# knightyxp/VideoCoF

Measured on AMD Instinct MI355X. Metric: denoised latent tokens/s (4-step 81f@480p Wan2.1 DiT denoise loop, all DiT tokens counted), higher is better.
Workload: dtype bf16; 1 GPU; Wan2.1-T2V-14B + VideoCoF layout, 4-step, 81f@480p (BASELINE configs[2]); layout=VideoCoF (src|ground|tgt), global_batch=1, parallelism=single

## Files before the change

include/wan_hip.h:

```cpp
#ifndef WAN_HIP_H
#define WAN_HIP_H

#include <stdint.h>

#ifdef __cplusplus
extern "C" {
#endif

#define WAN_ABI_VERSION 11

typedef enum {
    WAN_OK = 0,
    WAN_ERR_INVALID = 1,
    WAN_ERR_UNSUPPORTED = 2,
    WAN_ERR_LAUNCH = 3
} wan_status_t;

int wan_abi_version(void);
const char* wan_last_error(void);

wan_status_t wan_set_tuning(const char* key, int value);
int wan_get_tuning(const char* key);
#define WAN_ATTN_VARIANT_W4_LAZY 1
#define WAN_ATTN_VARIANT_W4_MAXFREE 2
#define WAN_ATTN_VARIANT_W8_RUNNING_MAX 3
#define WAN_ATTN_VARIANT_W4_LAZY_QK8 4
#define WAN_ATTN_VARIANT_W4_F8 5
#define WAN_ATTN_VARIANT_FAMILY_MASK 15
#define WAN_ATTN_VARIANT_XCD_PINNED 16
#define WAN_ATTN_VARIANT_SPLIT_TAIL 32

wan_status_t wan_ln_modulate(const float* x, const float* scale, const float* shift, int add_one,
                             void* out_bf16, int64_t rows, int dim, int64_t rows_per_batch,
                             float eps, void* stream);

typedef struct {
    int F, Hp, Wp;
    int mode;
    int f_src;
    int ground_end;
    int64_t token_offset;
    int64_t rows_per_batch;
    int max_pos;
} wan_rope_params;

wan_status_t wan_rmsnorm_rope(void* x0_bf16, const float* w0, void* x1_bf16, const float* w1,
                              int64_t ld, int64_t rows, int dim, int head_dim, float eps,
                              const float* rope_cos, const float* rope_sin,
                              const wan_rope_params* rp, float x0_scale, void* stream);

typedef enum {
    WAN_EPI_BF16 = 0,
    WAN_EPI_GELU_BF16 = 1,
    WAN_EPI_F32 = 2,
    WAN_EPI_RESID_F32 = 3,
    WAN_EPI_BF16_T = 4
} wan_epilogue_t;

wan_status_t wan_gemm_bf16(const void* A, int64_t lda, const void* W, int64_t ldw, const float* bias,
                           void* out, int64_t ldo, int M, int N, int K, int epilogue,
                           const float* gate, int64_t rows_per_batch, void* stream);
int wan_gemm_plan(int M, int N, int K);
#define WAN_GEMM_VARIANT_128 0
#define WAN_GEMM_VARIANT_256_W8 1
#define WAN_GEMM_VARIANT_256_W4 2
#define WAN_GEMM_VARIANT_256_PK 3

wan_status_t wan_gemm_bf16_ws(const void* A, int64_t lda, const void* W, int64_t ldw, const float* bias,
                              void* out, int64_t ldo, int M, int N, int K, int epilogue,
                              const float* gate, int64_t rows_per_batch, void* workspace, int64_t workspace_bytes, void* stream);
int64_t wan_gemm_workspace_bytes(int M, int N, int K);
int wan_gemm_ws_plan(int M, int N, int K);
int wan_gemm_ws_splits(int M, int N, int K);
int wan_gemm_pk_grid(int M, int N);
int wan_gemm_pk_segment(int M, int N, int K, int worker, int index, int* out);

wan_status_t wan_gemm_fp8(const void* A_fp8, int64_t lda, const float* a_row_scale, const void* W_fp8, int64_t ldw,
                          const float* w_row_scale, const float* bias, void* out, int64_t ldo, int M, int N, int K,
                          int epilogue, const float* gate, int64_t rows_per_batch, void* stream);
int wan_gemm_fp8_ws_plan(int M, int N, int K);
int64_t wan_gemm_fp8_workspace_bytes(int M, int N, int K);
wan_status_t wan_gemm_fp8_ws(const void* A_fp8, int64_t lda, const float* a_row_scale, const void* W_fp8, int64_t ldw,
                             const float* w_row_scale, const float* bias, void* out, int64_t ldo, int M, int N, int K,
                             int epilogue, const float* gate, int64_t rows_per_batch, void* workspace, int64_t workspace_bytes,
                             void* stream);
int wan_gemm_fp8_pk_segment(int M, int N, int K, int worker, int index, int* out);
wan_status_t wan_quantize_rows_fp8(const void* x_bf16, int64_t ldx, void* out_fp8, int64_t ldo, float* out_row_scale,
                                   int64_t rows, int cols, void* stream);
wan_status_t wan_ln_modulate_fp8(const float* x, const float* scale, const float* shift, int add_one, void* out_fp8,
                                 float* out_row_scale, int64_t rows, int dim, int64_t rows_per_batch, float eps, void* stream);

wan_status_t wan_attention_fwd(const void* q, int64_t ldq, int64_t q_bstride,
                               const void* k, int64_t ldk, int64_t k_bstride,
                               const void* vt, int64_t ldvt, int64_t vt_bstride,
                               void* out, int64_t ldo, int64_t o_bstride,
                               int batch, int Lq, int Lk, int num_heads, int head_dim,
                               float softmax_scale, int flags, void* workspace, int64_t workspace_bytes,
                               void* stream);
wan_status_t wan_attention_fwd_varlen(const void* q, int64_t ldq, int64_t q_bstride,
                                      const void* k, int64_t ldk, int64_t k_bstride,
                                      const void* vt, int64_t ldvt, int64_t vt_bstride,
                                      void* out, int64_t ldo, int64_t o_bstride,
                                      int batch, int Lq, int Lk, const int32_t* k_lens, int num_heads, int head_dim,
                                      float softmax_scale, int flags, void* workspace, int64_t workspace_bytes,
                                      void* stream);
int64_t wan_attention_workspace_bytes(int batch, int Lq, int Lk, int num_heads, int head_dim);
int wan_attention_plan(int batch, int Lq, int Lk, int num_heads, int head_dim, int flags, int64_t workspace_bytes);
#define WAN_ATTN_Q_PRESCALED 1
#define WAN_ATTN_QK_FP8 2
#define WAN_ATTN_PV_FP8 4
#define WAN_ATTN_QSCALE(softmax_scale) ((softmax_scale) * 1.4426950408889634f)

wan_status_t wan_attention_fwd_qk8(const void* q8, int64_t ldq8, int64_t q8_bstride, int q_exp,
                                   const void* k8, int64_t ldk8, int64_t k8_bstride, int k_exp,
                                   const void* vt, int64_t ldvt, int64_t vt_bstride,
                                   void* out, int64_t ldo, int64_t o_bstride,
                                   int batch, int Lq, int Lk, int num_heads, int head_dim,
                                   void* workspace, int64_t workspace_bytes, void* stream);
wan_status_t wan_attention_fwd_f8(const void* q8, int64_t ldq8, int64_t q8_bstride, int q_exp,
                                  const void* k8, int64_t ldk8, int64_t k8_bstride, int k_exp,
                                  const void* v8, int64_t ldv8, int64_t v8_bstride, const void* v8_scales,
                                  const void* vt, int64_t ldvt, int64_t vt_bstride,
                                  void* out, int64_t ldo, int64_t o_bstride,
                                  int batch, int Lq, int Lk, int num_heads, int head_dim,
                                  void* workspace, int64_t workspace_bytes, void* stream);
int64_t wan_vt_mx_scale_bytes(int batch, int num_heads, int Lk);
wan_status_t wan_vt_quantize_mx(const void* vt_bf16, int64_t ldvt, int64_t vt_bstride, int batch, int num_heads, int Lk,
                                void* v8, int64_t ldv8, int64_t v8_bstride, void* v8_scales, void* stream);
wan_status_t wan_rmsnorm_rope_fp8(const void* x0_bf16, const float* w0, const void* x1_bf16, const float* w1,
                                  int64_t ld, int64_t rows, int dim, int head_dim, float eps,
                                  const float* rope_cos, const float* rope_sin, const wan_rope_params* rp,
                                  float x0_scale, float x1_scale, void* out0_fp8, void* out1_fp8, void* stream);

int64_t wan_col_mean_workspace_bytes(int batch, int dim);
wan_status_t wan_col_mean_bf16(const void* x_bf16, int64_t ld, int64_t rows_per_batch, int valid_rows, int batch, int dim,
                               void* workspace, float* mean, void* stream);
wan_status_t wan_qk_quantize_fp8(const void* q_bf16, const void* k_bf16, int64_t ld, int64_t rows, int dim, int64_t rows_per_batch,
                                 const float* k_mean, float q_scale, float k_scale, void* q8, void* k8, void* stream);

wan_status_t wan_cross_probs(const void* q, int64_t ldq, const void* k, int64_t ldk, int64_t k_bstride, void* probs, int64_t ldp,
                             int batch, int64_t rows_per_batch, int num_heads, int kept, int pad_count, void* stream);
wan_status_t wan_cross_fold_values(const void* w_co, int64_t ldw, const void* vt, int64_t ldvt, int64_t vt_bstride, void* vfold,
                                   int64_t ldo, int64_t vfold_bstride, int batch, int dim, int num_heads, int kept, void* stream);
int wan_cross_fold_plan(int64_t rows, int num_heads, int text_len, int kept, int weights_bf16);
int64_t wan_cross_fold_workspace_bytes(int batch, int dim);

wan_status_t wan_transpose_bf16(const void* in, int64_t ld, void* out_t, int64_t ldt,
                                int64_t rows, int cols, void* stream);

wan_status_t wan_patchify(const void* latent, int in_dtype, void* tokens_bf16, int64_t ldt,
                          int Cin, int F, int H, int W, int pt, int ph, int pw, void* stream);
wan_status_t wan_unpatchify(const float* tokens, int64_t ldt, void* out, int out_dtype,
                            int Cout, int F, int Hp, int Wp, int pt, int ph, int pw, int zero_frames, void* stream);
wan_status_t wan_unpatchify_rep(const float* tokens, int64_t ldt, void* out, int out_dtype,
                                int Cout, int F, int Hp, int Wp, int pt, int ph, int pw, int zero_frames,
                                int rep, int64_t rep_stride, void* stream);

wan_status_t wan_rmsnorm_rope_sp(const void* x0_bf16, const float* w0, const void* x1_bf16, const float* w1,
                                 int64_t ld, int64_t rows, int dim, int head_dim, float eps,
                                 const float* rope_cos, const float* rope_sin, const wan_rope_params* rp,
                                 float x0_scale, void* wire0, void* wire1, int slabs, int batch, void* stream);
wan_status_t wan_sp_pack_heads(const void* x_bf16, int64_t ldx, void* wire, int P, int T, int B, int Cl, void* stream);
wan_status_t wan_sp_unpack_heads(const void* wire, void* x_bf16, int64_t ldx, int P, int T, int B, int Cl, void* stream);
wan_status_t wan_sp_unpack_vt(const void* wire, void* vt_bf16, int64_t ldvt, int P, int B, int Cl, int T, void* stream);
wan_status_t wan_rmsnorm_rope_sp_split(const void* x0_bf16, const float* w0, const void* x1_bf16, const float* w1,
                                       int64_t ld, int64_t rows, int dim, int head_dim, float eps,
                                       const float* rope_cos, const float* rope_sin, const wan_rope_params* rp,
                                       float x0_scale, void* wire0, void* wire1, int slabs, int batch, int split, void* stream);
wan_status_t wan_sp_pack_heads_split(const void* x_bf16, int64_t ldx, void* wire, int P, int T, int B, int Cl, int split, void* stream);
wan_status_t wan_sp_unpack_heads_split(const void* wire, void* x_bf16, int64_t ldx, int P, int T, int B, int Cl, int split, void* stream);

typedef struct wan_sp_comm wan_sp_comm;
#define WAN_SP_UNIQUE_ID_BYTES 128
wan_status_t wan_sp_unique_id(void* id128);
wan_status_t wan_sp_init(wan_sp_comm** comm, const void* id128, int rank, int world_size);
wan_status_t wan_sp_init_from_comm(wan_sp_comm** comm, void* nccl_comm, int rank, int world_size);
int wan_sp_rank(const wan_sp_comm* comm);
int wan_sp_world_size(const wan_sp_comm* comm);
wan_status_t wan_sp_a2a_scatter_heads(wan_sp_comm* comm, const void* send_wire, void* recv_wire, int64_t bytes_total, void* compute_stream);
wan_status_t wan_sp_a2a_gather_heads(wan_sp_comm* comm, const void* send_wire, void* recv_wire, int64_t bytes_total, void* compute_stream);
wan_status_t wan_sp_all_gather(wan_sp_comm* comm, const void* send, void* recv, int64_t bytes_per_rank, void* compute_stream);
wan_status_t wan_sp_wait(wan_sp_comm* comm, void* compute_stream);
int64_t wan_sp_ticket(const wan_sp_comm* comm);
wan_status_t wan_sp_wait_for(wan_sp_comm* comm, int64_t ticket, void* compute_stream);
wan_status_t wan_sp_destroy(wan_sp_comm* comm);

wan_status_t wan_sp_channel_copy(void* dst, const void* src, int64_t bytes, int channels, int threads, void* stream);

typedef struct {
    int dim, ffn_dim, num_heads, text_len;
    float eps;
    const void *w_qk, *w_v, *w_o, *w_cq, *w_co, *w_ffn0, *w_ffn2;
    const float *b_qk, *b_v, *b_o, *b_cq, *b_co, *b_ffn0, *b_ffn2;
    const float *norm_q, *norm_k, *norm_cq;
    const float *norm3_w, *norm3_b;
} wan_block_weights;

typedef struct {
    void *h, *qk, *att, *cq, *ff, *vt;
    int64_t ldvt;
    void* attn_ws_self; int64_t attn_ws_self_bytes;
    void* attn_ws_cross; int64_t attn_ws_cross_bytes;
    void* gemm_ws; int64_t gemm_ws_bytes;
    void* vfold; int64_t vfold_bytes;
    int text_kept;
} wan_block_workspace;

wan_status_t wan_dit_block_forward(float* x, const float* emod, const void* ctx_k, const void* ctx_vt,
                                   const wan_block_weights* w, const wan_block_workspace* ws,
                                   const float* rope_cos, const float* rope_sin, const wan_rope_params* rp,
                                   int batch, int64_t rows_per_batch, int64_t valid_tokens, void* stream);
wan_status_t wan_dit_block_tail_forward(float* x, const float* emod, const void* ctx_k, const void* ctx_vt,
                                        const wan_block_weights* w, const wan_block_workspace* ws,
                                        int batch, int64_t rows_per_batch, void* stream);
wan_status_t wan_dit_block_workspace_bytes(int dim, int ffn_dim, int batch, int64_t rows_per_batch, int64_t valid_tokens,
                                           int64_t* bytes , int64_t* ldvt);

typedef struct {
    int num_layers, in_dim, out_dim, pt, ph, pw;
    const wan_block_weights* blocks;
    const void* pe_w; const float* pe_b;
    const void* head_w; const float* head_b;
} wan_dit_weights;

typedef struct {
    wan_block_workspace block;
    float* x;
    void* tokens;
    float* head_out;
} wan_dit_workspace;

wan_status_t wan_dit_forward(const void* latent, int latent_dtype, void* out, int out_dtype, const float* emod,
                             const float* ehead, const void* const* ctx_k, const void* const* ctx_vt,
                             const wan_dit_weights* w, const wan_dit_workspace* ws, const float* rope_cos,
                             const float* rope_sin, const wan_rope_params* rp, int batch, int F, int H, int W,
                             int64_t rows_per_batch, int zero_frames, void* stream);
wan_status_t wan_dit_forward_rep(const void* latent, int latent_dtype, void* out, int out_dtype, const float* emod,
                                 const float* ehead, const void* const* ctx_k, const void* const* ctx_vt,
                                 const wan_dit_weights* w, const wan_dit_workspace* ws, const float* rope_cos,
                                 const float* rope_sin, const wan_rope_params* rp, int batch, int F, int H, int W,
                                 int64_t rows_per_batch, int zero_frames, int rep, void* stream);

wan_status_t wan_lincomb(void* out, int dtype, const void* x0, const void* x1, const void* x2, const void* x3,
                         float c0, float c1, float c2, float c3, int64_t n, void* stream);

wan_status_t wan_solver_step(void* x0_out, void* prev_out, int dtype, const void* sample, const void* v, const void* m1,
                             const void* m2, const float* noise, float a_s, float a_v, float c_s, float c_0, float c_1,
                             float c_2, float c_n, int64_t n, void* stream);


typedef struct {
    int T_in, H_in, W_in, Cin;
    int T_out, H_out, W_out, Cout;
    int KT, KH, KW;
    int st, sh, sw;
    int pt, ph, pw;
    int upsample2x;
    int time_interleave;
} wan_conv_params;

wan_status_t wan_conv_cl(const void* x, const void* hist, int hist_frames, const void* w, int64_t ldw,
                         const float* bias, const void* resid, void* out, int64_t ldo,
                         const wan_conv_params* p, void* stream);

wan_status_t wan_rmsnorm_silu_cl(const void* x_bf16, const float* gamma, void* out_bf16, int64_t rows, int C,
                                 int silu, void* stream);

wan_status_t wan_softmax_rows(const float* scores, int64_t lds, void* probs_bf16, int64_t ldp, int64_t rows,
                              int n, int npad, float scale, void* stream);

wan_status_t wan_video_to_cl(const void* video, int in_dtype, void* out_bf16, int Cv, int Cpad, int64_t npix, void* stream);
wan_status_t wan_cl_to_video(const void* x_bf16, int64_t ld, void* out, int out_dtype, int Cv, int64_t npix,
                             int clamp, void* stream);


wan_status_t wan_frames_u8_to_video(const void* frames_u8, void* out, int out_dtype, int B, int T, int H, int W,
                                    void* stream);

wan_status_t wan_video_to_frames_u8(const void* video, int in_dtype, void* frames_u8, int B, int T, int H, int W,
                                    int t0, int nt, int T_out, int t_dst, void* stream);

#define WAN_RESAMPLE_MAX_TAPS 24
int64_t wan_frames_resample_table_bytes(int n_out, int taps);
wan_status_t wan_frames_u8_resample(const void* src_u8, void* dst_u8, int B, int T, int H, int W, int Ho, int Wo,
                                    const void* xtab, int kx, const void* ytab, int ky, void* stream);

#define WAN_COMPOSE_MAX_SRC 16
enum { WAN_COMPOSE_U8 = 0, WAN_COMPOSE_F32 = 1, WAN_COMPOSE_BF16 = 2 };
enum { WAN_COMPOSE_COPY = 0, WAN_COMPOSE_LOADER_ROUNDTRIP = 1, WAN_COMPOSE_WRITER = 2, WAN_COMPOSE_NORMALIZE = 3 };
typedef struct {
    const void* base;
    const int* rescale_flag;
    int64_t extent;
    int64_t stride_c, stride_t, stride_y, stride_x;
// ... 74 lines not shown
```

videocof_amd/_lib.py:

```python
from __future__ import annotations

import ctypes
import os
from ctypes import POINTER, Structure, c_char_p, c_float, c_int, c_int64, c_void_p

_HERE = os.path.dirname(os.path.abspath(__file__))
LIB_PATH = os.environ.get("WAN_HIP_LIB") or os.path.join(_HERE, "libwan_hip.so")
ABI_VERSION = 11
ATTN_Q_PRESCALED = 1
LOG2E = 1.4426950408889634
ATTN_VARIANT_NAMES = {1: "attn_fwd_w4_kernel<.,.,ref> (4-wave, lazy softmax reference)",
                      2: "attn_fwd_w4_kernel<.,false,0> (4-wave, max-free attempt) + attn_fwd_w4_kernel<.,false,1,true> (lazy-reference fix-up of flagged workgroups)",
                      3: "(retired in round 5: the 8-wave running-max kernel)",
                      4: "attn_fwd_w4_kernel<0,.,1,false,true> (4-wave, lazy softmax reference, QK^T on the fp8 matrix pipe)",
                      5: "attn_fwd_f8_kernel (4-wave, QK^T and P.V on the fp8 matrix pipe, checked max-free softmax) + "
                         "attn_fwd_w4_kernel<0,false,1,true,true> (fp8-QK^T lazy-reference fix-up of flagged workgroups)"}
ATTN_VARIANT_XCD_PINNED, ATTN_VARIANT_SPLIT_TAIL = 16, 32
GEMM_VARIANT_KERNELS = {0: "gemm_bf16_kernel", 1: "gemm256_kernel", 2: "gemm_w4_kernel", 3: "gemm_pk_kernel"}


def attn_variant_name(code: int) -> str:
    name = ATTN_VARIANT_NAMES.get(code & 15, f"unknown({code})")
    if code & ATTN_VARIANT_XCD_PINNED:
        name += ", heads pinned to XCDs"
    if code & ATTN_VARIANT_SPLIT_TAIL:
        name += " + split-KV tail round (4-wave SPLIT kernel + attn_combine_kernel)"
    return name

WAN_OK, WAN_ERR_INVALID, WAN_ERR_UNSUPPORTED, WAN_ERR_LAUNCH = 0, 1, 2, 3
EPI_BF16, EPI_GELU_BF16, EPI_F32, EPI_RESID_F32, EPI_BF16_T = 0, 1, 2, 3, 4


class RopeParams(Structure):
    _fields_ = [("F", c_int), ("Hp", c_int), ("Wp", c_int), ("mode", c_int), ("f_src", c_int),
                ("ground_end", c_int), ("token_offset", c_int64), ("rows_per_batch", c_int64),
                ("max_pos", c_int)]


class BoxProbeResult(Structure):
    _fields_ = [("mfma_mix_tflops", c_float), ("copy_tbps", c_float), ("mfma_ms", c_float), ("copy_ms", c_float)]


class ComposeSrc(Structure):
    _fields_ = ([("base", c_void_p), ("rescale_flag", c_void_p), ("extent", c_int64)] +
                [(n, c_int64) for n in ("stride_c", "stride_t", "stride_y", "stride_x")] +
                [(n, c_int) for n in ("kind", "mode", "rescale", "t0", "y0", "x0", "nt", "h", "w", "dst_y", "dst_x")])


COMPOSE_MAX_SRC = 16
COMPOSE_U8, COMPOSE_F32, COMPOSE_BF16 = 0, 1, 2
COMPOSE_COPY, COMPOSE_LOADER_ROUNDTRIP, COMPOSE_WRITER, COMPOSE_NORMALIZE = 0, 1, 2, 3


class YuvPlanes(Structure):
    _fields_ = ([(n, c_void_p) for n in ("y", "cb", "cr")] +
                [(n, c_int64) for n in ("y_extent", "cb_extent", "cr_extent", "y_row", "y_frame", "c_row", "c_frame")] +
                [(n, c_int) for n in ("c_step", "sub_x", "sub_y", "cosited")])


class YuvCoef(Structure):
    _fields_ = [("k", c_int * 9), ("yo", c_int)]


class ConvParams(Structure):
    _fields_ = [(n, c_int) for n in ("T_in", "H_in", "W_in", "Cin", "T_out", "H_out", "W_out", "Cout",
                                     "KT", "KH", "KW", "st", "sh", "sw", "pt", "ph", "pw",
                                     "upsample2x", "time_interleave")]


class BlockWeights(Structure):
    _fields_ = ([(n, c_int) for n in ("dim", "ffn_dim", "num_heads", "text_len")] + [("eps", c_float)] +
                [(n, c_void_p) for n in ("w_qk", "w_v", "w_o", "w_cq", "w_co", "w_ffn0", "w_ffn2",
                                         "b_qk", "b_v", "b_o", "b_cq", "b_co", "b_ffn0", "b_ffn2",
                                         "norm_q", "norm_k", "norm_cq", "norm3_w", "norm3_b")])


class BlockWorkspace(Structure):
    _fields_ = ([(n, c_void_p) for n in ("h", "qk", "att", "cq", "ff", "vt")] + [("ldvt", c_int64)] +
                [("attn_ws_self", c_void_p), ("attn_ws_self_bytes", c_int64),
                 ("attn_ws_cross", c_void_p), ("attn_ws_cross_bytes", c_int64),
                 ("gemm_ws", c_void_p), ("gemm_ws_bytes", c_int64),
                 ("vfold", c_void_p), ("vfold_bytes", c_int64), ("text_kept", c_int)])


class DitWeights(Structure):
    _fields_ = ([(n, c_int) for n in ("num_layers", "in_dim", "out_dim", "pt", "ph", "pw")] +
                [("blocks", POINTER(BlockWeights))] + [(n, c_void_p) for n in ("pe_w", "pe_b", "head_w", "head_b")])


class DitWorkspace(Structure):
    _fields_ = [("block", BlockWorkspace), ("x", c_void_p), ("tokens", c_void_p), ("head_out", c_void_p)]


SIGNATURES = {
    "wan_abi_version": (c_int, []),
    "wan_box_probe_scratch_bytes": (c_int64, []),
    "wan_box_probe": (c_int, [POINTER(BoxProbeResult), c_void_p, c_int64, c_int, c_void_p]),
    "wan_last_error": (c_char_p, []),
    "wan_set_tuning": (c_int, [c_char_p, c_int]),
    "wan_get_tuning": (c_int, [c_char_p]),
    "wan_ln_modulate": (c_int, [c_void_p, c_void_p, c_void_p, c_int, c_void_p, c_int64, c_int, c_int64,
                                c_float, c_void_p]),
    "wan_rmsnorm_rope": (c_int, [c_void_p, c_void_p, c_void_p, c_void_p, c_int64, c_int64, c_int, c_int,
                                 c_float, c_void_p, c_void_p, POINTER(RopeParams), c_float, c_void_p]),
    "wan_gemm_bf16": (c_int, [c_void_p, c_int64, c_void_p, c_int64, c_void_p, c_void_p, c_int64,
                              c_int, c_int, c_int, c_int, c_void_p, c_int64, c_void_p]),
    "wan_rmsnorm_rope_sp": (c_int, [c_void_p, c_void_p, c_void_p, c_void_p, c_int64, c_int64, c_int, c_int,
                                    c_float, c_void_p, c_void_p, POINTER(RopeParams), c_float, c_void_p, c_void_p, c_int, c_int,
                                    c_void_p]),
    "wan_sp_pack_heads": (c_int, [c_void_p, c_int64, c_void_p, c_int, c_int, c_int, c_int, c_void_p]),
    "wan_sp_unpack_heads": (c_int, [c_void_p, c_void_p, c_int64, c_int, c_int, c_int, c_int, c_void_p]),
    "wan_sp_unpack_vt": (c_int, [c_void_p, c_void_p, c_int64, c_int, c_int, c_int, c_int, c_void_p]),
    "wan_rmsnorm_rope_sp_split": (c_int, [c_void_p, c_void_p, c_void_p, c_void_p, c_int64, c_int64, c_int, c_int,
                                          c_float, c_void_p, c_void_p, POINTER(RopeParams), c_float, c_void_p, c_void_p, c_int, c_int,
                                          c_int, c_void_p]),
    "wan_sp_pack_heads_split": (c_int, [c_void_p, c_int64, c_void_p, c_int, c_int, c_int, c_int, c_int, c_void_p]),
    "wan_sp_unpack_heads_split": (c_int, [c_void_p, c_void_p, c_int64, c_int, c_int, c_int, c_int, c_int, c_void_p]),
    "wan_dit_block_forward": (c_int, [c_void_p, c_void_p, c_void_p, c_void_p, POINTER(BlockWeights), POINTER(BlockWorkspace),
                                      c_void_p, c_void_p, POINTER(RopeParams), c_int, c_int64, c_int64, c_void_p]),
    "wan_dit_block_tail_forward": (c_int, [c_void_p, c_void_p, c_void_p, c_void_p, POINTER(BlockWeights), POINTER(BlockWorkspace),
                                           c_int, c_int64, c_void_p]),
    "wan_dit_forward": (c_int, [c_void_p, c_int, c_void_p, c_int, c_void_p, c_void_p, POINTER(c_void_p), POINTER(c_void_p),
                                POINTER(DitWeights), POINTER(DitWorkspace), c_void_p, c_void_p, POINTER(RopeParams),
                                c_int, c_int, c_int, c_int, c_int64, c_int, c_void_p]),
    "wan_dit_forward_rep": (c_int, [c_void_p, c_int, c_void_p, c_int, c_void_p, c_void_p, POINTER(c_void_p), POINTER(c_void_p),
                                    POINTER(DitWeights), POINTER(DitWorkspace), c_void_p, c_void_p, POINTER(RopeParams),
                                    c_int, c_int, c_int, c_int, c_int64, c_int, c_int, c_void_p]),
    "wan_dit_block_workspace_bytes": (c_int, [c_int, c_int, c_int, c_int64, c_int64, POINTER(c_int64), POINTER(c_int64)]),
    "wan_gemm_fp8": (c_int, [c_void_p, c_int64, c_void_p, c_void_p, c_int64, c_void_p, c_void_p, c_void_p, c_int64,
                             c_int, c_int, c_int, c_int, c_void_p, c_int64, c_void_p]),
    "wan_gemm_fp8_ws": (c_int, [c_void_p, c_int64, c_void_p, c_void_p, c_int64, c_void_p, c_void_p, c_void_p, c_int64,
                                c_int, c_int, c_int, c_int, c_void_p, c_int64, c_void_p, c_int64, c_void_p]),
    "wan_gemm_fp8_ws_plan": (c_int, [c_int, c_int, c_int]),
    "wan_gemm_fp8_workspace_bytes": (c_int64, [c_int, c_int, c_int]),
    "wan_gemm_fp8_pk_segment": (c_int, [c_int, c_int, c_int, c_int, c_int, POINTER(c_int)]),
    "wan_quantize_rows_fp8": (c_int, [c_void_p, c_int64, c_void_p, c_int64, c_void_p, c_int64, c_int, c_void_p]),
    "wan_ln_modulate_fp8": (c_int, [c_void_p, c_void_p, c_void_p, c_int, c_void_p, c_void_p, c_int64, c_int, c_int64,
                                    c_float, c_void_p]),
    "wan_attention_fwd": (c_int, [c_void_p, c_int64, c_int64, c_void_p, c_int64, c_int64,
                                  c_void_p, c_int64, c_int64, c_void_p, c_int64, c_int64,
                                  c_int, c_int, c_int, c_int, c_int, c_float, c_int, c_void_p, c_int64, c_void_p]),
    "wan_attention_fwd_varlen": (c_int, [c_void_p, c_int64, c_int64, c_void_p, c_int64, c_int64,
                                         c_void_p, c_int64, c_int64, c_void_p, c_int64, c_int64,
                                         c_int, c_int, c_int, c_void_p, c_int, c_int, c_float, c_int, c_void_p, c_int64, c_void_p]),
    "wan_attention_fwd_qk8": (c_int, [c_void_p, c_int64, c_int64, c_int, c_void_p, c_int64, c_int64, c_int,
                                      c_void_p, c_int64, c_int64, c_void_p, c_int64, c_int64,
                                      c_int, c_int, c_int, c_int, c_int, c_void_p, c_int64, c_void_p]),
    "wan_rmsnorm_rope_fp8": (c_int, [c_void_p, c_void_p, c_void_p, c_void_p, c_int64, c_int64, c_int, c_int,
                                     c_float, c_void_p, c_void_p, POINTER(RopeParams), c_float, c_float, c_void_p, c_void_p,
                                     c_void_p]),
    "wan_attention_fwd_f8": (c_int, [c_void_p, c_int64, c_int64, c_int, c_void_p, c_int64, c_int64, c_int,
                                     c_void_p, c_int64, c_int64, c_void_p, c_void_p, c_int64, c_int64, c_void_p, c_int64, c_int64,
                                     c_int, c_int, c_int, c_int, c_int, c_void_p, c_int64, c_void_p]),
    "wan_vt_mx_scale_bytes": (c_int64, [c_int, c_int, c_int]),
    "wan_vt_quantize_mx": (c_int, [c_void_p, c_int64, c_int64, c_int, c_int, c_int, c_void_p, c_int64, c_int64, c_void_p, c_void_p]),
    "wan_col_mean_workspace_bytes": (c_int64, [c_int, c_int]),
    "wan_col_mean_bf16": (c_int, [c_void_p, c_int64, c_int64, c_int, c_int, c_int, c_void_p, c_void_p, c_void_p]),
    "wan_qk_quantize_fp8": (c_int, [c_void_p, c_void_p, c_int64, c_int64, c_int, c_int64, c_void_p, c_float, c_float, c_void_p, c_void_p,
                                    c_void_p]),
    "wan_attention_workspace_bytes": (c_int64, [c_int, c_int, c_int, c_int, c_int]),
    "wan_cross_probs": (c_int, [c_void_p, c_int64, c_void_p, c_int64, c_int64, c_void_p, c_int64, c_int, c_int64, c_int, c_int, c_int,
                                c_void_p]),
    "wan_cross_fold_values": (c_int, [c_void_p, c_int64, c_void_p, c_int64, c_int64, c_void_p, c_int64, c_int64, c_int, c_int, c_int,
                                      c_int, c_void_p]),
    "wan_cross_fold_plan": (c_int, [c_int64, c_int, c_int, c_int, c_int]),
    "wan_cross_fold_workspace_bytes": (c_int64, [c_int, c_int]),
    "wan_sp_unique_id": (c_int, [c_void_p]),
    "wan_sp_init": (c_int, [ctypes.POINTER(c_void_p), c_void_p, c_int, c_int]),
    "wan_sp_init_from_comm": (c_int, [ctypes.POINTER(c_void_p), c_void_p, c_int, c_int]),
    "wan_sp_rank": (c_int, [c_void_p]),
    "wan_sp_world_size": (c_int, [c_void_p]),
    "wan_sp_a2a_scatter_heads": (c_int, [c_void_p, c_void_p, c_void_p, c_int64, c_void_p]),
    "wan_sp_a2a_gather_heads": (c_int, [c_void_p, c_void_p, c_void_p, c_int64, c_void_p]),
    "wan_sp_all_gather": (c_int, [c_void_p, c_void_p, c_void_p, c_int64, c_void_p]),
    "wan_sp_wait": (c_int, [c_void_p, c_void_p]),
    "wan_sp_ticket": (c_int64, [c_void_p]),
    "wan_sp_wait_for": (c_int, [c_void_p, c_int64, c_void_p]),
    "wan_sp_destroy": (c_int, [c_void_p]),
    "wan_sp_channel_copy": (c_int, [c_void_p, c_void_p, c_int64, c_int, c_int, c_void_p]),
    "wan_attention_plan": (c_int, [c_int, c_int, c_int, c_int, c_int, c_int, c_int64]),
    "wan_gemm_plan": (c_int, [c_int, c_int, c_int]),
    "wan_gemm_ws_plan": (c_int, [c_int, c_int, c_int]),
    "wan_gemm_ws_splits": (c_int, [c_int, c_int, c_int]),
    "wan_gemm_workspace_bytes": (c_int64, [c_int, c_int, c_int]),
    "wan_gemm_pk_grid": (c_int, [c_int, c_int]),
    "wan_gemm_pk_segment": (c_int, [c_int, c_int, c_int, c_int, c_int, POINTER(c_int)]),
    "wan_gemm_bf16_ws": (c_int, [c_void_p, c_int64, c_void_p, c_int64, c_void_p, c_void_p, c_int64,
                                 c_int, c_int, c_int, c_int, c_void_p, c_int64, c_void_p, c_int64, c_void_p]),
    "wan_transpose_bf16": (c_int, [c_void_p, c_int64, c_void_p, c_int64, c_int64, c_int, c_void_p]),
    "wan_patchify": (c_int, [c_void_p, c_int, c_void_p, c_int64, c_int, c_int, c_int, c_int,
                             c_int, c_int, c_int, c_void_p]),
    "wan_unpatchify": (c_int, [c_void_p, c_int64, c_void_p, c_int, c_int, c_int, c_int, c_int,
                               c_int, c_int, c_int, c_int, c_void_p]),
    "wan_unpatchify_rep": (c_int, [c_void_p, c_int64, c_void_p, c_int, c_int, c_int, c_int, c_int,
                                   c_int, c_int, c_int, c_int, c_int, c_int64, c_void_p]),
    "wan_lincomb": (c_int, [c_void_p, c_int, c_void_p, c_void_p, c_void_p, c_void_p, c_float, c_float, c_float, c_float,
                            c_int64, c_void_p]),
    "wan_solver_step": (c_int, [c_void_p, c_void_p, c_int, c_void_p, c_void_p, c_void_p, c_void_p, c_void_p, c_float, c_float,
                                c_float, c_float, c_float, c_float, c_float, c_int64, c_void_p]),
    "wan_gemm_bf16_batched": (c_int, [c_void_p, c_int64, c_int64, c_void_p, c_int64, c_int64, c_void_p, c_int64, c_int64,
                                      c_int, c_int, c_int, c_int, c_int, c_void_p]),
    "wan_embedding_rows": (c_int, [c_void_p, c_void_p, c_int64, c_void_p, c_int64, c_int, c_void_p]),
    "wan_rmsnorm_rows": (c_int, [c_void_p, c_void_p, c_void_p, c_int, c_int64, c_int, c_float, c_void_p]),
    "wan_t5_softmax_bias": (c_int, [c_void_p, c_int64, c_void_p, c_void_p, c_void_p, c_int64, c_int, c_int, c_int, c_int,
                                    c_int, c_void_p]),
    "wan_mul_bf16": (c_int, [c_void_p, c_void_p, c_void_p, c_int64, c_void_p]),
    "wan_conv_cl": (c_int, [c_void_p, c_void_p, c_int, c_void_p, c_int64, c_void_p, c_void_p, c_void_p, c_int64,
                            POINTER(ConvParams), c_void_p]),
    "wan_rmsnorm_silu_cl": (c_int, [c_void_p, c_void_p, c_void_p, c_int64, c_int, c_int, c_void_p]),
    "wan_softmax_rows": (c_int, [c_void_p, c_int64, c_void_p, c_int64, c_int64, c_int, c_int, c_float, c_void_p]),
    "wan_video_to_cl": (c_int, [c_void_p, c_int, c_void_p, c_int, c_int, c_int64, c_void_p]),
    "wan_cl_to_video": (c_int, [c_void_p, c_int64, c_void_p, c_int, c_int, c_int64, c_int, c_void_p]),
    "wan_frames_u8_to_video": (c_int, [c_void_p, c_void_p, c_int, c_int, c_int, c_int, c_int, c_void_p]),
    "wan_video_to_frames_u8": (c_int, [c_void_p, c_int, c_void_p, c_int, c_int, c_int, c_int, c_int, c_int, c_int, c_int,
                                       c_void_p]),
    "wan_frames_resample_table_bytes": (c_int64, [c_int, c_int]),
    "wan_frames_u8_resample": (c_int, [c_void_p, c_void_p, c_int, c_int, c_int, c_int, c_int, c_int, c_void_p, c_int, c_void_p, c_int,
                                       c_void_p]),
    "wan_frames_u8_compose": (c_int, [POINTER(ComposeSrc), c_int, c_void_p, c_int, c_int, c_int, c_int, c_void_p]),
    "wan_video_range_flag": (c_int, [c_void_p, c_int, c_int64, c_void_p, c_void_p]),
    "wan_yuv_to_frames_u8": (c_int, [POINTER(YuvPlanes), POINTER(YuvCoef), c_void_p, c_int, c_int, c_int, c_void_p]),
    "wan_frames_u8_to_yuv": (c_int, [c_void_p, POINTER(YuvPlanes), POINTER(YuvCoef), c_int, c_int, c_int, c_void_p]),
    "wan_change_mask_workspace_bytes": (c_int64, [c_int, c_int, c_int, c_int]),
    "wan_change_mask": (c_int, [c_void_p, c_void_p, c_void_p, c_int, c_int, c_int, c_int, c_int, c_int, c_int, c_int, c_int, c_void_p,
                                c_int64, c_void_p]),
    "wan_plane_u8_resample": (c_int, [c_void_p, c_void_p, c_void_p, c_int, c_int, c_int, c_int, c_int, c_void_p, c_int, c_void_p, c_int,
                                      c_void_p]),
    "wan_frames_u8_composite": (c_int, [c_void_p, c_void_p, c_void_p, c_void_p, c_int, c_int, c_int, c_int, c_int, c_int, c_int,
                                        c_void_p]),
    "wan_clip_stats_workspace_bytes": (c_int64, [c_int, c_int, c_int]),
    "wan_clip_stats": (c_int, [c_void_p, c_void_p, c_void_p, c_void_p, c_int, c_int, c_int, c_int, c_void_p, c_int64, c_void_p]),
}

_lib = None


def load() -> ctypes.CDLL:
    global _lib
    if _lib is not None:
        return _lib
    if not os.path.isfile(LIB_PATH):
        raise RuntimeError(
            f"{LIB_PATH} not found: the HIP kernels are not built. Run `make` (or "
            "`python -c 'import __graft_entry__ as g; g.build()'`) in the repo root. "
            "There is no CPU/eager fallback for this path.")
    lib = ctypes.CDLL(LIB_PATH)
    for name, (res, args) in SIGNATURES.items():
        try:
            fn = getattr(lib, name)
        except AttributeError as e:
            raise RuntimeError(f"{LIB_PATH} does not export `{name}` (stale build?)") from e
        fn.restype = res
        fn.argtypes = args
    if lib.wan_abi_version() != ABI_VERSION:
        raise RuntimeError(f"libwan_hip ABI {lib.wan_abi_version()} != binding ABI {ABI_VERSION}; rebuild")
    _lib = lib
    return lib


def check(status: int, what: str) -> None:
    if status == WAN_OK:
        return
    msg = load().wan_last_error().decode(errors="replace")
    if status == WAN_ERR_INVALID:
        raise ValueError(f"{what}: {msg}")
    raise RuntimeError(f"{what}: {msg} (status {status})")
```

videocof_amd/csrc/common.hpp:

```cpp
#pragma once
#include <hip/hip_runtime.h>
#include <stdint.h>
#include <stdio.h>
#include <stdarg.h>

#include "../../include/wan_hip.h"

typedef __bf16 bf16_t;
typedef __bf16 bf16x2 __attribute__((ext_vector_type(2)));
typedef __bf16 bf16x4 __attribute__((ext_vector_type(4)));
typedef __bf16 bf16x8 __attribute__((ext_vector_type(8)));
typedef float f32x2 __attribute__((ext_vector_type(2)));
typedef float f32x4 __attribute__((ext_vector_type(4)));
typedef float f32x16 __attribute__((ext_vector_type(16)));
typedef unsigned int u32x2 __attribute__((ext_vector_type(2)));
typedef unsigned int u32x4 __attribute__((ext_vector_type(4)));

#define WAN_WAVE 64

void wan_set_error(const char* fmt, ...);
int wan_cu_count();
int wan_resident_cus();
enum { WAN_TUNE_ATTN_TAIL = 0, WAN_TUNE_ATTN_FAST, WAN_TUNE_ATTN_XCD_MAP, WAN_TUNE_GEMM_GM, WAN_TUNE_GEMM_PHASES,
       WAN_TUNE_DEBUG_CHECKS, WAN_TUNE_GEMM_VARIANT, WAN_TUNE_CONV_XCD, WAN_TUNE_GEMM_W4, WAN_TUNE_CONV_FAST, WAN_TUNE_CONV_PATCH, WAN_TUNE_ATTN_REF, WAN_TUNE_CONV_HEAD, WAN_TUNE_GEMM_EXP, WAN_TUNE_GEMM_PK, WAN_TUNE_GEMM_PK_WORKERS, WAN_TUNE_GEMM_PK_MIN_UNITS, WAN_TUNE_GEMM_PK_ORDER, WAN_TUNE_GEMM_PK_FORM, WAN_TUNE_ROW_GROUP, WAN_TUNE_SP_INLINE, WAN_TUNE_GEMM_SPLITK, WAN_TUNE_CONV_MFMA, WAN_TUNE_ATTN_PERSIST, WAN_TUNE_SP_RESERVE_CUS, WAN_TUNE_CROSS_FOLD, WAN_TUNE_COUNT };
int wan_tune(int which);
void wan_note_attn_variant(int variant);
void wan_note_cross_fold(int folded);
int wan_last_cross_fold();
#ifdef __cplusplus
#include <atomic>
wan_status_t wan_once_per_device(std::atomic<uint64_t>& done, wan_status_t (*init)());
#endif
#define WAN_REQUIRE(cond, code, ...)            \
    do {                                        \
        if (!(cond)) {                          \
            wan_set_error(__VA_ARGS__);         \
            return (code);                      \
        }                                       \
    } while (0)
#define WAN_CHECK_LAUNCH(name)                                                        \
    do {                                                                              \
        hipError_t e__ = hipGetLastError();                                           \
        if (e__ != hipSuccess) {                                                      \
            wan_set_error("%s: launch failed: %s", name, hipGetErrorString(e__));     \
            return WAN_ERR_LAUNCH;                                                    \
        }                                                                             \
    } while (0)

__device__ __forceinline__ float bf16lo_to_f32(unsigned int w) { return __uint_as_float(w << 16); }
__device__ __forceinline__ float bf16hi_to_f32(unsigned int w) { return __uint_as_float(w & 0xffff0000u); }

__device__ __forceinline__ unsigned int pack_bf16x2(float lo, float hi) {
    f32x2 v = {lo, hi};
    bf16x2 b = __builtin_convertvector(v, bf16x2);
    return __builtin_bit_cast(unsigned int, b);
}

__device__ __forceinline__ float wave_sum(float v) {
#pragma unroll
    for (int o = 32; o > 0; o >>= 1) v += __shfl_xor(v, o, 64);
    return v;
}

template <int NW>
__device__ __forceinline__ float block_sum(float v, float* red) {
    v = wave_sum(v);
    const int wid = threadIdx.x >> 6;
    __syncthreads();
    if ((threadIdx.x & 63) == 0) red[wid] = v;
    __syncthreads();
    float t = 0.f;
#pragma unroll
    for (int i = 0; i < NW; ++i) t += red[i];
    return t;
}

__device__ __forceinline__ float wave_max(float v) {
#pragma unroll
    for (int o = 32; o > 0; o >>= 1) v = fmaxf(v, __shfl_xor(v, o, 64));
    return v;
}

template <int NW>
__device__ __forceinline__ float block_max(float v, float* red) {
    v = wave_max(v);
    const int wid = threadIdx.x >> 6;
    __syncthreads();
    if ((threadIdx.x & 63) == 0) red[wid] = v;
    __syncthreads();
    float t = red[0];
#pragma unroll
    for (int i = 1; i < NW; ++i) t = fmaxf(t, red[i]);
    return t;
}

__device__ __forceinline__ unsigned int pack_fp8x4(float a, float b, float c, float d) {
    a = fminf(fmaxf(a, -448.f), 448.f); b = fminf(fmaxf(b, -448.f), 448.f);
    c = fminf(fmaxf(c, -448.f), 448.f); d = fminf(fmaxf(d, -448.f), 448.f);
    int w = __builtin_amdgcn_cvt_pk_fp8_f32(a, b, 0, false);
    w = __builtin_amdgcn_cvt_pk_fp8_f32(c, d, w, true);
    return (unsigned int)w;
}

__device__ __forceinline__ float gelu_tanh_f32(float x) {
    constexpr float k1 = -2.0f * 0.7978845608028654f * 1.4426950408889634f;
    constexpr float k3 = k1 * 0.044715f;
    const float a = __builtin_fmaf(x * x, k3, k1) * x;
    return x * __builtin_amdgcn_rcpf(1.0f + __builtin_amdgcn_exp2f(a));
}

__device__ __forceinline__ void glds16(const void* gsrc, void* lds_wave_base) {
    __builtin_amdgcn_global_load_lds(
        (const __attribute__((address_space(1))) void*)gsrc,
        (__attribute__((address_space(3))) void*)lds_wave_base, 16, 0, 0);
}
```

videocof_amd/csrc/cross_fold.hip:

```cpp
#include "common.hpp"

#include <math.h>

namespace {

constexpr int CF_KEYS = 64;
constexpr int CF_D = 128;
constexpr int CF_PROB_NB = 8;
constexpr int CF_FOLD_NB = 2;
constexpr int CF_VS_LD = CF_D + 8;

__device__ __forceinline__ int perm_row(int t, int r) { return 16 * (r >> 3) + 8 * ((r >> 2) & 1) + 4 * t + (r & 3); }

__device__ __forceinline__ void mfma_head(const bf16x8 (&a)[2][8], const bf16x8 (&b)[8], f32x16 (&acc)[2]) {
#pragma unroll
    for (int t = 0; t < 2; ++t) {
#pragma unroll
        for (int i = 0; i < 16; ++i) acc[t][i] = 0.f;
#pragma unroll
        for (int s = 0; s < 8; ++s) acc[t] = __builtin_amdgcn_mfma_f32_32x32x16_bf16(a[t][s], b[s], acc[t], 0, 0, 0);
    }
}

__device__ __forceinline__ u32x4 pack8(const f32x16 (&acc)[2], int i) {
    u32x4 o;
    o[0] = pack_bf16x2(acc[0][4 * i + 0], acc[0][4 * i + 1]);
    o[1] = pack_bf16x2(acc[0][4 * i + 2], acc[0][4 * i + 3]);
    o[2] = pack_bf16x2(acc[1][4 * i + 0], acc[1][4 * i + 1]);
    o[3] = pack_bf16x2(acc[1][4 * i + 2], acc[1][4 * i + 3]);
    return o;
}

__global__ __launch_bounds__(256) void cross_probs_kernel(const bf16_t* __restrict__ q, int64_t ldq, const bf16_t* __restrict__ k,
                                                          int64_t ldk, int64_t k_bstride, bf16_t* __restrict__ p, int64_t ldp, int L,
                                                          int kept, float log2_pad) {
    const int lane = threadIdx.x & 63, wave = threadIdx.x >> 6, r = lane & 31, g = lane >> 5;
    const int h = blockIdx.y, b = blockIdx.z;
    const bf16x8 zero8 = {0, 0, 0, 0, 0, 0, 0, 0};
    bf16x8 ka[2][8];
    const bf16_t* kh = k + (int64_t)b * k_bstride + (int64_t)h * CF_D + g * 64;
#pragma unroll
    for (int t = 0; t < 2; ++t) {
        const int key = perm_row(t, r);
#pragma unroll
        for (int s = 0; s < 8; ++s) ka[t][s] = key <= kept ? *(const bf16x8*)(kh + (int64_t)key * ldk + s * 8) : zero8;
    }
    const int first = blockIdx.x * (4 * CF_PROB_NB);
    for (int it = 0; it < CF_PROB_NB; ++it) {
        const int row0 = (first + it * 4 + wave) * 32;
        if (row0 >= L) break;
        const int row = row0 + r;
        const int64_t grow = (int64_t)b * L + (row < L ? row : L - 1);
        const bf16_t* qr = q + grow * ldq + (int64_t)h * CF_D + g * 64;
        bf16x8 qb[8];
#pragma unroll
        for (int s = 0; s < 8; ++s) qb[s] = *(const bf16x8*)(qr + s * 8);
        f32x16 acc[2];
        mfma_head(ka, qb, acc);
        float m = -INFINITY;
#pragma unroll
        for (int t = 0; t < 2; ++t)
#pragma unroll
            for (int i = 0; i < 4; ++i)
#pragma unroll
                for (int jj = 0; jj < 4; ++jj) {
                    const int key = 16 * i + 8 * g + 4 * t + jj;
                    float s = acc[t][4 * i + jj];
                    s = key == kept ? s + log2_pad : s;
                    s = key > kept ? -INFINITY : s;
                    acc[t][4 * i + jj] = s;
                    m = fmaxf(m, s);
                }
        m = fmaxf(m, __shfl_xor(m, 32, 64));
        float sum = 0.f;
#pragma unroll
        for (int t = 0; t < 2; ++t)
#pragma unroll
            for (int i = 0; i < 16; ++i) {
                const float e = __builtin_amdgcn_exp2f(acc[t][i] - m);
                acc[t][i] = e;
                sum += e;
            }
        sum += __shfl_xor(sum, 32, 64);
        const float inv = __builtin_amdgcn_rcpf(sum);
#pragma unroll
        for (int t = 0; t < 2; ++t)
#pragma unroll
            for (int i = 0; i < 16; ++i) acc[t][i] *= inv;
        if (row < L) {
            bf16_t* pr = p + grow * ldp + (int64_t)h * CF_KEYS + 8 * g;
#pragma unroll
            for (int i = 0; i < 4; ++i) *(u32x4*)(pr + 16 * i) = pack8(acc, i);
        }
    }
}

__global__ __launch_bounds__(256) void cross_fold_kernel(const bf16_t* __restrict__ w, int64_t ldw, const bf16_t* __restrict__ vt,
                                                         int64_t ldvt, int64_t vt_bstride, bf16_t* __restrict__ out, int64_t ldo,
                                                         int64_t out_bstride, int C, int kept) {
    __shared__ __attribute__((aligned(16))) bf16_t vs[CF_KEYS * CF_VS_LD];
    const int lane = threadIdx.x & 63, wave = threadIdx.x >> 6, r = lane & 31, g = lane >> 5;
    const int h = blockIdx.y, b = blockIdx.z;
    const bf16_t* vh = vt + (int64_t)b * vt_bstride + (int64_t)h * CF_D * ldvt;
#pragma unroll
    for (int it = 0; it < 4; ++it) {
        const int idx = it * 256 + threadIdx.x, d = idx >> 3, c = idx & 7;
        bf16x8 v = {0, 0, 0, 0, 0, 0, 0, 0};
        if (c * 8 <= kept) v = *(const bf16x8*)(vh + (int64_t)d * ldvt + c * 8);
#pragma unroll
        for (int e = 0; e < 8; ++e) vs[(c * 8 + e) * CF_VS_LD + d] = c * 8 + e <= kept ? v[e] : (bf16_t)0.f;
    }
    __syncthreads();
    bf16x8 va[2][8];
#pragma unroll
    for (int t = 0; t < 2; ++t)
#pragma unroll
        for (int s = 0; s < 8; ++s) va[t][s] = *(const bf16x8*)(vs + perm_row(t, r) * CF_VS_LD + g * 64 + s * 8);
    const int first = blockIdx.x * (4 * CF_FOLD_NB);
    for (int it = 0; it < CF_FOLD_NB; ++it) {
        const int n0 = (first + it * 4 + wave) * 32;
        if (n0 >= C) break;
        const int n = n0 + r;
        const bf16_t* wr = w + (int64_t)n * ldw + (int64_t)h * CF_D + g * 64;
        bf16x8 wb[8];
#pragma unroll
        for (int s = 0; s < 8; ++s) wb[s] = *(const bf16x8*)(wr + s * 8);
        f32x16 acc[2];
        mfma_head(va, wb, acc);
        bf16_t* orow = out + (int64_t)b * out_bstride + (int64_t)n * ldo + (int64_t)h * CF_KEYS + 8 * g;
#pragma unroll
        for (int i = 0; i < 4; ++i) *(u32x4*)(orow + 16 * i) = pack8(acc, i);
    }
}

inline bool aligned16(const void* p) { return ((uintptr_t)p & 15) == 0; }

std::atomic<int> g_last_cross_fold{0};

}

int wan_last_cross_fold() { return g_last_cross_fold.load(std::memory_order_relaxed); }
void wan_note_cross_fold(int folded) { g_last_cross_fold.store(folded, std::memory_order_relaxed); }

#define WAN_CROSS_FOLD_MIN_ROWS 2048
extern "C" int wan_cross_fold_plan(int64_t rows, int num_heads, int text_len, int kept, int weights_bf16) {
    const int mode = wan_tune(WAN_TUNE_CROSS_FOLD);
    if (mode <= 0 || !weights_bf16 || rows <= 0 || num_heads <= 0) return 0;
    if (kept < 1 || kept + 1 > CF_KEYS || kept >= text_len) return 0;
    if (mode >= 2) return 1;
    const int K = num_heads * CF_KEYS;
    if (K < 1024 || K % 128 != 0) return 0;
    return rows >= WAN_CROSS_FOLD_MIN_ROWS ? 1 : 0;
}

extern "C" int64_t wan_cross_fold_workspace_bytes(int batch, int dim) {
    if (batch <= 0 || dim <= 0 || dim % CF_D != 0) return 0;
    return (int64_t)batch * dim * (dim / CF_D * CF_KEYS) * 2;
}

extern "C" wan_status_t wan_cross_probs(const void* q, int64_t ldq, const void* k, int64_t ldk, int64_t k_bstride, void* probs,
                                        int64_t ldp, int batch, int64_t rows_per_batch, int num_heads, int kept, int pad_count,
                                        void* stream) {
    WAN_REQUIRE(q && k && probs, WAN_ERR_INVALID, "wan_cross_probs: null tensor");
    WAN_REQUIRE(batch > 0 && rows_per_batch > 0 && num_heads > 0 && (int64_t)batch * rows_per_batch <= 0x7fffffff && batch <= 65535 &&
                    num_heads <= 65535,
                WAN_ERR_INVALID, "wan_cross_probs: batch=%d rows_per_batch=%lld heads=%d", batch, (long long)rows_per_batch, num_heads);
    WAN_REQUIRE(kept >= 0 && kept + 1 <= CF_KEYS && pad_count >= 1, WAN_ERR_UNSUPPORTED,
                "wan_cross_probs: kept=%d (kept + 1 distinct keys must be <= 64) pad_count=%d", kept, pad_count);
    WAN_REQUIRE(ldq >= (int64_t)num_heads * CF_D && ldk >= (int64_t)num_heads * CF_D && ldp >= (int64_t)num_heads * CF_KEYS &&
                    k_bstride >= (int64_t)(kept + 1) * ldk,
                WAN_ERR_INVALID, "wan_cross_probs: ldq=%lld ldk=%lld ldp=%lld k_bstride=%lld too small", (long long)ldq, (long long)ldk,
                (long long)ldp, (long long)k_bstride);
    WAN_REQUIRE(ldq % 8 == 0 && ldk % 8 == 0 && ldp % 8 == 0 && k_bstride % 8 == 0 && aligned16(q) && aligned16(k) && aligned16(probs),
                WAN_ERR_INVALID, "wan_cross_probs: rows must be 16-byte aligned");
    const int L = (int)rows_per_batch;
    const int per_wg = 32 * 4 * CF_PROB_NB;
    dim3 grid((L + per_wg - 1) / per_wg, num_heads, batch);
    hipLaunchKernelGGL(cross_probs_kernel, grid, dim3(256), 0, (hipStream_t)stream, (const bf16_t*)q, ldq, (const bf16_t*)k, ldk,
                       k_bstride, (bf16_t*)probs, ldp, L, kept, log2f((float)pad_count));
    WAN_CHECK_LAUNCH("wan_cross_probs");
    return WAN_OK;
}

extern "C" wan_status_t wan_cross_fold_values(const void* w_co, int64_t ldw, const void* vt, int64_t ldvt, int64_t vt_bstride,
                                              void* vfold, int64_t ldo, int64_t vfold_bstride, int batch, int dim, int num_heads,
                                              int kept, void* stream) {
    WAN_REQUIRE(w_co && vt && vfold, WAN_ERR_INVALID, "wan_cross_fold_values: null tensor");
    WAN_REQUIRE(batch > 0 && batch <= 65535 && num_heads > 0 && num_heads <= 65535 && dim == num_heads * CF_D, WAN_ERR_UNSUPPORTED,
                "wan_cross_fold_values: batch=%d dim=%d heads=%d (head_dim must be 128)", batch, dim, num_heads);
    WAN_REQUIRE(kept >= 0 && kept + 1 <= CF_KEYS, WAN_ERR_UNSUPPORTED, "wan_cross_fold_values: kept=%d (kept + 1 must be <= 64)", kept);
    const int64_t K = (int64_t)num_heads * CF_KEYS;
    WAN_REQUIRE(ldw >= dim && ldvt >= (kept + 8) / 8 * 8 && ldo >= K && vt_bstride >= (int64_t)dim * ldvt && vfold_bstride >= (int64_t)dim * ldo,
                WAN_ERR_INVALID, "wan_cross_fold_values: ldw=%lld ldvt=%lld ldo=%lld vt_bstride=%lld vfold_bstride=%lld too small",
                (long long)ldw, (long long)ldvt, (long long)ldo, (long long)vt_bstride, (long long)vfold_bstride);
    WAN_REQUIRE(ldw % 8 == 0 && ldvt % 8 == 0 && ldo % 8 == 0 && vt_bstride % 8 == 0 && vfold_bstride % 8 == 0 && aligned16(w_co) &&
                    aligned16(vt) && aligned16(vfold),
                WAN_ERR_INVALID, "wan_cross_fold_values: rows must be 16-byte aligned");
    const int per_wg = 32 * 4 * CF_FOLD_NB;
    dim3 grid((dim + per_wg - 1) / per_wg, num_heads, batch);
    hipLaunchKernelGGL(cross_fold_kernel, grid, dim3(256), 0, (hipStream_t)stream, (const bf16_t*)w_co, ldw, (const bf16_t*)vt, ldvt,
                       vt_bstride, (bf16_t*)vfold, ldo, vfold_bstride, dim, kept);
    WAN_CHECK_LAUNCH("wan_cross_fold_values");
    return WAN_OK;
}
```

videocof_amd/csrc/dit_block.cpp:

```cpp
#include "common.hpp"

namespace {
inline const char* at(const void* p, int64_t bytes) { return (const char*)p + bytes; }
inline char* at(void* p, int64_t bytes) { return (char*)p + bytes; }
}

#define WAN_TRY(call)                   \
    do {                                \
        const wan_status_t st__ = (call); \
        if (st__ != WAN_OK) return st__; \
    } while (0)

extern "C" wan_status_t wan_dit_block_tail_forward(float* x, const float* emod, const void* ctx_k, const void* ctx_vt,
                                                   const wan_block_weights* w, const wan_block_workspace* ws,
                                                   int batch, int64_t rows_per_batch, void* stream);

extern "C" wan_status_t wan_dit_block_forward(float* x, const float* emod, const void* ctx_k, const void* ctx_vt,
                                              const wan_block_weights* w, const wan_block_workspace* ws,
                                              const float* rope_cos, const float* rope_sin, const wan_rope_params* rp,
                                              int batch, int64_t rows_per_batch, int64_t valid_tokens, void* stream) {
    WAN_REQUIRE(x && emod && ctx_k && ctx_vt && w && ws && rope_cos && rope_sin && rp, WAN_ERR_INVALID,
                "wan_dit_block_forward: null argument");
    WAN_REQUIRE(batch > 0 && rows_per_batch > 0 && valid_tokens > 0 && valid_tokens <= rows_per_batch, WAN_ERR_INVALID,
                "wan_dit_block_forward: batch=%d rows_per_batch=%lld valid_tokens=%lld", batch, (long long)rows_per_batch,
                (long long)valid_tokens);
    const int C = w->dim, F = w->ffn_dim, H = w->num_heads, T = w->text_len;
    WAN_REQUIRE(C > 0 && H > 0 && C == H * 128 && F > 0 && T > 0, WAN_ERR_UNSUPPORTED,
                "wan_dit_block_forward: dim=%d heads=%d (head_dim must be 128) ffn=%d text_len=%d", C, H, F, T);
    WAN_REQUIRE(ws->h && ws->qk && ws->att && ws->cq && ws->ff && ws->vt, WAN_ERR_INVALID, "wan_dit_block_forward: null workspace");
    void* const GWS = ws->gemm_ws;
    const int64_t GWSB = ws->gemm_ws_bytes;
    const int64_t Ll = rows_per_batch, M = (int64_t)batch * Ll;
    WAN_REQUIRE(M <= 0x7fffffff && valid_tokens <= 0x7fffffff, WAN_ERR_UNSUPPORTED, "wan_dit_block_forward: too many rows");
    const int64_t lk_pad = (valid_tokens + 63) / 64 * 64;
    WAN_REQUIRE(ws->ldvt >= lk_pad && ws->ldvt % 8 == 0, WAN_ERR_INVALID,
                "wan_dit_block_forward: ldvt=%lld must be >= roundup(valid_tokens,64)=%lld and a multiple of 8", (long long)ws->ldvt,
                (long long)lk_pad);
    const float eps = w->eps;
    const float qs = (float)(0.08838834764831845 * 1.4426950408889634);
    const int64_t bC = (int64_t)batch * C;
    const float* shift_msa = emod, *scale_msa = emod + bC, *gate_msa = emod + 2 * bC;
    void* qk = ws->qk;
    void* kpart = at(qk, (int64_t)C * 2);
    wan_rope_params rope = *rp;
    rope.rows_per_batch = Ll;

    WAN_TRY(wan_ln_modulate(x, scale_msa, shift_msa, 1, ws->h, M, C, Ll, eps, stream));
    WAN_TRY(wan_gemm_bf16_ws(ws->h, C, w->w_qk, C, w->b_qk, qk, 2 * C, (int)M, 2 * C, C, WAN_EPI_BF16, nullptr, 0, GWS, GWSB, stream));
    WAN_TRY(wan_rmsnorm_rope(qk, w->norm_q, kpart, w->norm_k, 2 * C, M, C, 128, eps, rope_cos, rope_sin, &rope, qs, stream));
    for (int b = 0; b < batch; ++b)
        WAN_TRY(wan_gemm_bf16_ws(at(ws->h, (int64_t)b * Ll * C * 2), C, w->w_v, C, w->b_v, at(ws->vt, (int64_t)b * C * ws->ldvt * 2),
                              ws->ldvt, (int)valid_tokens, C, C, WAN_EPI_BF16_T, nullptr, 0, GWS, GWSB, stream));
    WAN_TRY(wan_attention_fwd(qk, 2 * C, Ll * 2 * C, kpart, 2 * C, Ll * 2 * C, ws->vt, ws->ldvt, (int64_t)C * ws->ldvt, ws->att, C, Ll * C,
                              batch, (int)Ll, (int)valid_tokens, H, 128, 0.f, WAN_ATTN_Q_PRESCALED, ws->attn_ws_self,
                              ws->attn_ws_self_bytes, stream));
    WAN_TRY(wan_gemm_bf16_ws(ws->att, C, w->w_o, C, w->b_o, x, C, (int)M, C, C, WAN_EPI_RESID_F32, gate_msa, Ll, GWS, GWSB, stream));
    return wan_dit_block_tail_forward(x, emod, ctx_k, ctx_vt, w, ws, batch, rows_per_batch, stream);
}

extern "C" wan_status_t wan_dit_block_tail_forward(float* x, const float* emod, const void* ctx_k, const void* ctx_vt,
                                                   const wan_block_weights* w, const wan_block_workspace* ws,
                                                   int batch, int64_t rows_per_batch, void* stream) {
    WAN_REQUIRE(x && emod && ctx_k && ctx_vt && w && ws, WAN_ERR_INVALID, "wan_dit_block_tail_forward: null argument");
    WAN_REQUIRE(batch > 0 && rows_per_batch > 0, WAN_ERR_INVALID, "wan_dit_block_tail_forward: batch=%d rows_per_batch=%lld", batch,
                (long long)rows_per_batch);
    const int C = w->dim, F = w->ffn_dim, H = w->num_heads, T = w->text_len;
    WAN_REQUIRE(C > 0 && H > 0 && C == H * 128 && F > 0 && T > 0, WAN_ERR_UNSUPPORTED,
                "wan_dit_block_tail_forward: dim=%d heads=%d (head_dim must be 128) ffn=%d text_len=%d", C, H, F, T);
    WAN_REQUIRE(ws->h && ws->att && ws->cq && ws->ff, WAN_ERR_INVALID, "wan_dit_block_tail_forward: null workspace");
    void* const GWS = ws->gemm_ws;
    const int64_t GWSB = ws->gemm_ws_bytes;
    const int64_t Ll = rows_per_batch, M = (int64_t)batch * Ll;
    WAN_REQUIRE(M <= 0x7fffffff, WAN_ERR_UNSUPPORTED, "wan_dit_block_tail_forward: too many rows");
    const float eps = w->eps;
    const float qs = (float)(0.08838834764831845 * 1.4426950408889634);
    const int64_t bC = (int64_t)batch * C;
    const float* shift_mlp = emod + 3 * bC, *scale_mlp = emod + 4 * bC, *gate_mlp = emod + 5 * bC;
    WAN_TRY(wan_ln_modulate(x, w->norm3_w, w->norm3_b, 0, ws->h, M, C, M, eps, stream));
    WAN_TRY(wan_gemm_bf16_ws(ws->h, C, w->w_cq, C, w->b_cq, ws->cq, C, (int)M, C, C, WAN_EPI_BF16, nullptr, 0, GWS, GWSB, stream));
    WAN_TRY(wan_rmsnorm_rope(ws->cq, w->norm_cq, nullptr, nullptr, C, M, C, 128, eps, nullptr, nullptr, nullptr, qs, stream));
    const int kept = ws->text_kept;
    const bool fold = ws->vfold && ws->vfold_bytes >= wan_cross_fold_workspace_bytes(batch, C) && wan_cross_fold_plan(M, H, T, kept, 1);
    wan_note_cross_fold(fold ? 1 : 0);
    if (fold) {
        const int64_t Kf = (int64_t)H * 64;
        WAN_TRY(wan_cross_probs(ws->cq, C, ctx_k, C, (int64_t)T * C, ws->att, Kf, batch, Ll, H, kept, T - kept, stream));
        WAN_TRY(wan_cross_fold_values(w->w_co, C, ctx_vt, T, (int64_t)C * T, ws->vfold, Kf, (int64_t)C * Kf, batch, C, H, kept, stream));
        for (int b = 0; b < batch; ++b)
            WAN_TRY(wan_gemm_bf16_ws(at(ws->att, (int64_t)b * Ll * Kf * 2), Kf, at(ws->vfold, (int64_t)b * C * Kf * 2), Kf, w->b_co,
                                  x + (int64_t)b * Ll * C, C, (int)Ll, C, (int)Kf, WAN_EPI_RESID_F32, nullptr, 0, GWS, GWSB, stream));
    } else {
        WAN_TRY(wan_attention_fwd(ws->cq, C, Ll * C, ctx_k, C, (int64_t)T * C, ctx_vt, T, (int64_t)C * T, ws->att, C, Ll * C, batch, (int)Ll,
                                  T, H, 128, 0.f, WAN_ATTN_Q_PRESCALED, ws->attn_ws_cross, ws->attn_ws_cross_bytes, stream));
        WAN_TRY(wan_gemm_bf16_ws(ws->att, C, w->w_co, C, w->b_co, x, C, (int)M, C, C, WAN_EPI_RESID_F32, nullptr, 0, GWS, GWSB, stream));
    }
    WAN_TRY(wan_ln_modulate(x, scale_mlp, shift_mlp, 1, ws->h, M, C, Ll, eps, stream));
    WAN_TRY(wan_gemm_bf16_ws(ws->h, C, w->w_ffn0, C, w->b_ffn0, ws->ff, F, (int)M, F, C, WAN_EPI_GELU_BF16, nullptr, 0, GWS, GWSB, stream));
    WAN_TRY(wan_gemm_bf16_ws(ws->ff, F, w->w_ffn2, F, w->b_ffn2, x, C, (int)M, C, F, WAN_EPI_RESID_F32, gate_mlp, Ll, GWS, GWSB, stream));
    return WAN_OK;
}

extern "C" wan_status_t wan_dit_block_workspace_bytes(int dim, int ffn_dim, int batch, int64_t rows_per_batch, int64_t valid_tokens,
                                                      int64_t* bytes , int64_t* ldvt) {
    WAN_REQUIRE(bytes && ldvt && dim > 0 && ffn_dim > 0 && batch > 0 && rows_per_batch > 0 && valid_tokens > 0, WAN_ERR_INVALID,
                "wan_dit_block_workspace_bytes: bad argument");
    const int64_t M = (int64_t)batch * rows_per_batch;
    *ldvt = (valid_tokens + 63) / 64 * 64;
    bytes[0] = M * dim * 2; bytes[1] = M * 2 * dim * 2; bytes[2] = M * dim * 2; bytes[3] = M * dim * 2;
    bytes[4] = M * ffn_dim * 2; bytes[5] = (int64_t)batch * dim * *ldvt * 2;
    return WAN_OK;
}

static wan_status_t dit_forward(const void* latent, int latent_dtype, void* out, int out_dtype, const float* emod,
                                const float* ehead, const void* const* ctx_k, const void* const* ctx_vt,
                                const wan_dit_weights* w, const wan_dit_workspace* ws, const float* rope_cos,
                                const float* rope_sin, const wan_rope_params* rp, int batch, int F, int H, int W,
                                int64_t rows_per_batch, int zero_frames, int rep, void* stream) {
    WAN_REQUIRE(latent && out && emod && ehead && ctx_k && ctx_vt && w && ws && rp, WAN_ERR_INVALID, "wan_dit_forward: null argument");
    WAN_REQUIRE(w->num_layers > 0 && w->blocks && w->pe_w && w->pe_b && w->head_w && w->head_b, WAN_ERR_INVALID,
                "wan_dit_forward: incomplete weights");
    WAN_REQUIRE(ws->x && ws->tokens && ws->head_out, WAN_ERR_INVALID, "wan_dit_forward: null workspace");
    void* const GWS = ws->block.gemm_ws;
    const int64_t GWSB = ws->block.gemm_ws_bytes;
    const int pt = w->pt, ph = w->ph, pw = w->pw;
    WAN_REQUIRE(pt > 0 && ph > 0 && pw > 0 && F > 0 && H > 0 && W > 0 && F % pt == 0 && H % ph == 0 && W % pw == 0, WAN_ERR_INVALID,
                "wan_dit_forward: latent (%d,%d,%d) is not a multiple of the patch (%d,%d,%d)", F, H, W, pt, ph, pw);
    const int gf = F / pt, gh = H / ph, gw = W / pw;
    const int64_t L = (int64_t)gf * gh * gw, Ll = rows_per_batch;
    WAN_REQUIRE(batch > 0 && L <= Ll && (int64_t)batch * Ll <= 0x7fffffff, WAN_ERR_INVALID,
                "wan_dit_forward: batch=%d tokens=%lld rows_per_batch=%lld", batch, (long long)L, (long long)Ll);
    WAN_REQUIRE(rp->F == gf && rp->Hp == gh && rp->Wp == gw, WAN_ERR_INVALID, "wan_dit_forward: rope grid (%d,%d,%d) != latent grid (%d,%d,%d)",
                rp->F, rp->Hp, rp->Wp, gf, gh, gw);
    const int C = w->blocks[0].dim;
    const int pv = pt * ph * pw, Kpe = w->in_dim * pv, Nh = w->out_dim * pv;
    const int64_t M = (int64_t)batch * Ll;
    const int64_t lat_el = latent_dtype == 0 ? 4 : 2, out_el = out_dtype == 0 ? 4 : 2;
    WAN_REQUIRE((latent_dtype == 0 || latent_dtype == 1) && (out_dtype == 0 || out_dtype == 1), WAN_ERR_INVALID,
                "wan_dit_forward: dtypes must be 0 (fp32) or 1 (bf16)");

    WAN_REQUIRE(hipMemsetAsync(ws->x, 0, (size_t)M * C * 4, (hipStream_t)stream) == hipSuccess, WAN_ERR_LAUNCH,
                "wan_dit_forward: hipMemsetAsync failed");
    for (int b = 0; b < batch; ++b) {
        WAN_TRY(wan_patchify(at(latent, (int64_t)b * w->in_dim * F * H * W * lat_el), latent_dtype, ws->tokens, Kpe, w->in_dim, F, H, W,
                             pt, ph, pw, stream));
        WAN_TRY(wan_gemm_bf16_ws(ws->tokens, Kpe, w->pe_w, Kpe, w->pe_b, ws->x + (int64_t)b * Ll * C, C, (int)L, C, Kpe, WAN_EPI_F32,
                              nullptr, 0, GWS, GWSB, stream));
    }
    const int64_t emod_layer = 6 * (int64_t)batch * C;
    for (int l = 0; l < w->num_layers; ++l) {
        WAN_REQUIRE(w->blocks[l].dim == C, WAN_ERR_INVALID, "wan_dit_forward: block %d has dim %d != %d", l, w->blocks[l].dim, C);
        WAN_TRY(wan_dit_block_forward(ws->x, emod + l * emod_layer, ctx_k[l], ctx_vt[l], &w->blocks[l], &ws->block, rope_cos, rope_sin, rp,
                                      batch, Ll, L, stream));
    }
    const int64_t bC = (int64_t)batch * C;
    WAN_TRY(wan_ln_modulate(ws->x, ehead + bC, ehead, 1, ws->block.h, M, C, Ll, w->blocks[0].eps, stream));
    WAN_TRY(wan_gemm_bf16_ws(ws->block.h, C, w->head_w, C, w->head_b, ws->head_out, Nh, (int)M, Nh, C, WAN_EPI_F32, nullptr, 0, GWS, GWSB, stream));
    WAN_REQUIRE(rep >= 1, WAN_ERR_INVALID, "wan_dit_forward: rep=%d", rep);
    const int64_t sample = (int64_t)w->out_dim * F * H * W;
    for (int b = 0; b < batch; ++b) {
        if (rep == 1)
            WAN_TRY(wan_unpatchify(ws->head_out + (int64_t)b * Ll * Nh, Nh, at(out, b * sample * out_el), out_dtype,
                                   w->out_dim, gf, gh, gw, pt, ph, pw, zero_frames, stream));
        else
            WAN_TRY(wan_unpatchify_rep(ws->head_out + (int64_t)b * Ll * Nh, Nh, at(out, b * sample * out_el), out_dtype,
                                       w->out_dim, gf, gh, gw, pt, ph, pw, zero_frames, rep, batch * sample, stream));
    }
    return WAN_OK;
}

extern "C" wan_status_t wan_dit_forward(const void* latent, int latent_dtype, void* out, int out_dtype, const float* emod,
                                        const float* ehead, const void* const* ctx_k, const void* const* ctx_vt,
                                        const wan_dit_weights* w, const wan_dit_workspace* ws, const float* rope_cos,
                                        const float* rope_sin, const wan_rope_params* rp, int batch, int F, int H, int W,
                                        int64_t rows_per_batch, int zero_frames, void* stream) {
    return dit_forward(latent, latent_dtype, out, out_dtype, emod, ehead, ctx_k, ctx_vt, w, ws, rope_cos, rope_sin, rp, batch, F, H, W,
                       rows_per_batch, zero_frames, 1, stream);
}

extern "C" wan_status_t wan_dit_forward_rep(const void* latent, int latent_dtype, void* out, int out_dtype, const float* emod,
                                            const float* ehead, const void* const* ctx_k, const void* const* ctx_vt,
                                            const wan_dit_weights* w, const wan_dit_workspace* ws, const float* rope_cos,
                                            const float* rope_sin, const wan_rope_params* rp, int batch, int F, int H, int W,
                                            int64_t rows_per_batch, int zero_frames, int rep, void* stream) {
    return dit_forward(latent, latent_dtype, out, out_dtype, emod, ehead, ctx_k, ctx_vt, w, ws, rope_cos, rope_sin, rp, batch, F, H, W,
                       rows_per_batch, zero_frames, rep, stream);
}
```

videocof_amd/csrc/norm_kernels.hip:

```cpp
#include "common.hpp"

namespace {

constexpr int kThreads = 256;
constexpr int kWaves = kThreads / 64;

template <int NV, bool FP8 = false>
__global__ __launch_bounds__(kThreads) void ln_modulate_kernel(
    const float* __restrict__ x, const float* __restrict__ scale, const float* __restrict__ shift,
    float add_one, bf16_t* __restrict__ out, int dim, int64_t rows_per_batch, float eps, float* __restrict__ row_scale = nullptr) {
    __shared__ float red[kWaves];
    const int64_t row = blockIdx.x;
    const int64_t b = row / rows_per_batch;
    const int nvec = dim >> 2;
    const float4* xr = reinterpret_cast<const float4*>(x + row * (int64_t)dim);
    float4 v[NV];
    float s = 0.f;
#pragma unroll
    for (int i = 0; i < NV; ++i) {
        const int idx = threadIdx.x + i * kThreads;
        if (idx < nvec) {
            v[i] = xr[idx];
            s += (v[i].x + v[i].y) + (v[i].z + v[i].w);
        } else {
            v[i] = make_float4(0.f, 0.f, 0.f, 0.f);
        }
    }
    const float mean = block_sum<kWaves>(s, red) / (float)dim;
    float q = 0.f;
#pragma unroll
    for (int i = 0; i < NV; ++i) {
        const int idx = threadIdx.x + i * kThreads;
        if (idx < nvec) {
            const float a = v[i].x - mean, bb = v[i].y - mean, c = v[i].z - mean, d = v[i].w - mean;
            q += (a * a + bb * bb) + (c * c + d * d);
        }
    }
    const float rstd = rsqrtf(block_sum<kWaves>(q, red) / (float)dim + eps);
    const float4* sc = scale ? reinterpret_cast<const float4*>(scale + b * dim) : nullptr;
    const float4* sh = shift ? reinterpret_cast<const float4*>(shift + b * dim) : nullptr;
    u32x2* orow = reinterpret_cast<u32x2*>(out + row * (int64_t)dim);
    float amax = 0.f;
#pragma unroll
    for (int i = 0; i < NV; ++i) {
        const int idx = threadIdx.x + i * kThreads;
        if (idx < nvec) {
            float4 a = make_float4(add_one, add_one, add_one, add_one);
            float4 c = make_float4(0.f, 0.f, 0.f, 0.f);
            if (sc) { const float4 t = sc[idx]; a.x += t.x; a.y += t.y; a.z += t.z; a.w += t.w; }
            else if (add_one == 0.f) { a = make_float4(1.f, 1.f, 1.f, 1.f); }
            if (sh) c = sh[idx];
            const float y0 = (v[i].x - mean) * rstd * a.x + c.x;
            const float y1 = (v[i].y - mean) * rstd * a.y + c.y;
            const float y2 = (v[i].z - mean) * rstd * a.z + c.z;
            const float y3 = (v[i].w - mean) * rstd * a.w + c.w;
            if constexpr (FP8) {
                v[i] = make_float4(y0, y1, y2, y3);
                amax = fmaxf(fmaxf(amax, fmaxf(fabsf(y0), fabsf(y1))), fmaxf(fabsf(y2), fabsf(y3)));
            } else {
                u32x2 o = {pack_bf16x2(y0, y1), pack_bf16x2(y2, y3)};
                orow[idx] = o;
            }
        }
    }
    if constexpr (FP8) {
        amax = fmaxf(block_max<kWaves>(amax, red), 1e-12f);
        const float s = amax * (1.0f / 448.0f), inv = 448.0f / amax;
        if (threadIdx.x == 0) row_scale[row] = s;
        unsigned int* qrow = reinterpret_cast<unsigned int*>(reinterpret_cast<unsigned char*>(out) + row * (int64_t)dim);
#pragma unroll
        for (int i = 0; i < NV; ++i) {
            const int idx = threadIdx.x + i * kThreads;
            if (idx < nvec) qrow[idx] = pack_fp8x4(v[i].x * inv, v[i].y * inv, v[i].z * inv, v[i].w * inv);
        }
    }
}


template <int NW, int R>
__device__ __forceinline__ void block_sum_n(float (&v)[R], float (*red)[NW]) {
#pragma unroll
    for (int r = 0; r < R; ++r) v[r] = wave_sum(v[r]);
    const int wid = threadIdx.x >> 6;
    __syncthreads();
    if ((threadIdx.x & 63) == 0) {
#pragma unroll
        for (int r = 0; r < R; ++r) red[r][wid] = v[r];
    }
    __syncthreads();
#pragma unroll
    for (int r = 0; r < R; ++r) {
        float t = 0.f;
#pragma unroll
        for (int i = 0; i < NW; ++i) t += red[r][i];
        v[r] = t;
    }
}

template <int NV, int R>
__global__ __launch_bounds__(kThreads) void ln_modulate_rows_kernel(
    const float* __restrict__ x, const float* __restrict__ scale, const float* __restrict__ shift,
    float add_one, bf16_t* __restrict__ out, int dim, int64_t rows, int64_t rows_per_batch, float eps) {
    __shared__ float red[R][kWaves];
    const int64_t row0 = (int64_t)blockIdx.x * R;
    const int nvec = dim >> 2;
    float4 v[R][NV];
#pragma unroll
    for (int r = 0; r < R; ++r) {
        const float4* xr = reinterpret_cast<const float4*>(x + (row0 + r) * (int64_t)dim);
        const bool live = row0 + r < rows;
#pragma unroll
        for (int i = 0; i < NV; ++i) {
            const int idx = threadIdx.x + i * kThreads;
            v[r][i] = (live && idx < nvec) ? xr[idx] : make_float4(0.f, 0.f, 0.f, 0.f);
        }
    }
    float s[R];
#pragma unroll
    for (int r = 0; r < R; ++r) {
        s[r] = 0.f;
#pragma unroll
        for (int i = 0; i < NV; ++i)
            if (threadIdx.x + i * kThreads < nvec) s[r] += (v[r][i].x + v[r][i].y) + (v[r][i].z + v[r][i].w);
    }
    block_sum_n<kWaves, R>(s, red);
    float mean[R], q[R];
#pragma unroll
    for (int r = 0; r < R; ++r) {
        mean[r] = s[r] / (float)dim;
        q[r] = 0.f;
#pragma unroll
        for (int i = 0; i < NV; ++i) {
            if (threadIdx.x + i * kThreads < nvec) {
                const float a = v[r][i].x - mean[r], bb = v[r][i].y - mean[r], c = v[r][i].z - mean[r], d = v[r][i].w - mean[r];
                q[r] += (a * a + bb * bb) + (c * c + d * d);
            }
        }
    }
    block_sum_n<kWaves, R>(q, red);
    const int64_t last = (row0 + R < rows ? row0 + R : rows) - 1;
    const int64_t b0 = row0 / rows_per_batch;
    const bool one_sample = last / rows_per_batch == b0;
#pragma unroll
    for (int i = 0; i < NV; ++i) {
        const int idx = threadIdx.x + i * kThreads;
        if (idx < nvec) {
            float4 a, c;
            auto fetch = [&](int64_t b) {
                a = make_float4(add_one, add_one, add_one, add_one);
                c = make_float4(0.f, 0.f, 0.f, 0.f);
                if (scale) { const float4 t = reinterpret_cast<const float4*>(scale + b * dim)[idx]; a.x += t.x; a.y += t.y; a.z += t.z; a.w += t.w; }
                else if (add_one == 0.f) { a = make_float4(1.f, 1.f, 1.f, 1.f); }
                if (shift) c = reinterpret_cast<const float4*>(shift + b * dim)[idx];
            };
            fetch(b0);
#pragma unroll
            for (int r = 0; r < R; ++r) {
                if (row0 + r < rows) {
                    if (!one_sample) fetch((row0 + r) / rows_per_batch);
                    const float rstd = rsqrtf(q[r] / (float)dim + eps);
                    const float y0 = (v[r][i].x - mean[r]) * rstd * a.x + c.x;
                    const float y1 = (v[r][i].y - mean[r]) * rstd * a.y + c.y;
                    const float y2 = (v[r][i].z - mean[r]) * rstd * a.z + c.z;
                    const float y3 = (v[r][i].w - mean[r]) * rstd * a.w + c.w;
                    u32x2 o = {pack_bf16x2(y0, y1), pack_bf16x2(y2, y3)};
                    reinterpret_cast<u32x2*>(out + (row0 + r) * (int64_t)dim)[idx] = o;
                }
            }
        }
    }
}

struct RopeDev {
    int F, Hp, Wp, mode, f_src, ground_end, max_pos;
    int ct, ch;
    int64_t token_offset, rows_per_batch;
};

template <int NV>
__global__ __launch_bounds__(kThreads) void rmsnorm_rope_kernel(
    bf16_t* __restrict__ x0, const float* __restrict__ w0, bf16_t* __restrict__ x1,
    const float* __restrict__ w1, int64_t ld, int dim, int head_dim, float eps,
    const float* __restrict__ rope_cos, const float* __restrict__ rope_sin, RopeDev rp, float x0_scale,
    bf16_t* __restrict__ out0, bf16_t* __restrict__ out1, int out_slabs, int out_batch, float x1_scale, int out_fp8, int out_split) {
    __shared__ float red[kWaves];
    __shared__ __attribute__((aligned(16))) float2 cs[128];
    const int64_t row = blockIdx.x;
    bf16_t* xb = blockIdx.y == 0 ? x0 : x1;
    bf16_t* ob = blockIdx.y == 0 ? out0 : out1;
    const float* w = blockIdx.y == 0 ? w0 : w1;
    u32x4* xr = reinterpret_cast<u32x4*>(xb + row * ld);
    const int nchunk = dim >> 3;
    const int half = head_dim >> 1;

    bool rotate = rope_cos != nullptr;
    if (rotate) {
        const int64_t tok = rp.token_offset + (row % rp.rows_per_batch);
        const int64_t hw = (int64_t)rp.Hp * rp.Wp;
        rotate = tok < (int64_t)rp.F * hw;
        if (rotate && threadIdx.x < half) {
            const int f = (int)(tok / hw);
            const int rem = (int)(tok - (int64_t)f * hw);
            const int hh = rem / rp.Wp, ww = rem - hh * rp.Wp;
            int pt = f;
            if (rp.mode == 1) pt = f < rp.f_src ? f : f - rp.f_src;
            else if (rp.mode == 2)
                pt = f < rp.f_src ? f + 1 : (f < rp.ground_end ? 0 : f - rp.ground_end + 1);
            const int p = threadIdx.x;
            int pos = p < rp.ct ? pt : (p < rp.ct + rp.ch ? hh : ww);
            pos = pos < rp.max_pos ? pos : rp.max_pos - 1;
            cs[p] = make_float2(rope_cos[(int64_t)pos * half + p], rope_sin[(int64_t)pos * half + p]);
        }
    }

    u32x4 v[NV];
    float ss = 0.f;
#pragma unroll
    for (int i = 0; i < NV; ++i) {
        const int idx = threadIdx.x + i * kThreads;
        if (idx < nchunk) {
            v[i] = xr[idx];
#pragma unroll
            for (int j = 0; j < 4; ++j) {
                const float a = bf16lo_to_f32(v[i][j]), b = bf16hi_to_f32(v[i][j]);
                ss += a * a + b * b;
            }
        }
    }
    const float rstd = rsqrtf(block_sum<kWaves>(ss, red) / (float)dim + eps)
                       * (blockIdx.y == 0 ? x0_scale : x1_scale);
#pragma unroll
    for (int i = 0; i < NV; ++i) {
        const int idx = threadIdx.x + i * kThreads;
        if (idx < nchunk) {
            const float4 wa = reinterpret_cast<const float4*>(w)[idx * 2];
            const float4 wb = reinterpret_cast<const float4*>(w)[idx * 2 + 1];
            const float wv[8] = {wa.x, wa.y, wa.z, wa.w, wb.x, wb.y, wb.z, wb.w};
            const int p0 = ((idx << 3) % head_dim) >> 1;
            u32x4 o;
#pragma unroll
            for (int j = 0; j < 4; ++j) {
                float a = bf16lo_to_f32(v[i][j]) * rstd * wv[2 * j];
                float b = bf16hi_to_f32(v[i][j]) * rstd * wv[2 * j + 1];
                if (rotate) {
                    const float2 c = cs[p0 + j];
                    const float ra = a * c.x - b * c.y;
                    const float rb = a * c.y + b * c.x;
                    a = ra; b = rb;
                }
                o[j] = pack_bf16x2(a, b);
            }
            if (ob == nullptr) {
                xr[idx] = o;
            } else if (out_fp8) {
                u32x2 q8 = {pack_fp8x4(bf16lo_to_f32(o[0]), bf16hi_to_f32(o[0]), bf16lo_to_f32(o[1]), bf16hi_to_f32(o[1])),
                            pack_fp8x4(bf16lo_to_f32(o[2]), bf16hi_to_f32(o[2]), bf16lo_to_f32(o[3]), bf16hi_to_f32(o[3]))};
                *reinterpret_cast<u32x2*>(reinterpret_cast<unsigned char*>(ob) + row * (int64_t)dim + (idx << 3)) = q8;
            } else {
                const int Cl = dim / out_slabs, c = idx << 3;
                const int slab = c / Cl, cl = c - slab * Cl;
                const int64_t bi = row / rp.rows_per_batch, t = row - bi * rp.rows_per_batch;
                const int64_t cell = ((int64_t)slab * rp.rows_per_batch + t) * out_batch + bi;
                const int64_t at = out_split <= 0 ? cell * Cl + cl
                                 : cl < out_split ? cell * out_split + cl
                                                  : (int64_t)out_slabs * rp.rows_per_batch * out_batch * out_split + cell * (Cl - out_split) + (cl - out_split);
                *reinterpret_cast<u32x4*>(ob + at) = o;
            }
        }
    }
}


template <int NV, int R>
__global__ __launch_bounds__(kThreads) void rmsnorm_rope_rows_kernel(
    bf16_t* __restrict__ x0, const float* __restrict__ w0, bf16_t* __restrict__ x1,
    const float* __restrict__ w1, int64_t ld, int64_t rows, int dim, int head_dim, float eps,
    const float* __restrict__ rope_cos, const float* __restrict__ rope_sin, RopeDev rp, float x0_scale,
    bf16_t* __restrict__ out0, bf16_t* __restrict__ out1, int out_slabs, int out_batch, float x1_scale, int out_fp8, int out_split) {
    __shared__ float red[R][kWaves];
    __shared__ __attribute__((aligned(16))) float2 cs[R][128];
    const int64_t row0 = (int64_t)blockIdx.x * R;
    bf16_t* xb = blockIdx.y == 0 ? x0 : x1;
    bf16_t* ob = blockIdx.y == 0 ? out0 : out1;
    const float* w = blockIdx.y == 0 ? w0 : w1;
    const int nchunk = dim >> 3;
    const int half = head_dim >> 1;

    u32x4 v[R][NV];
#pragma unroll
    for (int r = 0; r < R; ++r) {
        const u32x4* xr = reinterpret_cast<const u32x4*>(xb + (row0 + r) * ld);
        const bool live = row0 + r < rows;
#pragma unroll
        for (int i = 0; i < NV; ++i) {
            const int idx = threadIdx.x + i * kThreads;
            if (live && idx < nchunk) v[r][i] = xr[idx]; else v[r][i] = u32x4{0u, 0u, 0u, 0u};
        }
    }
    bool rotate[R];
    const int64_t hw = (int64_t)rp.Hp * rp.Wp;
#pragma unroll
    for (int r = 0; r < R; ++r)
        rotate[r] = rope_cos != nullptr && rp.token_offset + ((row0 + r) % rp.rows_per_batch) < (int64_t)rp.F * hw;
    if (rope_cos != nullptr) {
        for (int e = threadIdx.x; e < R * half; e += kThreads) {
            const int r = e / half, p = e - r * half;
            const int64_t tok = rp.token_offset + ((row0 + r) % rp.rows_per_batch);
            if (row0 + r < rows && tok < (int64_t)rp.F * hw) {
                const int f = (int)(tok / hw);
                const int rem = (int)(tok - (int64_t)f * hw);
                const int hh = rem / rp.Wp, ww = rem - hh * rp.Wp;
                int pt = f;
                if (rp.mode == 1) pt = f < rp.f_src ? f : f - rp.f_src;
                else if (rp.mode == 2)
                    pt = f < rp.f_src ? f + 1 : (f < rp.ground_end ? 0 : f - rp.ground_end + 1);
                int pos = p < rp.ct ? pt : (p < rp.ct + rp.ch ? hh : ww);
                pos = pos < rp.max_pos ? pos : rp.max_pos - 1;
                cs[r][p] = make_float2(rope_cos[(int64_t)pos * half + p], rope_sin[(int64_t)pos * half + p]);
            }
        }
    }
    float ss[R];
#pragma unroll
    for (int r = 0; r < R; ++r) {
        ss[r] = 0.f;
#pragma unroll
        for (int i = 0; i < NV; ++i) {
            if (threadIdx.x + i * kThreads < nchunk) {
#pragma unroll
                for (int j = 0; j < 4; ++j) {
                    const float a = bf16lo_to_f32(v[r][i][j]), b = bf16hi_to_f32(v[r][i][j]);
                    ss[r] += a * a + b * b;
                }
            }
        }
    }
    block_sum_n<kWaves, R>(ss, red);
    const float post = blockIdx.y == 0 ? x0_scale : x1_scale;
#pragma unroll
    for (int i = 0; i < NV; ++i) {
        const int idx = threadIdx.x + i * kThreads;
        if (idx < nchunk) {
            const float4 wa = reinterpret_cast<const float4*>(w)[idx * 2];
            const float4 wb = reinterpret_cast<const float4*>(w)[idx * 2 + 1];
            const float wv[8] = {wa.x, wa.y, wa.z, wa.w, wb.x, wb.y, wb.z, wb.w};
            const int p0 = ((idx << 3) % head_dim) >> 1;
#pragma unroll
            for (int r = 0; r < R; ++r) {
                const int64_t row = row0 + r;
                if (row >= rows) continue;
                const float rstd = rsqrtf(ss[r] / (float)dim + eps) * post;
                u32x4 o;
#pragma unroll
                for (int j = 0; j < 4; ++j) {
                    float a = bf16lo_to_f32(v[r][i][j]) * rstd * wv[2 * j];
                    float b = bf16hi_to_f32(v[r][i][j]) * rstd * wv[2 * j + 1];
                    if (rotate[r]) {
                        const float2 c = cs[r][p0 + j];
                        const float ra = a * c.x - b * c.y;
                        const float rb = a * c.y + b * c.x;
                        a = ra; b = rb;
                    }
                    o[j] = pack_bf16x2(a, b);
                }
                if (ob == nullptr) {
                    reinterpret_cast<u32x4*>(xb + row * ld)[idx] = o;
                } else if (out_fp8) {
                    u32x2 q8 = {pack_fp8x4(bf16lo_to_f32(o[0]), bf16hi_to_f32(o[0]), bf16lo_to_f32(o[1]), bf16hi_to_f32(o[1])),
                                pack_fp8x4(bf16lo_to_f32(o[2]), bf16hi_to_f32(o[2]), bf16lo_to_f32(o[3]), bf16hi_to_f32(o[3]))};
                    *reinterpret_cast<u32x2*>(reinterpret_cast<unsigned char*>(ob) + row * (int64_t)dim + (idx << 3)) = q8;
                } else {
                    const int Cl = dim / out_slabs, c = idx << 3;
                    const int slab = c / Cl, cl = c - slab * Cl;
                    const int64_t bi = row / rp.rows_per_batch, t = row - bi * rp.rows_per_batch;
                    const int64_t cell = ((int64_t)slab * rp.rows_per_batch + t) * out_batch + bi;
                    const int64_t at = out_split <= 0 ? cell * Cl + cl
                                     : cl < out_split ? cell * out_split + cl
                                                      : (int64_t)out_slabs * rp.rows_per_batch * out_batch * out_split + cell * (Cl - out_split) + (cl - out_split);
                    *reinterpret_cast<u32x4*>(ob + at) = o;
                }
            }
        }
    }
}

}

extern "C" wan_status_t wan_ln_modulate(const float* x, const float* scale, const float* shift, int add_one,
                                        void* out_bf16, int64_t rows, int dim, int64_t rows_per_batch,
                                        float eps, void* stream) {
    WAN_REQUIRE(x && out_bf16, WAN_ERR_INVALID, "wan_ln_modulate: null tensor");
    WAN_REQUIRE(dim > 0 && dim % 4 == 0, WAN_ERR_INVALID, "wan_ln_modulate: dim=%d must be a multiple of 4", dim);
    WAN_REQUIRE(dim <= 8192, WAN_ERR_UNSUPPORTED, "wan_ln_modulate: dim=%d > 8192", dim);
    WAN_REQUIRE(rows >= 0 && rows_per_batch > 0, WAN_ERR_INVALID, "wan_ln_modulate: rows=%lld rows_per_batch=%lld",
                (long long)rows, (long long)rows_per_batch);
    if (rows == 0) return WAN_OK;
    hipStream_t s = (hipStream_t)stream;
    const int nv = (dim / 4 + kThreads - 1) / kThreads;
    dim3 grid((unsigned)rows), block(kThreads);
    bf16_t* out = (bf16_t*)out_bf16;
    const float ao = add_one ? 1.f : 0.f;
    const int R = wan_tune(WAN_TUNE_ROW_GROUP);
    if ((R == 2 || R == 4) && nv <= 6) {
        dim3 ggrid((unsigned)((rows + R - 1) / R));
#define LG_CASE(N) case N: if (R == 4) hipLaunchKernelGGL((ln_modulate_rows_kernel<N, 4>), ggrid, block, 0, s, x, scale, shift, ao, out, dim, rows, rows_per_batch, eps); \
                           else hipLaunchKernelGGL((ln_modulate_rows_kernel<N, 2>), ggrid, block, 0, s, x, scale, shift, ao, out, dim, rows, rows_per_batch, eps); break;
        switch (nv) { LG_CASE(1) LG_CASE(2) LG_CASE(3) LG_CASE(4) LG_CASE(5) LG_CASE(6) }
#undef LG_CASE
        WAN_CHECK_LAUNCH("wan_ln_modulate");
        return WAN_OK;
    }
#define LN_CASE(N) case N: hipLaunchKernelGGL(ln_modulate_kernel<N>, grid, block, 0, s, x, scale, shift, ao, out, dim, rows_per_batch, eps); break;
    switch (nv) { LN_CASE(1) LN_CASE(2) LN_CASE(3) LN_CASE(4) LN_CASE(5) LN_CASE(6) LN_CASE(7) LN_CASE(8) }
#undef LN_CASE
    WAN_CHECK_LAUNCH("wan_ln_modulate");
    return WAN_OK;
}

extern "C" wan_status_t wan_ln_modulate_fp8(const float* x, const float* scale, const float* shift, int add_one,
                                            void* out_fp8, float* out_row_scale, int64_t rows, int dim,
                                            int64_t rows_per_batch, float eps, void* stream) {
    WAN_REQUIRE(x && out_fp8 && out_row_scale, WAN_ERR_INVALID, "wan_ln_modulate_fp8: null tensor");
    WAN_REQUIRE(dim > 0 && dim % 16 == 0, WAN_ERR_INVALID, "wan_ln_modulate_fp8: dim=%d must be a multiple of 16", dim);
    WAN_REQUIRE(dim <= 8192, WAN_ERR_UNSUPPORTED, "wan_ln_modulate_fp8: dim=%d > 8192", dim);
    WAN_REQUIRE(rows >= 0 && rows_per_batch > 0, WAN_ERR_INVALID, "wan_ln_modulate_fp8: rows=%lld rows_per_batch=%lld",
                (long long)rows, (long long)rows_per_batch);
    if (rows == 0) return WAN_OK;
    hipStream_t s = (hipStream_t)stream;
    const int nv = (dim / 4 + kThreads - 1) / kThreads;
    dim3 grid((unsigned)rows), block(kThreads);
    const float ao = add_one ? 1.f : 0.f;
#define LN_CASE(N) case N: hipLaunchKernelGGL((ln_modulate_kernel<N, true>), grid, block, 0, s, x, scale, shift, ao, (bf16_t*)out_fp8, dim, rows_per_batch, eps, out_row_scale); break;
    switch (nv) { LN_CASE(1) LN_CASE(2) LN_CASE(3) LN_CASE(4) LN_CASE(5) LN_CASE(6) LN_CASE(7) LN_CASE(8) }
#undef LN_CASE
    WAN_CHECK_LAUNCH("wan_ln_modulate_fp8");
    return WAN_OK;
}

namespace {
__global__ __launch_bounds__(kThreads) void quantize_rows_fp8_kernel(const bf16_t* __restrict__ x, int64_t ldx,
                                                                     unsigned char* __restrict__ out, int64_t ldo,
                                                                     float* __restrict__ row_scale, int cols) {
    __shared__ float red[kWaves];
    const int64_t row = blockIdx.x;
    const u32x2* xr = reinterpret_cast<const u32x2*>(x + row * ldx);
    const int n4 = cols >> 2;
    float amax = 0.f;
    for (int i = threadIdx.x; i < n4; i += kThreads) {
        const u32x2 w = xr[i];
        amax = fmaxf(fmaxf(amax, fmaxf(fabsf(bf16lo_to_f32(w[0])), fabsf(bf16hi_to_f32(w[0])))),
                     fmaxf(fabsf(bf16lo_to_f32(w[1])), fabsf(bf16hi_to_f32(w[1]))));
    }
    amax = fmaxf(block_max<kWaves>(amax, red), 1e-12f);
    const float inv = 448.0f / amax;
    if (threadIdx.x == 0) row_scale[row] = amax * (1.0f / 448.0f);
    unsigned int* qr = reinterpret_cast<unsigned int*>(out + row * ldo);
    for (int i = threadIdx.x; i < n4; i += kThreads) {
        const u32x2 w = xr[i];
        qr[i] = pack_fp8x4(bf16lo_to_f32(w[0]) * inv, bf16hi_to_f32(w[0]) * inv, bf16lo_to_f32(w[1]) * inv, bf16hi_to_f32(w[1]) * inv);
    }
}
}

extern "C" wan_status_t wan_quantize_rows_fp8(const void* x_bf16, int64_t ldx, void* out_fp8, int64_t ldo,
                                              float* out_row_scale, int64_t rows, int cols, void* stream) {
    WAN_REQUIRE(x_bf16 && out_fp8 && out_row_scale, WAN_ERR_INVALID, "wan_quantize_rows_fp8: null tensor");
    WAN_REQUIRE(cols > 0 && cols % 4 == 0 && ldx >= cols && ldx % 4 == 0 && ldo >= cols && ldo % 4 == 0, WAN_ERR_INVALID,
                "wan_quantize_rows_fp8: cols=%d ldx=%lld ldo=%lld must be multiples of 4 with ld >= cols", cols, (long long)ldx, (long long)ldo);
    WAN_REQUIRE(rows >= 0, WAN_ERR_INVALID, "wan_quantize_rows_fp8: rows=%lld", (long long)rows);
    if (rows == 0) return WAN_OK;
    hipLaunchKernelGGL(quantize_rows_fp8_kernel, dim3((unsigned)rows), dim3(kThreads), 0, (hipStream_t)stream, (const bf16_t*)x_bf16,
                       ldx, (unsigned char*)out_fp8, ldo, out_row_scale, cols);
    WAN_CHECK_LAUNCH("wan_quantize_rows_fp8");
    return WAN_OK;
}

static wan_status_t rmsnorm_rope_impl_ex(void* x0, const float* w0, void* x1, const float* w1,
                                         int64_t ld, int64_t rows, int dim, int head_dim, float eps,
                                         const float* rope_cos, const float* rope_sin, const wan_rope_params* rp,
                                         float x0_scale, void* out0, void* out1, int out_slabs, int out_batch, void* stream,
                                         float x1_scale, int out_fp8, int out_split = 0);

static wan_status_t rmsnorm_rope_impl(void* x0, const float* w0, void* x1, const float* w1,
                                      int64_t ld, int64_t rows, int dim, int head_dim, float eps,
                                      const float* rope_cos, const float* rope_sin, const wan_rope_params* rp,
                                      float x0_scale, void* out0, void* out1, int out_slabs, int out_batch, void* stream) {
    return rmsnorm_rope_impl_ex(x0, w0, x1, w1, ld, rows, dim, head_dim, eps, rope_cos, rope_sin, rp, x0_scale, out0, out1, out_slabs,
                                out_batch, stream, 1.0f, 0);
}

static wan_status_t rmsnorm_rope_impl_ex(void* x0, const float* w0, void* x1, const float* w1,
                                         int64_t ld, int64_t rows, int dim, int head_dim, float eps,
                                         const float* rope_cos, const float* rope_sin, const wan_rope_params* rp,
                                         float x0_scale, void* out0, void* out1, int out_slabs, int out_batch, void* stream,
                                         float x1_scale, int out_fp8, int out_split) {
    WAN_REQUIRE(x0 && w0, WAN_ERR_INVALID, "wan_rmsnorm_rope: null tensor");
    if (out_fp8) {
        WAN_REQUIRE(out0 != nullptr && (out1 != nullptr) == (x1 != nullptr), WAN_ERR_INVALID, "wan_rmsnorm_rope_fp8: one output per input tensor");
        WAN_REQUIRE(x1_scale == x1_scale && x1_scale != 0.f, WAN_ERR_INVALID, "wan_rmsnorm_rope_fp8: x1_scale must be a non-zero number");
    } else if (out0 || out1) {
        WAN_REQUIRE(rp != nullptr && rope_cos != nullptr, WAN_ERR_INVALID, "wan_rmsnorm_rope_sp: needs rope tables and parameters");
        WAN_REQUIRE(out0 != nullptr && (out1 != nullptr) == (x1 != nullptr), WAN_ERR_INVALID, "wan_rmsnorm_rope_sp: one output per input tensor");
        WAN_REQUIRE(out_slabs > 0 && out_batch > 0 && dim % out_slabs == 0 && (dim / out_slabs) % 8 == 0 &&
                        rows == (int64_t)out_batch * rp->rows_per_batch, WAN_ERR_INVALID,
// ... 181 lines not shown
```

videocof_amd/ops.py:

```python
from __future__ import annotations

import ctypes
import functools
import math
from typing import Optional, Tuple

import torch

from . import _lib
from ._lib import RopeParams

EPI_BF16, EPI_GELU_BF16, EPI_F32, EPI_RESID_F32, EPI_BF16_T = (
    _lib.EPI_BF16, _lib.EPI_GELU_BF16, _lib.EPI_F32, _lib.EPI_RESID_F32, _lib.EPI_BF16_T)


def _stream() -> int:
    return torch.cuda.current_stream().cuda_stream


def _on_tensor_device(fn):
    @functools.wraps(fn)
    def wrapper(*args, **kwargs):
        t = next((a for a in args if torch.is_tensor(a)), None)
        if t is None and args and isinstance(args[0], (list, tuple)):
# ... 318 lines not shown
                                       int(rows_per_batch), float(eps), _stream()), "wan_ln_modulate_fp8")
    return out, out_scale


@_on_tensor_device
def quantize_rows_fp8(x: torch.Tensor, out: Optional[torch.Tensor] = None,
                      out_scale: Optional[torch.Tensor] = None) -> Tuple[torch.Tensor, torch.Tensor]:
    _need(x, torch.bfloat16, "quantize_rows_fp8.x")
    if x.dim() != 2:
        raise ValueError("quantize_rows_fp8.x must be 2-D")
    rows, cols = x.shape
    if out is None:
        out = torch.empty(rows, cols, device=x.device, dtype=FP8)
    if out_scale is None:
        out_scale = torch.empty(rows, device=x.device, dtype=torch.float32)
    _need(out, FP8, "quantize_rows_fp8.out")
    _need(out_scale, torch.float32, "quantize_rows_fp8.out_scale")
    lib = _lib.load()
    _lib.check(lib.wan_quantize_rows_fp8(_p(x), x.stride(0), _p(out), out.stride(0), _p(out_scale), rows, cols, _stream()),
               "wan_quantize_rows_fp8")
    return out, out_scale


def quantize_weight_fp8(w: torch.Tensor) -> Tuple[torch.Tensor, torch.Tensor]:
    wf = w.float()
    s = wf.abs().amax(dim=1).clamp_min(1e-12) / FP8_MAX
    return (wf / s[:, None]).clamp(-FP8_MAX, FP8_MAX).to(FP8).contiguous(), s.contiguous()


@_on_tensor_device
def gemm_fp8(a: torch.Tensor, a_scale: torch.Tensor, w: torch.Tensor, w_scale: torch.Tensor, bias: Optional[torch.Tensor],
             epilogue: int, out: Optional[torch.Tensor] = None, gate: Optional[torch.Tensor] = None,
             rows_per_batch: int = 0, ldo_t: int = 0) -> torch.Tensor:
    _need(a, FP8, "gemm_fp8.a")
    _need(w, FP8, "gemm_fp8.w")
    _need(a_scale, torch.float32, "gemm_fp8.a_scale")
    _need(w_scale, torch.float32, "gemm_fp8.w_scale")
    M, K = a.shape
    N, Kw = w.shape
    if K != Kw or a_scale.numel() < M or w_scale.numel() != N:
        raise ValueError(f"gemm_fp8: a is [{M},{K}], w is [{N},{Kw}], scales {a_scale.numel()} / {w_scale.numel()}")
    if bias is not None:
        _need(bias, torch.float32, "gemm_fp8.bias")
        if bias.numel() != N:
            raise ValueError("gemm_fp8: bias length != N")
    dev = a.device
    if epilogue in (EPI_BF16, EPI_GELU_BF16):
        if out is None:
            out = torch.empty(M, N, device=dev, dtype=torch.bfloat16)
        _need(out, torch.bfloat16, "gemm_fp8.out")
    elif epilogue == EPI_F32:
        if out is None:
            out = torch.empty(M, N, device=dev, dtype=torch.float32)
        _need(out, torch.float32, "gemm_fp8.out")
    elif epilogue == EPI_RESID_F32:
        if out is None:
            raise ValueError("gemm_fp8: EPI_RESID_F32 needs the residual stream as `out`")
        _need(out, torch.float32, "gemm_fp8.out")
        if gate is not None:
            _need(gate, torch.float32, "gemm_fp8.gate")
    elif epilogue == EPI_BF16_T:
        if out is None:
            out = torch.zeros(N, ldo_t or round_up(M, 64), device=dev, dtype=torch.bfloat16)
        _need(out, torch.bfloat16, "gemm_fp8.out")
        if out.shape[0] != N or out.shape[1] < M:
            raise ValueError(f"gemm_fp8: transposed out must be [N={N}, >= M={M}], got {tuple(out.shape)}")
    else:
        raise ValueError(f"gemm_fp8: unknown epilogue {epilogue}")
    if epilogue != EPI_BF16_T and tuple(out.shape) != (M, N):
        raise ValueError(f"gemm_fp8: out shape {tuple(out.shape)} != ({M},{N})")
    lib = _lib.load()
    ws = gemm_workspace(dev, M, N, K, fp8=True)
    _lib.check(lib.wan_gemm_fp8_ws(_p(a), a.stride(0), _p(a_scale), _p(w), w.stride(0), _p(w_scale), _p(bias), _p(out),
                                   out.stride(0), M, N, K, epilogue, _p(gate), int(rows_per_batch), _p(ws),
                                   ws.numel() if ws is not None else 0, _stream()), "wan_gemm_fp8_ws")
    return out


_ATTN_WS = {}


@_on_tensor_device
def attention_fwd(q: torch.Tensor, k: torch.Tensor, vt: torch.Tensor, num_heads: int, k_len: Optional[int] = None,
                  softmax_scale: Optional[float] = None, out: Optional[torch.Tensor] = None,
                  q_prescaled: bool = False, workspace: Optional[AttentionWorkspace] = None,
                  k_lens: Optional[torch.Tensor] = None) -> torch.Tensor:
    for nm, t in (("q", q), ("k", k), ("vt", vt)):
        _need(t, torch.bfloat16, "attention." + nm)
        if t.dim() != 3:
            raise ValueError(f"attention.{nm} must be 3-D [B, rows, cols]")
    B, Lq, C = q.shape
    Lk = k.shape[1] if k_len is None else int(k_len)
    if Lk > k.shape[1] or Lk <= 0:
        raise ValueError(f"attention: k_len={Lk} outside (0, {k.shape[1]}]")
    head_dim = C // num_heads
    if out is None:
        out = torch.empty(B, Lq, C, device=q.device, dtype=torch.bfloat16)
    _need(out, torch.bfloat16, "attention.out")
    if vt.shape[1] != C or k.shape[2] != C or k.shape[0] != B or vt.shape[0] != B:
        raise ValueError("attention: q/k/vt shapes disagree")
    scale = softmax_scale if softmax_scale is not None else 1.0 / math.sqrt(head_dim)
    lib = _lib.load()
    ws, ws_bytes = None, int(lib.wan_attention_workspace_bytes(B, Lq, Lk, num_heads, head_dim))
    if ws_bytes > 0:
        if workspace is None:
            key = (q.device, _stream())
            workspace = _ATTN_WS.get(key)
            if workspace is None:
                workspace = _ATTN_WS[key] = AttentionWorkspace()
        ws = workspace.get(q.device, ws_bytes)
    if k_lens is not None:
        _need(k_lens, torch.int32, "attention.k_lens")
        if k_lens.shape != (B,) or not k_lens.is_contiguous():
            raise ValueError(f"attention.k_lens must be a contiguous int32 [{B}]")
        _lib.check(lib.wan_attention_fwd_varlen(_p(q), q.stride(1), q.stride(0), _p(k), k.stride(1), k.stride(0),
                                                _p(vt), vt.stride(1), vt.stride(0), _p(out), out.stride(1), out.stride(0),
                                                B, Lq, Lk, _p(k_lens), num_heads, head_dim, float(scale),
                                                _lib.ATTN_Q_PRESCALED if q_prescaled else 0, _p(ws),
                                                ws_bytes if ws is not None else 0, _stream()), "wan_attention_fwd_varlen")
        return out
    _lib.check(lib.wan_attention_fwd(_p(q), q.stride(1), q.stride(0), _p(k), k.stride(1), k.stride(0),
                                     _p(vt), vt.stride(1), vt.stride(0), _p(out), out.stride(1), out.stride(0),
                                     B, Lq, Lk, num_heads, head_dim, float(scale),
                                     _lib.ATTN_Q_PRESCALED if q_prescaled else 0, _p(ws), ws_bytes if ws is not None else 0,
                                     _stream()), "wan_attention_fwd")
    return out


def cross_fold_plan(rows: int, num_heads: int, text_len: int, kept: int, weights_bf16: bool = True) -> bool:
    return bool(_lib.load().wan_cross_fold_plan(int(rows), int(num_heads), int(text_len), int(kept), int(bool(weights_bf16))))


@_on_tensor_device
def cross_probs(q: torch.Tensor, k: torch.Tensor, num_heads: int, kept: int, pad_count: int,
                out: Optional[torch.Tensor] = None) -> torch.Tensor:
    _need(q, torch.bfloat16, "cross_probs.q")
    _need(k, torch.bfloat16, "cross_probs.k")
    B, L, C = q.shape
    if k.dim() != 3 or k.shape[0] != B or k.shape[2] != C or C != num_heads * 128 or k.shape[1] < kept + 1:
        raise ValueError(f"cross_probs: q {tuple(q.shape)} / k {tuple(k.shape)} / heads {num_heads} / kept {kept} disagree")
    if B > 1 and q.stride(0) != L * q.stride(1):
        raise ValueError("cross_probs: the samples of q must follow each other without a gap")
    if out is None:
        out = torch.empty(B * L, num_heads * 64, device=q.device, dtype=torch.bfloat16)
    _need(out, torch.bfloat16, "cross_probs.out")
    if tuple(out.shape) != (B * L, num_heads * 64):
        raise ValueError(f"cross_probs: out shape {tuple(out.shape)} != ({B * L},{num_heads * 64})")
    _lib.check(_lib.load().wan_cross_probs(_p(q), q.stride(1), _p(k), k.stride(1), k.stride(0), _p(out), out.stride(0), B, L,
                                           int(num_heads), int(kept), int(pad_count), _stream()), "wan_cross_probs")
    return out


@_on_tensor_device
def cross_fold_values(w_co: torch.Tensor, vt: torch.Tensor, num_heads: int, kept: int,
                      out: Optional[torch.Tensor] = None) -> torch.Tensor:
    _need(w_co, torch.bfloat16, "cross_fold_values.w_co")
    _need(vt, torch.bfloat16, "cross_fold_values.vt")
    B, C, T = vt.shape
    if tuple(w_co.shape) != (C, C) or C != num_heads * 128:
        raise ValueError(f"cross_fold_values: w_co {tuple(w_co.shape)} / vt {tuple(vt.shape)} / heads {num_heads} disagree")
    if out is None:
        out = torch.empty(B, C, num_heads * 64, device=vt.device, dtype=torch.bfloat16)
    _need(out, torch.bfloat16, "cross_fold_values.out")
    if tuple(out.shape) != (B, C, num_heads * 64):
        raise ValueError(f"cross_fold_values: out shape {tuple(out.shape)} != ({B},{C},{num_heads * 64})")
    _lib.check(_lib.load().wan_cross_fold_values(_p(w_co), w_co.stride(0), _p(vt), vt.stride(1), vt.stride(0), _p(out), out.stride(1),
                                                 out.stride(0), B, C, int(num_heads), int(kept), _stream()), "wan_cross_fold_values")
    return out


@_on_tensor_device
def rmsnorm_rope_fp8(x0: torch.Tensor, w0: torch.Tensor, x1: Optional[torch.Tensor], w1: Optional[torch.Tensor], head_dim: int,
                     eps: float, rope: Optional[Tuple[torch.Tensor, torch.Tensor]], rope_params: Optional[RopeParams],
                     out0: torch.Tensor, out1: Optional[torch.Tensor], x0_scale: float = 1.0, x1_scale: float = 1.0) -> None:
    _need(x0, torch.bfloat16, "rmsnorm_rope_fp8.x0")
    _need(w0, torch.float32, "rmsnorm_rope_fp8.w0")
    rows, dim = x0.shape
    ld = x0.stride(0)
    for nm, t in (("out0", out0), ("out1", out1)):
        if t is not None:
            _need(t, FP8, "rmsnorm_rope_fp8." + nm)
            if not t.is_contiguous() or t.numel() < rows * dim:
                raise ValueError(f"rmsnorm_rope_fp8.{nm} must be contiguous with >= rows * dim bytes")
    if x1 is not None:
        _need(x1, torch.bfloat16, "rmsnorm_rope_fp8.x1")
        _need(w1, torch.float32, "rmsnorm_rope_fp8.w1")
        if x1.shape != x0.shape or x1.stride(0) != ld or out1 is None:
            raise ValueError("rmsnorm_rope_fp8: x0 / x1 must share shape and row stride, and x1 needs out1")
    cos = sin = None
    if rope is not None:
        cos, sin = rope
        if rope_params is None:
            raise ValueError("rmsnorm_rope_fp8: rope tables given without rope_params")
    lib = _lib.load()
    _lib.check(lib.wan_rmsnorm_rope_fp8(_p(x0), _p(w0), _p(x1), _p(w1), ld, rows, dim, head_dim, float(eps), _p(cos), _p(sin),
                                        ctypes.byref(rope_params) if rope_params is not None else None, float(x0_scale),
                                        float(x1_scale), _p(out0), _p(out1), _stream()), "wan_rmsnorm_rope_fp8")


@_on_tensor_device
def vt_quantize_mx(vt: torch.Tensor, num_heads: int, k_len: int, v8: Optional[torch.Tensor] = None,
                   scales: Optional[torch.Tensor] = None) -> Tuple[torch.Tensor, torch.Tensor]:
    _need(vt, torch.bfloat16, "vt_quantize_mx.vt")
    if vt.dim() != 3:
        raise ValueError("vt_quantize_mx.vt must be [B, H*128, ldvt]")
    B, C, ld = vt.shape
    lib = _lib.load()
    nsc = int(lib.wan_vt_mx_scale_bytes(B, num_heads, int(k_len)))
    if v8 is None:
        v8 = torch.empty(B, C, ld, device=vt.device, dtype=FP8)
    if scales is None:
        scales = torch.empty(nsc, device=vt.device, dtype=torch.uint8)
    _need(v8, FP8, "vt_quantize_mx.v8")
    _need(scales, torch.uint8, "vt_quantize_mx.scales")
    if v8.shape != vt.shape or scales.numel() < nsc or not scales.is_contiguous():
        raise ValueError("vt_quantize_mx: v8 must have vt's shape and scales wan_vt_mx_scale_bytes() contiguous bytes")
    _lib.check(lib.wan_vt_quantize_mx(_p(vt), vt.stride(1), vt.stride(0), B, int(num_heads), int(k_len), _p(v8), v8.stride(1), v8.stride(0),
                                      _p(scales), _stream()), "wan_vt_quantize_mx")
    return v8, scales


@_on_tensor_device
def attention_fwd_f8(q8: torch.Tensor, k8: torch.Tensor, v8: torch.Tensor, v8_scales: torch.Tensor, vt: torch.Tensor, num_heads: int,
                     q_exp: int, k_exp: int, k_len: Optional[int] = None, out: Optional[torch.Tensor] = None,
                     workspace: Optional[AttentionWorkspace] = None) -> torch.Tensor:
    for nm, t, dt in (("q8", q8, FP8), ("k8", k8, FP8), ("v8", v8, FP8), ("vt", vt, torch.bfloat16)):
        _need(t, dt, "attention_f8." + nm)
        if t.dim() != 3:
            raise ValueError(f"attention_f8.{nm} must be 3-D [B, rows, cols]")
    _need(v8_scales, torch.uint8, "attention_f8.v8_scales")
    B, Lq, C = q8.shape
    Lk = k8.shape[1] if k_len is None else int(k_len)
    if Lk > k8.shape[1] or Lk <= 0:
        raise ValueError(f"attention_f8: k_len={Lk} outside (0, {k8.shape[1]}]")
    head_dim = C // num_heads
    if out is None:
        out = torch.empty(B, Lq, C, device=q8.device, dtype=torch.bfloat16)
    _need(out, torch.bfloat16, "attention_f8.out")
    if vt.shape[1] != C or v8.shape != vt.shape or k8.shape[2] != C or k8.shape[0] != B or vt.shape[0] != B:
        raise ValueError("attention_f8: q8/k8/v8/vt shapes disagree")
    lib = _lib.load()
    ws_bytes = max(int(lib.wan_attention_workspace_bytes(B, Lq, Lk, num_heads, head_dim)), 16)
    if workspace is None:
        key = (q8.device, _stream())
        workspace = _ATTN_WS.get(key)
        if workspace is None:
            workspace = _ATTN_WS[key] = AttentionWorkspace()
    ws = workspace.get(q8.device, ws_bytes)
    _lib.check(lib.wan_attention_fwd_f8(_p(q8), q8.stride(1), q8.stride(0), int(q_exp), _p(k8), k8.stride(1), k8.stride(0), int(k_exp),
                                        _p(v8), v8.stride(1), v8.stride(0), _p(v8_scales), _p(vt), vt.stride(1), vt.stride(0),
                                        _p(out), out.stride(1), out.stride(0), B, Lq, Lk, num_heads, head_dim, _p(ws), ws_bytes, _stream()),
               "wan_attention_fwd_f8")
    return out


@_on_tensor_device
def col_mean(x: torch.Tensor, rows_per_batch: int, valid_rows: int, batch: int, out: Optional[torch.Tensor] = None,
             workspace: Optional[torch.Tensor] = None) -> torch.Tensor:
    _need(x, torch.bfloat16, "col_mean.x")
    dim = x.shape[1]
    lib = _lib.load()
    need = int(lib.wan_col_mean_workspace_bytes(batch, dim)) // 4
    if workspace is None:
        workspace = torch.empty(need, device=x.device, dtype=torch.float32)
    _need(workspace, torch.float32, "col_mean.workspace")
    if workspace.numel() < need or not workspace.is_contiguous():
        raise ValueError(f"col_mean.workspace needs {need} contiguous fp32 elements")
    if out is None:
        out = torch.empty(batch, dim, device=x.device, dtype=torch.float32)
    _need(out, torch.float32, "col_mean.out")
    _lib.check(lib.wan_col_mean_bf16(_p(x), x.stride(0), int(rows_per_batch), int(valid_rows), int(batch), dim, _p(workspace), _p(out),
                                     _stream()), "wan_col_mean_bf16")
    return out


@_on_tensor_device
def qk_quantize_fp8(q: Optional[torch.Tensor], k: Optional[torch.Tensor], rows_per_batch: int, k_mean: Optional[torch.Tensor],
                    q_scale: float, k_scale: float, q8: Optional[torch.Tensor], k8: Optional[torch.Tensor]) -> None:
    if (q is None) != (q8 is None) or (k is None) != (k8 is None) or (q is None and k is None):
        raise ValueError("qk_quantize_fp8: q comes with q8, k with k8, and at least one pair is needed")
    if k is None and k_mean is not None:
        raise ValueError("qk_quantize_fp8: k_mean without k")
    ref = q if q is not None else k
    for nm, t in (("q", q), ("k", k)):
        if t is not None:
            _need(t, torch.bfloat16, "qk_quantize_fp8." + nm)
            if t.dim() != 2 or t.shape != ref.shape or t.stride(0) != ref.stride(0):
                raise ValueError("qk_quantize_fp8: q and k must be 2-D and share shape and row stride")
    rows, dim = ref.shape
    for nm, t in (("q8", q8), ("k8", k8)):
        if t is None:
            continue
        _need(t, FP8, "qk_quantize_fp8." + nm)
        if not t.is_contiguous() or t.numel() < rows * dim:
            raise ValueError(f"qk_quantize_fp8.{nm} must be contiguous with >= rows * dim bytes")
    if k_mean is not None:
        _need(k_mean, torch.float32, "qk_quantize_fp8.k_mean")
        if not k_mean.is_contiguous() or k_mean.shape[-1] != dim:
            raise ValueError("qk_quantize_fp8.k_mean must be contiguous [batch, dim]")
    lib = _lib.load()
    _lib.check(lib.wan_qk_quantize_fp8(_p(q), _p(k), ref.stride(0), rows, dim, int(rows_per_batch), _p(k_mean), float(q_scale),
                                       float(k_scale), _p(q8), _p(k8), _stream()), "wan_qk_quantize_fp8")


@_on_tensor_device
def attention_fwd_qk8(q8: torch.Tensor, k8: torch.Tensor, vt: torch.Tensor, num_heads: int, q_exp: int, k_exp: int,
# ... 652 lines not shown
```

videocof_amd/wan_transformer3d.py:

```python
from __future__ import annotations

import ctypes
import glob
import json
import math
import os
from collections import namedtuple
from types import SimpleNamespace
from typing import Dict, List, Optional, Sequence, Tuple

import torch
import torch.nn as nn

from . import ops
from ._lib import BlockWeights, BlockWorkspace, DitWeights, DitWorkspace, RopeParams, check, load
from .dist import get_sp_group

__all__ = ["WanTransformer3DModel", "sinusoidal_embedding_1d", "rope_params"]


def sinusoidal_embedding_1d(dim: int, position: torch.Tensor) -> torch.Tensor:
    if dim % 2:
        raise AssertionError("dim must be even")
    half = dim // 2
    pos = position.to(torch.float64)
    inv = torch.exp(-math.log(10000.0) * torch.arange(half, dtype=torch.float64, device=pos.device) / half)
    ang = torch.outer(pos, inv)
    return torch.cat([ang.cos(), ang.sin()], dim=1)


def rope_params(max_seq_len: int, dim: int, theta: float = 10000.0) -> torch.Tensor:
    inv = 1.0 / torch.pow(torch.tensor(theta, dtype=torch.float64),
                          torch.arange(0, dim, 2, dtype=torch.float64) / dim)
    ang = torch.outer(torch.arange(max_seq_len, dtype=torch.float64), inv)
    return torch.polar(torch.ones_like(ang), ang)


IncompatibleKeys = namedtuple("IncompatibleKeys", ["missing_keys", "unexpected_keys"])


class StateDictShapeError(ValueError, RuntimeError):
    """A checkpoint tensor whose shape does not fit the configured model.  ValueError for callers that validate inputs,
    RuntimeError because that is what ``nn.Module.load_state_dict`` raises for "size mismatch for <key>"."""


def ulysses_head_padding(num_heads: int, degree: int, head_dim: int):
    Hl = (num_heads + degree - 1) // degree
    Hp, Cp = Hl * degree, Hl * degree * head_dim
    cp = torch.arange(Cp)
    r, sl, j = cp // (Hl * head_dim), (cp % (Hl * head_dim)) // head_dim, cp % head_dim
    hreal = sl * degree + r
    valid = hreal < num_heads
    src = torch.where(valid, hreal * head_dim + j, torch.zeros_like(cp))
    return Hp, Cp, src, valid


class _Block:
    __slots__ = ("w_qk", "b_qk", "w_v", "b_v", "w_o", "b_o", "nq", "nk",
                 "w_cq", "b_cq", "w_ck", "b_ck", "w_cv", "b_cv", "w_co", "b_co", "ncq", "nck",
                 "n3w", "n3b", "w1", "b1", "w2", "b2", "modulation", "f8", "_cw", "spw")


_LINEARS = {"qk": ("w_qk", "b_qk"), "v": ("w_v", "b_v"), "o": ("w_o", "b_o"), "cq": ("w_cq", "b_cq"), "co": ("w_co", "b_co"),
            "w1": ("w1", "b1"), "w2": ("w2", "b2")}
_SPW_LINEARS = {("qk", 0): ("w_q", "b_q"), ("qk", 1): ("w_k", "b_k"), ("v", None): ("w_v", "b_v"), ("o", None): ("w_o", None)}
_ROW_QUANT = {"o": ("attq", "atts"), "co": ("attq", "atts"), "w2": ("ffq", "ffs")}


def _e4m3_exponent(amax: float) -> int:
    return int(max(-8, min(8, math.floor(math.log2(448.0 / max(amax, 1e-30))) - 1)))


def cfg_skip_active(batch: int, cfg_skip_ratio, current_steps, num_inference_steps) -> bool:
    return bool(batch >= 2 and cfg_skip_ratio is not None and current_steps >= num_inference_steps * (1 - cfg_skip_ratio))


def cfg_skip_half(arg, half: int):
    import numpy as np
    return arg[half:] if isinstance(arg, (torch.Tensor, list, tuple, np.ndarray)) else arg


class WanTransformer3DModel(nn.Module):
    def __init__(self, model_type="t2v", patch_size=(1, 2, 2), text_len=512, in_dim=16, dim=2048,
                 ffn_dim=8192, freq_dim=256, text_dim=4096, out_dim=16, num_heads=16, num_layers=32,
                 window_size=(-1, -1), qk_norm=True, cross_attn_norm=True, eps=1e-6, in_channels=16,
                 hidden_size=2048, add_control_adapter=False, in_dim_control_adapter=24,
                 downscale_factor_control_adapter=8, add_ref_conv=False, in_dim_ref_conv=16,
                 cross_attn_type=None):
        super().__init__()
        if model_type != "t2v" or cross_attn_type not in (None, "t2v_cross_attn"):
            raise NotImplementedError("only the t2v cross-attention variant is on the VideoCoF path")
        if add_control_adapter or add_ref_conv:
            raise NotImplementedError("control adapter / ref conv belong to other model families")
        if not (qk_norm and cross_attn_norm) or tuple(window_size) != (-1, -1):
            raise NotImplementedError("Wan2.1 T2V uses qk_norm, cross_attn_norm and global attention")
        if dim % num_heads or dim // num_heads != 128:
            raise NotImplementedError(f"head_dim {dim / num_heads} (the gfx950 attention kernel is built for 128)")
        self.config = SimpleNamespace(
            model_type=model_type, patch_size=tuple(patch_size), text_len=text_len, in_dim=in_dim, dim=dim,
            ffn_dim=ffn_dim, freq_dim=freq_dim, text_dim=text_dim, out_dim=out_dim, num_heads=num_heads,
            num_layers=num_layers, window_size=tuple(window_size), qk_norm=qk_norm,
            cross_attn_norm=cross_attn_norm, eps=eps,
            in_channels=in_channels, hidden_size=hidden_size, add_control_adapter=add_control_adapter,
            in_dim_control_adapter=in_dim_control_adapter, downscale_factor_control_adapter=downscale_factor_control_adapter,
            add_ref_conv=add_ref_conv, in_dim_ref_conv=in_dim_ref_conv, cross_attn_type=cross_attn_type)
        self.model_type, self.patch_size, self.text_len = model_type, tuple(patch_size), text_len
        self.in_dim, self.dim, self.ffn_dim, self.freq_dim = in_dim, dim, ffn_dim, freq_dim
        self.text_dim, self.out_dim, self.num_heads, self.num_layers = text_dim, out_dim, num_heads, num_layers
        self.eps = eps
        self.d = dim // num_heads
        self._qs = ops.q_prescale(self.d)
        d = self.d
        self.freqs = torch.cat([rope_params(1024, d - 4 * (d // 6)), rope_params(1024, 2 * (d // 6)),
                                rope_params(1024, 2 * (d // 6))], dim=1)
        self._rope_dev: Optional[Tuple[torch.Tensor, torch.Tensor]] = None
        self.blocks: List[_Block] = []
        self._w: Dict[str, torch.Tensor] = {}
        self._dtype = torch.bfloat16
        self._device = torch.device("cpu")
        self.teacache = None
        self.should_calc = True
        self.cfg_skip_ratio = None
        self.current_steps = 0
        self.num_inference_steps = None
        self._cfg_skip_suspended = False
        self._bufs_used = None
        self.sp_world_size = 1
        self.sp_world_rank = 0
        self._sp = None
        self.force_ulysses = False
        self.sp_head_groups = 2
        self._sp_pad = None
        self._usp = False
        self._comm_events = None
        self.cache_context = False
        self._text_kept = text_len
        self.last_cross_fold = False
        self._ctx_cache = None
        self._fp8 = ()
        self.fp8_attn_exponents = (5, 2)
        self.fp8_attn_calibrate = True
        self.fp8_attn_smooth_k = True
        self.use_block_composite = True
        self.use_forward_composite = True
        self._cdw = None
        self._bufs = {}
        self._bufs_last = None
        self._graph_epoch = 0
        self.skip_source_frames = 0
        self.mask_source_frames = 0
        self._ws_self, self._ws_cross = ops.AttentionWorkspace(), ops.AttentionWorkspace()
        self._ws_self_sfx, self._ws_cross_sfx = ops.AttentionWorkspace(), ops.AttentionWorkspace()
        self._probe_layer = None
        self._probe = None
        self._attn_events = None
        self._last_attn_rows = 0
        self._last_attn_variant = 0

    @property
    def dtype(self):
        return self._dtype

    @property
    def device(self):
        return self._device

    def expected_shapes(self) -> Dict[str, Tuple[int, ...]]:
        C, F, T = self.dim, self.ffn_dim, self.text_dim
        pt, ph, pw = self.patch_size
        sh = {"patch_embedding.weight": (C, self.in_dim, pt, ph, pw), "patch_embedding.bias": (C,),
              "text_embedding.0.weight": (C, T), "text_embedding.0.bias": (C,),
              "text_embedding.2.weight": (C, C), "text_embedding.2.bias": (C,),
              "time_embedding.0.weight": (C, self.freq_dim), "time_embedding.0.bias": (C,),
              "time_embedding.2.weight": (C, C), "time_embedding.2.bias": (C,),
              "time_projection.1.weight": (6 * C, C), "time_projection.1.bias": (6 * C,),
              "head.head.weight": (self.out_dim * pt * ph * pw, C), "head.head.bias": (self.out_dim * pt * ph * pw,),
              "head.modulation": (1, 2, C)}
        for i in range(self.num_layers):
            p = f"blocks.{i}."
            sh[p + "modulation"] = (1, 6, C)
            for a in ("self_attn", "cross_attn"):
                for l in ("q", "k", "v", "o"):
                    sh[f"{p}{a}.{l}.weight"], sh[f"{p}{a}.{l}.bias"] = (C, C), (C,)
                sh[f"{p}{a}.norm_q.weight"] = sh[f"{p}{a}.norm_k.weight"] = (C,)
            sh[p + "norm3.weight"] = sh[p + "norm3.bias"] = (C,)
            sh[p + "ffn.0.weight"], sh[p + "ffn.0.bias"] = (F, C), (F,)
            sh[p + "ffn.2.weight"], sh[p + "ffn.2.bias"] = (C, F), (C,)
        return sh

    def _fresh_value(self, key: str, shape: Tuple[int, ...], gen: torch.Generator) -> torch.Tensor:
        if key.endswith("modulation"):
            return torch.randn(shape, generator=gen) / self.dim ** 0.5
        if key.endswith(".bias") or key == "head.head.weight":
            return torch.zeros(shape)
        if "norm" in key:
            return torch.ones(shape)
        if key.startswith(("text_embedding", "time_embedding")):
            return torch.randn(shape, generator=gen) * 0.02
        fan_out, fan_in = shape[0], int(math.prod(shape[1:]))
        bound = math.sqrt(6.0 / (fan_in + fan_out))
        return (torch.rand(shape, generator=gen) * 2 - 1) * bound

    def load_state_dict(self, state_dict, strict: bool = True, device=None):
        sd = state_dict
        expect = self.expected_shapes()
        bad = [(k, tuple(v.shape), expect[k]) for k, v in sd.items() if k in expect and tuple(v.shape) != expect[k]]
        if bad:
            k, got, want = bad[0]
            raise StateDictShapeError(f"size mismatch for {k}: checkpoint tensor is {list(got)}, the model "
                                      f"(dim={self.dim}, ffn_dim={self.ffn_dim}, in_dim={self.in_dim}, text_dim={self.text_dim}) "
                                      f"expects {list(want)}" + (f" (+{len(bad) - 1} more)" if len(bad) > 1 else ""))
        missing = [k for k in expect if k not in sd]
        if strict and missing:
            raise KeyError(f"missing key in state_dict: {missing[0]}" + (f" (+{len(missing) - 1} more)" if len(missing) > 1 else ""))
        if strict and any(k not in expect for k in sd):
            extra = [k for k in sd if k not in expect]
            raise KeyError(f"unexpected keys in state_dict: {extra[:5]}{'...' if len(extra) > 5 else ''}")
        dev = torch.device(device) if device is not None else torch.device("cuda", torch.cuda.current_device())
        if dev.type != "cuda":
            raise RuntimeError("WanTransformer3DModel runs on a HIP device only (no CPU fallback)")
        if missing:
            if getattr(self, "_w", None):
                current = self.state_dict()
                sd = {**{k: current[k] for k in missing}, **sd}
            else:
                gen = torch.Generator().manual_seed(0)
                sd = {**{k: self._fresh_value(k, expect[k], gen) for k in missing}, **sd}
        used = set()

        def get(k):
            if k not in sd:
                raise KeyError(f"missing key in state_dict: {k}")
            used.add(k)
            return sd[k]

        def mat(k):
            return get(k).detach().to(device=dev, dtype=torch.bfloat16).contiguous()

        def vec(k):
            return get(k).detach().to(device=dev, dtype=torch.float32).contiguous()

        def bvec(k):
            return get(k).detach().to(device=dev, dtype=torch.bfloat16).to(torch.float32).contiguous()

        C = self.dim
        w = self._w = {}
        w["pe_w"] = get("patch_embedding.weight").detach().reshape(C, -1).to(device=dev, dtype=torch.bfloat16).contiguous()
        w["pe_b"] = vec("patch_embedding.bias")
        for i in ("0", "2"):
            w[f"te_w{i}"] = mat(f"text_embedding.{i}.weight")
            w[f"te_b{i}"] = vec(f"text_embedding.{i}.bias")
            w[f"tm_w{i}"] = mat(f"time_embedding.{i}.weight").to(torch.float32)
            w[f"tm_b{i}"] = bvec(f"time_embedding.{i}.bias")
        w["tp_w"] = mat("time_projection.1.weight").to(torch.float32)
        w["tp_b"] = bvec("time_projection.1.bias")
        w["head_w"] = mat("head.head.weight")
        w["head_b"] = vec("head.head.bias")
        w["head_mod"] = vec("head.modulation").reshape(2, C)
        self.blocks = []
        for i in range(self.num_layers):
            p = f"blocks.{i}."
            b = _Block()
            b.w_qk = torch.cat([mat(p + "self_attn.q.weight"), mat(p + "self_attn.k.weight")], dim=0).contiguous()
            b.b_qk = torch.cat([vec(p + "self_attn.q.bias"), vec(p + "self_attn.k.bias")]).contiguous()
            b.w_v, b.b_v = mat(p + "self_attn.v.weight"), vec(p + "self_attn.v.bias")
            b.w_o, b.b_o = mat(p + "self_attn.o.weight"), vec(p + "self_attn.o.bias")
            b.nq, b.nk = vec(p + "self_attn.norm_q.weight"), vec(p + "self_attn.norm_k.weight")
            b.w_cq, b.b_cq = mat(p + "cross_attn.q.weight"), vec(p + "cross_attn.q.bias")
            b.w_ck, b.b_ck = mat(p + "cross_attn.k.weight"), vec(p + "cross_attn.k.bias")
            b.w_cv, b.b_cv = mat(p + "cross_attn.v.weight"), vec(p + "cross_attn.v.bias")
            b.w_co, b.b_co = mat(p + "cross_attn.o.weight"), vec(p + "cross_attn.o.bias")
            b.ncq, b.nck = vec(p + "cross_attn.norm_q.weight"), vec(p + "cross_attn.norm_k.weight")
            b.n3w, b.n3b = vec(p + "norm3.weight"), vec(p + "norm3.bias")
            b.w1, b.b1 = mat(p + "ffn.0.weight"), vec(p + "ffn.0.bias")
            b.w2, b.b2 = mat(p + "ffn.2.weight"), vec(p + "ffn.2.bias")
            b.modulation = vec(p + "modulation").reshape(6, C)
            b.f8 = None
            b._cw = None
            b.spw = None
            self.blocks.append(b)
        w["mod_all"] = torch.stack([b.modulation for b in self.blocks])
        self._cdw = None
        extra = [k for k in sd.keys() if k not in used]
        ang = torch.view_as_real(self.freqs)
        self._rope_dev = (ang[..., 0].to(torch.float32).contiguous().to(dev),
                          ang[..., 1].to(torch.float32).contiguous().to(dev))
        self._device = dev
        self._ctx_cache = None
        self._graph_epoch += 1
        self._reset_attention_scratch()
# ... 123 lines not shown
        m, u = model.load_state_dict(kept, strict=False)
        print(f"### missing keys: {len(m)}; \n### unexpected keys: {len(u)};")
        print(m)
        n_all = sum(int(math.prod(s_)) for s_ in expect.values())
        n_attn = sum(int(math.prod(s_)) for k_, s_ in expect.items() if "self_attn." in k_)
        print(f"### All Parameters: {n_all / 1e6} M")
        print(f"### self-attention Parameters: {n_attn / 1e6} M")
        return model

    def enable_multi_gpus_inference(self):
        sp = get_sp_group()
        if sp is None:
            raise RuntimeError("sequence-parallel group is not initialised (videocof_amd.dist.set_multi_gpus_devices)")
        self._sp, self.sp_world_size, self.sp_world_rank = sp, sp.world_size, sp.rank
        self._sp_pad = None
        if self.num_heads % sp.world_size:
            self._pad_heads_for_ulysses(sp.world_size)

    def _pad_heads_for_ulysses(self, P: int):
        if self._fp8:
            raise NotImplementedError("fp8 projections with padded heads under sequence parallelism")
        H, C, d, dev = self.num_heads, self.dim, self.d, self._device
        Hp, Cp, src, valid = ulysses_head_padding(H, P, d)
        src, valid = src.to(dev), valid.to(dev)
        gain = math.sqrt(C / Cp)

        def rows(w):
            out = w.index_select(0, src)
            out[~valid] = 0
            return out.contiguous()
        for blk in self.blocks:
            spw = SimpleNamespace()
            spw.w_q, spw.b_q = rows(blk.w_qk[:C]), rows(blk.b_qk[:C])
            spw.w_k, spw.b_k = rows(blk.w_qk[C:]), rows(blk.b_qk[C:])
            spw.w_v, spw.b_v = rows(blk.w_v), rows(blk.b_v)
            spw.nq, spw.nk = rows(blk.nq) * gain, rows(blk.nk) * gain
            spw.w_o = rows(blk.w_o.t().contiguous()).t().contiguous()
            blk.spw = spw
        self._sp_pad = SimpleNamespace(H=Hp, C=Cp, eps=self.eps * C / Cp, pad_heads=Hp - H)
        self._bufs, self._bufs_last = {}, None

    def enable_fp8_linear(self, layers=("qkv", "ffn"), attn_smooth_k: bool = True):
        if getattr(self, "_sp_pad", None) is not None:
            raise NotImplementedError("fp8 projections with padded heads under sequence parallelism (num_heads % ulysses degree != 0)")
        layers = tuple(layers)
        if not set(layers) <= {"qkv", "ffn", "o", "cross", "attn", "attn_pv"} or not layers:
            raise ValueError(f"enable_fp8_linear: layers must be drawn from ('qkv', 'ffn', 'o', 'cross', 'attn', 'attn_pv'), got {layers}")
        if "attn_pv" in layers and "attn" not in layers:
            raise ValueError("enable_fp8_linear: 'attn_pv' (fp8 P.V) extends 'attn' (fp8 QK^T): name both")
        if "attn" in layers and self.d != 128:
            raise NotImplementedError("the fp8 QK^T attention kernel is built for head_dim 128")
        if self.dim % 128 or self.ffn_dim % 128:
            raise NotImplementedError("fp8 projections need dim and ffn_dim to be multiples of 128")
        self.fp8_attn_smooth_k = bool(attn_smooth_k)
        for blk in self.blocks:
            blk.f8 = {}
            if "qkv" in layers:
                blk.f8["qk"], blk.f8["v"] = ops.quantize_weight_fp8(blk.w_qk), ops.quantize_weight_fp8(blk.w_v)
            if "ffn" in layers:
                blk.f8["w1"], blk.f8["w2"] = ops.quantize_weight_fp8(blk.w1), ops.quantize_weight_fp8(blk.w2)
            if "o" in layers:
                blk.f8["o"], blk.f8["co"] = ops.quantize_weight_fp8(blk.w_o), ops.quantize_weight_fp8(blk.w_co)
            if "cross" in layers:
                blk.f8["cq"] = ops.quantize_weight_fp8(blk.w_cq)
            if "attn" in layers:
                blk.f8["attn"] = True
            if "attn_pv" in layers:
                blk.f8["attn_pv"] = True
        self._fp8 = layers
        self._bufs, self._bufs_last = {}, None
        self._graph_epoch += 1
        self._reset_attention_scratch()

    def disable_fp8_linear(self):
        for blk in self.blocks:
            blk.f8 = None
        self._fp8 = ()
        self._bufs, self._bufs_last = {}, None
        self._graph_epoch += 1
        self._reset_attention_scratch()

    def _reset_attention_scratch(self):
        for ws in (self._ws_self, self._ws_cross, self._ws_self_sfx, self._ws_cross_sfx):
            ws.reset()

    def clear_context_cache(self):
        self._ctx_cache = None

    def enable_teacache(self, coefficients, num_steps: int, rel_l1_thresh: float, num_skip_start_steps: int = 0,
                        offload: bool = True):
        from .cache_utils import TeaCache
        self.teacache = TeaCache(coefficients, num_steps, rel_l1_thresh=rel_l1_thresh,
                                 num_skip_start_steps=num_skip_start_steps, offload=offload)

    def share_teacache(self, transformer=None):
        self.teacache = transformer.teacache

    def disable_teacache(self):
        self.teacache = None

    def enable_cfg_skip(self, cfg_skip_ratio, num_steps):
        if not 0 <= cfg_skip_ratio <= 1:
            raise ValueError(f"enable_cfg_skip: cfg_skip_ratio={cfg_skip_ratio} is a share of the steps, in [0, 1]")
        if cfg_skip_ratio != 0:
            self.cfg_skip_ratio, self.current_steps, self.num_inference_steps = cfg_skip_ratio, 0, num_steps
        else:
            self.cfg_skip_ratio, self.current_steps, self.num_inference_steps = None, 0, None

    def disable_cfg_skip(self):
        self.cfg_skip_ratio, self.current_steps, self.num_inference_steps = None, 0, None

    def cfg_skip_now(self, batch: int) -> bool:
        return not self._cfg_skip_suspended and cfg_skip_active(batch, self.cfg_skip_ratio, self.current_steps,
                                                                self.num_inference_steps)

    def share_cfg_skip(self, transformer=None):
        self.cfg_skip_ratio = transformer.cfg_skip_ratio
        self.current_steps = transformer.current_steps
        self.num_inference_steps = transformer.num_inference_steps

    def enable_riflex(self, k=6, L_test=66, L_test_scale=4.886):
        raise NotImplementedError("RIFLEx temporal frequencies are not built (SURVEY.md section 2: out of scope; no CLI of this path enables them)")

    def disable_riflex(self):
        return None

    def unpatchify(self, x, grid_sizes):
        grids = grid_sizes.tolist() if torch.is_tensor(grid_sizes) else [tuple(g) for g in grid_sizes]
        out = []
        for u, v in zip(x, grids):
            o = ops.unpatchify(u.float().contiguous(), tuple(int(i) for i in v), tuple(self.patch_size), self.out_dim,
                               torch.float32 if u.dtype == torch.float32 else torch.bfloat16)
            out.append(o if o.dtype == u.dtype else o.to(u.dtype))
        return out

    def _time_embed(self, t: torch.Tensor):
        w = self._w
        s = sinusoidal_embedding_1d(self.freq_dim, t.to(self._device)).float()
        e = torch.addmm(w["tm_b2"], torch.nn.functional.silu(torch.addmm(w["tm_b0"], s, w["tm_w0"].t())), w["tm_w2"].t())
        e0 = torch.addmm(w["tp_b"], torch.nn.functional.silu(e), w["tp_w"].t()).unflatten(1, (6, self.dim))
        return e, e0

    def _text_embed(self, context: Sequence[torch.Tensor]) -> torch.Tensor:
        w = self._w
        B = len(context)
        ctx = torch.zeros(B * self.text_len, self.text_dim, device=self._device, dtype=torch.bfloat16)
        for b, u in enumerate(context):
            if u.shape[0] > self.text_len or u.shape[1] != self.text_dim:
                raise ValueError(f"context[{b}] has shape {tuple(u.shape)}; expected [<= {self.text_len}, {self.text_dim}]")
            ctx[b * self.text_len: b * self.text_len + u.shape[0]] = u.to(device=self._device, dtype=torch.bfloat16)
        hid = ops.gemm(ctx, w["te_w0"], w["te_b0"], ops.EPI_GELU_BF16)
        return ops.gemm(hid, w["te_w2"], w["te_b2"], ops.EPI_BF16)

    def _context_kv(self, blk: _Block, ctx: torch.Tensor, B: int, out=None):
        C, T = self.dim, self.text_len
        ck, cvt = out if out is not None else (None, None)
        ck = ops.gemm(ctx, blk.w_ck, blk.b_ck, ops.EPI_BF16, out=None if ck is None else ck.view(B * T, C))
        ops.rmsnorm_rope_(ck, blk.nck, None, None, self.d, self.eps)
        if cvt is None:
            cvt = torch.empty(B, C, T, device=self._device, dtype=torch.bfloat16)
        for b in range(B):
            ops.gemm(ctx[b * T:(b + 1) * T], blk.w_cv, blk.b_cv, ops.EPI_BF16_T, out=cvt[b])
        return ck.view(B, T, C), cvt

    def _hoisted_context(self, context, B, into=None):
        vers = tuple(u._version for u in context)
        if self._ctx_cache is not None:
            held, v0, kv = self._ctx_cache[:3]
            if (len(held) == len(context) and all(a is b for a, b in zip(held, context)) and v0 == vers
                    and (into is None or kv is into)):
                return kv
            n = len(context)
            if (0 < n < len(held) and all(a is b for a, b in zip(held[-n:], context)) and v0[-n:] == vers):
                tails = self._ctx_cache[3]
                if n not in tails:
                    tails[n] = [(ck[-n:], cvt[-n:]) for ck, cvt in kv]
                if into is None or into is tails[n] or into[0][0].data_ptr() == tails[n][0][0].data_ptr():
                    return tails[n] if into is None else into
        old = into
        if old is None and self._ctx_cache is not None and self._ctx_cache[2][0][0].shape[0] == B:
            old = self._ctx_cache[2]
        self._ctx_cache = None
        ctx = self._text_embed(context)
        kv = [self._context_kv(blk, ctx, B, out=None if old is None else old[i]) for i, blk in enumerate(self.blocks)]
        self._ctx_cache = (list(context), vers, kv, {})
        return kv

    def _event_pair(self):
        if self._attn_events is None:
            return None
        a, b = torch.cuda.Event(enable_timing=True), torch.cuda.Event(enable_timing=True)
        a.record()
        return a, b

    def _event_done(self, ev, rows):
        if ev is not None:
            ev[1].record()
            self._attn_events.append(ev)
            self._last_attn_rows = rows
            self._last_attn_variant = ops.get_tuning("last_attn_variant")

    def _comm_pair(self, tag):
        if self._comm_events is None:
            return None
        a, b = torch.cuda.Event(enable_timing=True), torch.cuda.Event(enable_timing=True)
        a.record()
        return tag, a, b

    def _comm_done(self, ev):
        if ev is not None:
            ev[2].record()
            self._comm_events.append(ev)

    def _rope_map(self, grid, frame_split_indices, ground_frame_indices, token_offset, rows):
        mode, f_src, g_end = 0, 0, 0
        if frame_split_indices is not None and len(frame_split_indices) > 0:
            if len(set(frame_split_indices)) != 1:
                raise NotImplementedError("all samples of a call must share frame_split_indices")
            f_src, mode = int(frame_split_indices[0]), 1
            if ground_frame_indices is not None and len(ground_frame_indices) > 0:
                if len(set(tuple(g) for g in ground_frame_indices)) != 1:
                    raise NotImplementedError("all samples of a call must share ground_frame_indices")
                g0, g1 = ground_frame_indices[0]
                if int(g0) != f_src:
                    raise ValueError("ground frames must start at frame_split_indices (pipeline_wan.py:716-718)")
                mode, g_end = 2, int(g1)
        return RopeParams(grid[0], grid[1], grid[2], mode, f_src, g_end, token_offset, rows, self.freqs.shape[0])

    def _workspaces(self, B, Ll, L, seq_len):
        Ca = self._sp_pad.C if (self._usp and self._sp_pad is not None) else self.dim
        key = (B, Ll, L, seq_len, self.sp_world_size, self._usp, str(self._device), tuple(self._fp8), Ca)
        b = self._bufs.get(key)
        if b is not None:
            self._bufs_last = key
            if self._bufs_used is not None:
                self._bufs_used.append(b)
            return b
        keep_b = self.cfg_skip_ratio is not None
        for k in [k for k, v in self._bufs.items() if not getattr(v, "pinned", False) and not (keep_b and k[1:] == key[1:])]:
            del self._bufs[k]
        C, dev, M = self.dim, self._device, B * Ll
        b = SimpleNamespace()
        b.h = torch.empty(M, C, device=dev, dtype=torch.bfloat16)
        b.qk = torch.empty(M, 2 * C, device=dev, dtype=torch.bfloat16)
        b.att = torch.empty(M, C, device=dev, dtype=torch.bfloat16)
        b.cq = torch.empty(M, C, device=dev, dtype=torch.bfloat16)
        b.ff = torch.empty(M, self.ffn_dim, device=dev, dtype=torch.bfloat16)
        P = self.sp_world_size
        if not self._usp:
            b.vt = torch.zeros(B, C, ops.round_up(L, 64), device=dev, dtype=torch.bfloat16)
        else:
            b.vt = None
            for name in ("kw_s", "kw_r", "qw_s", "qw_r", "vw_s", "vw_r", "ow_s", "ow_r"):
                setattr(b, name, torch.empty(M * Ca, device=dev, dtype=torch.bfloat16))
            b.vt_full = torch.zeros(B, Ca // P, ops.round_up(seq_len, 64), device=dev, dtype=torch.bfloat16)
            if Ca != C:
                b.qk_a = torch.empty(M, 2 * Ca, device=dev, dtype=torch.bfloat16)
                b.att_a = torch.empty(M, Ca, device=dev, dtype=torch.bfloat16)
        b.qk3 = b.qk.view(B, Ll, 2 * C)
        if self._fp8:
            b.hq = torch.empty(M, C, device=dev, dtype=ops.FP8)
            b.rs = torch.empty(M, device=dev, dtype=torch.float32)
            if "ffn" in self._fp8:
                b.ffq = torch.empty(M, self.ffn_dim, device=dev, dtype=ops.FP8)
                b.ffs = torch.empty(M, device=dev, dtype=torch.float32)
            if "o" in self._fp8:
                b.attq = torch.empty(M, C, device=dev, dtype=ops.FP8)
                b.atts = torch.empty(M, device=dev, dtype=torch.float32)
            if "attn" in self._fp8:
                b.q8 = torch.empty(M, C, device=dev, dtype=ops.FP8)
                b.k8 = torch.empty(M, C, device=dev, dtype=ops.FP8)
                b.kmean = torch.empty(B, C, device=dev, dtype=torch.float32)
                b.kmean_ws = torch.empty(int(load().wan_col_mean_workspace_bytes(B, C)) // 4, device=dev, dtype=torch.float32)
                if "attn_pv" in self._fp8:
                    b.v8 = torch.empty_like(b.vt_full if self._usp else b.vt, dtype=ops.FP8)
                    b.v8s = torch.empty(int(load().wan_vt_mx_scale_bytes(B, self.num_heads // (P if self._usp else 1), L)), device=dev,
                                        dtype=torch.uint8)
        b.pinned = False
        self._bufs[key] = b
        self._bufs_last = key
        if self._bufs_used is not None:
            self._bufs_used.append(b)
        return b

    def release_workspaces(self, keep_pinned: bool = False):
        if keep_pinned:
            for k in [k for k, v in self._bufs.items() if not getattr(v, "pinned", False)]:
                del self._bufs[k]
        else:
            self._bufs = {}
            self._graph_epoch += 1
        self._bufs_last = None
        self._ctx_cache = None
        ops.release_gemm_workspaces(include_capture=False)

    def _linear(self, blk: _Block, key, a, epilogue, out, half=None, spw=None, **kw):
        wn, bn = _LINEARS[key]
        w, bias = getattr(blk, wn), getattr(blk, bn)
        if spw is not None and (key, half) in _SPW_LINEARS:
            wn, bn = _SPW_LINEARS[key, half]
            w, bias, half = getattr(spw, wn), (getattr(spw, bn) if bn else bias), None
        rows = None if half is None else slice(half * self.dim, (half + 1) * self.dim)
        if isinstance(a, tuple):
            w8, ws8 = blk.f8[key]
            if rows is not None:
                w8, ws8, bias = w8[rows], ws8[rows], bias[rows]
            return ops.gemm_fp8(a[0], a[1], w8, ws8, bias, epilogue, out=out, **kw)
        if rows is not None:
            w, bias = w[rows], bias[rows]
        return ops.gemm(a, w, bias, epilogue, out=out, **kw)

    @staticmethod
    def _rows(a, lo, hi):
        return (a[0][lo:hi], a[1][lo:hi]) if isinstance(a, tuple) else a[lo:hi]

    def _ln_operand(self, blk: _Block, key, x, scale, shift, add_one, rows, bufs, h=None, bf16=False):
# ... 2 lines not shown
            return bufs.hq, bufs.rs
        h = bufs.h if h is None else h
        ops.ln_modulate(x, scale, shift, add_one, rows, self.eps, out=h)
        return h

    def _row_operand(self, blk: _Block, key, a, bufs, bf16=False):
        if not bf16 and blk.f8 and key in blk.f8:
            q, s = (getattr(bufs, name) for name in _ROW_QUANT[key])
            ops.quantize_rows_fp8(a, out=q, out_scale=s)
            return q, s
        return a

    def _o_projection(self, blk: _Block, em, x, att, bufs, n, spw=None, bf16=False):
        self._linear(blk, "o", self._row_operand(blk, "o", att, bufs, bf16), ops.EPI_RESID_F32, x, spw=spw, gate=em[2], rows_per_batch=n)

    def _norm_rope(self, blk: _Block, bufs, rp, B, Ll, L):
        C, f8 = self.dim, blk.f8 or {}
        q, k = bufs.qk[:, :C], bufs.qk[:, C:]
        qe, ke = f8.get("attn_exp") or self.fp8_attn_exponents
        if "attn" in f8 and not self.fp8_attn_smooth_k:
            ops.rmsnorm_rope_fp8(q, blk.nq, k, blk.nk, self.d, self.eps, self._rope_dev, rp, bufs.q8, bufs.k8,
                                 x0_scale=self._qs * 2.0 ** qe, x1_scale=2.0 ** ke)
            return qe, ke
        ops.rmsnorm_rope_(q, blk.nq, k, blk.nk, self.d, self.eps, self._rope_dev, rp, x0_scale=self._qs)
        if "attn" in f8:
            ops.col_mean(k, Ll, L, B, out=bufs.kmean, workspace=bufs.kmean_ws)
            qe, ke = self._calibrate(f8, q, k, bufs.kmean, B, Ll, L)
            ops.qk_quantize_fp8(q, k, Ll, bufs.kmean, 2.0 ** qe, 2.0 ** ke, bufs.q8, bufs.k8)
        return qe, ke

    def _calibrate(self, f8, q_bf16, k_bf16, mean, B, rows_per_batch, L):
        if self.fp8_attn_calibrate and "attn_exp" not in f8 and not torch.cuda.is_current_stream_capturing():
            kc = k_bf16.float().view(B, rows_per_batch, -1)[:, :L] - mean[:, None, :].float()
            aq, ak = float(q_bf16.float().view(B, rows_per_batch, -1)[:, :L].abs().max()), float(kc.abs().max())
            f8["attn_exp"] = (_e4m3_exponent(aq), _e4m3_exponent(ak))
        return f8.get("attn_exp") or self.fp8_attn_exponents

    def _self_attention(self, blk: _Block, em, xs, bufs, rp, B, Ll, L):
        C, H, f8 = self.dim, self.num_heads, blk.f8 or {}
        vt, att = bufs.vt, bufs.att.view(B, Ll, C)
        a = self._ln_operand(blk, "qk", xs, em[1], em[0], True, Ll, bufs)
        self._linear(blk, "qk", a, ops.EPI_BF16, bufs.qk)
        qe, ke = self._norm_rope(blk, bufs, rp, B, Ll, L)
        for b in range(B):
            self._linear(blk, "v", self._rows(a, b * Ll, b * Ll + L), ops.EPI_BF16_T, vt[b])
        ev = self._event_pair()
        if "attn_pv" in f8:
            ops.vt_quantize_mx(vt, H, L, v8=bufs.v8, scales=bufs.v8s)
            ops.attention_fwd_f8(bufs.q8.view(B, Ll, C), bufs.k8.view(B, Ll, C), bufs.v8, bufs.v8s, vt, H, qe, ke, k_len=L, out=att,
                                 workspace=self._ws_self)
        elif "attn" in f8:
            ops.attention_fwd_qk8(bufs.q8.view(B, Ll, C), bufs.k8.view(B, Ll, C), vt, H, qe, ke, k_len=L, out=att, workspace=self._ws_self)
        else:
            ops.attention_fwd(bufs.qk3[:, :, :C], bufs.qk3[:, :, C:], vt, H, k_len=L, out=att, q_prescaled=True, workspace=self._ws_self)
        self._event_done(ev, B * Ll)
        return bufs.att

    def _self_attention_ulysses(self, blk: _Block, em, xs, bufs, rp, B, Ll, L, seq_len):
        P, sp, f8, pad = self.sp_world_size, self._sp, blk.f8 or {}, self._sp_pad
        spw = blk.spw if pad is not None else None
        Ca, Ha, eps_a = (pad.C, pad.H, pad.eps) if pad is not None else (self.dim, self.num_heads, self.eps)
        nq_a, nk_a, qk_a, att_a = (spw.nq, spw.nk, bufs.qk_a, bufs.att_a) if pad is not None else (blk.nq, blk.nk, bufs.qk, bufs.att)
        Cl, Lt = Ca // P, P * Ll
        a = self._ln_operand(blk, "qk", xs, em[1], em[0], True, Ll, bufs)
        self._linear(blk, "qk", a, ops.EPI_BF16, qk_a[:, Ca:], half=1, spw=spw)
        ops.rmsnorm_rope_sp(qk_a[:, Ca:], nk_a, None, None, self.d, eps_a, self._rope_dev, rp, bufs.kw_s, None, P, B)
        wait_k = sp.exchange(bufs.kw_r, bufs.kw_s, async_op=True)
        vsend = bufs.vw_s.view(Ca, B, Ll)
        for b in range(B):
            self._linear(blk, "v", self._rows(a, b * Ll, (b + 1) * Ll), ops.EPI_BF16_T, vsend[:, b], spw=spw)
        wait_v = sp.exchange(bufs.vw_r, bufs.vw_s, async_op=True)
        self._linear(blk, "qk", a, ops.EPI_BF16, qk_a[:, :Ca], half=0, spw=spw)
        Hl = Ha // P
        h0 = Hl // 2 if (self.sp_head_groups >= 2 and Hl >= 2) else 0
        split = h0 * self.d
        ops.rmsnorm_rope_sp(qk_a[:, :Ca], nq_a, None, None, self.d, eps_a, self._rope_dev, rp, bufs.qw_s, None, P, B,
                            x0_scale=self._qs, split=split)
        groups = [(c0, cg, hg, slice(Lt * B * c0, Lt * B * (c0 + cg)))
                  for c0, cg, hg in ([(0, split, h0), (split, Cl - split, Hl - h0)] if h0 else [(0, Cl, Hl)])]
        q_waits = [sp.exchange(bufs.qw_r[cut], bufs.qw_s[cut], async_op=True) for _, _, _, cut in groups]
        cev = self._comm_pair("q_g0")
        wait_k()
        wait_v()
        ops.sp_unpack_vt(bufs.vw_r, bufs.vt_full, P, Ll)
        k_all = bufs.kw_r.view(Lt, B, Cl).permute(1, 0, 2)
        fp8 = self._ulysses_fp8_k(f8, bufs, groups, q_waits, B, Cl, Lt, L) if "attn" in f8 else None
        wait_o = []
        ev = self._event_pair()
        for gi, (c0, cg, hg, cut) in enumerate(groups):
            q_waits[gi]()
            if gi == 0:
                self._comm_done(cev)
            o_g = bufs.ow_s[cut].view(Lt, B, cg).permute(1, 0, 2)
            if fp8 is not None:
                self._ulysses_fp8_attention(f8, bufs, groups[gi], fp8, o_g, B, Lt, L)
            else:
                ops.attention_fwd(bufs.qw_r[cut].view(Lt, B, cg).permute(1, 0, 2), k_all[..., c0:c0 + cg], bufs.vt_full[:, c0:c0 + cg], hg,
                                  k_len=L, out=o_g, q_prescaled=True, workspace=self._ws_self)
            if gi + 1 < len(groups):
                wait_o.append(sp.exchange(bufs.ow_r[cut], bufs.ow_s[cut], async_op=True))
        self._event_done(ev, B * seq_len)
        cev = self._comm_pair("o_g1")
        sp.exchange(bufs.ow_r[cut], bufs.ow_s[cut])
        for w_ in wait_o:
            w_()
        self._comm_done(cev)
        ops.sp_unpack_heads(bufs.ow_r, att_a, P, Ll, B, split=split)
        return att_a, spw

    def _ulysses_fp8_k(self, f8, bufs, groups, q_waits, B, Cl, Lt, L):
        k2d = bufs.kw_r.view(Lt, B * Cl)
        mean = (ops.col_mean(k2d, Lt, L, 1, out=bufs.kmean.view(-1)[:B * Cl].view(1, B * Cl), workspace=bufs.kmean_ws)
                if self.fp8_attn_smooth_k else None)
        if self.fp8_attn_calibrate and not f8.get("attn_exp_agreed"):
            if torch.cuda.is_current_stream_capturing():
                raise RuntimeError("fp8 attention under sequence parallelism calibrates its exponents on the first EAGER forward "
                                   "(one all-reduce per layer); run one before capturing a graph")
            for w_ in q_waits:
                w_()
            kc = k2d[:L].float() if mean is None else k2d[:L].float() - mean.float()
            q_amax = torch.stack([bufs.qw_r[cut.start:cut.start + L * B * cg].float().abs().max() for (_, cg, _, cut) in groups]).max()
            amax = torch.stack([q_amax, kc.abs().max()])
            if self.sp_world_size > 1:
                amax = self._sp.all_reduce_max(amax)
            aq, ak = (float(v) for v in amax.tolist())
            if "attn_exp" not in f8:
                f8["attn_exp"] = (_e4m3_exponent(aq), _e4m3_exponent(ak))
            f8["attn_exp_agreed"] = True
        qe, ke = f8.get("attn_exp") or self.fp8_attn_exponents
        k8w = bufs.k8.view(-1)[:Lt * B * Cl]
        ops.qk_quantize_fp8(None, k2d, Lt, mean, 1.0, 2.0 ** ke, None, k8w)
        return qe, ke, k8w.view(Lt, B, Cl).permute(1, 0, 2), int(load().wan_vt_mx_scale_bytes(1, 1, L)) if "attn_pv" in f8 else 0

    def _ulysses_fp8_attention(self, f8, bufs, group, fp8, o_g, B, Lt, L):
        (c0, cg, hg, cut), (qe, ke, k8_all, hs) = group, fp8
        q8g = bufs.q8.view(-1)[cut]
        ops.qk_quantize_fp8(bufs.qw_r[cut].view(Lt, B * cg), None, Lt, None, 2.0 ** qe, 1.0, q8g, None)
        q8v = q8g.view(Lt, B, cg).permute(1, 0, 2)
        vt_g = bufs.vt_full[:, c0:c0 + cg]
        if "attn_pv" in f8:
            v8g, s8g = bufs.v8[:, c0:c0 + cg], bufs.v8s[B * (c0 // self.d) * hs:B * (c0 // self.d + hg) * hs]
            ops.vt_quantize_mx(vt_g, hg, L, v8=v8g, scales=s8g)
            ops.attention_fwd_f8(q8v, k8_all[..., c0:c0 + cg], v8g, s8g, vt_g, hg, qe, ke, k_len=L, out=o_g, workspace=self._ws_self)
        else:
            ops.attention_fwd_qk8(q8v, k8_all[..., c0:c0 + cg], vt_g, hg, qe, ke, k_len=L, out=o_g, workspace=self._ws_self)

    def _block_tail(self, blk: _Block, em, xs, bufs, ctx_kv, B, n, ws_cross, r0=0, bf16=False):
        C = self.dim
        x, h, cq, att, ff = xs, bufs.h, bufs.cq, bufs.att, bufs.ff
        if r0:
            x, h, cq, att, ff = x[r0:], h[r0:], cq[r0:], att[r0:], ff[r0:]
        a = self._ln_operand(blk, "cq", x, blk.n3w, blk.n3b, False, B * n, bufs, h, bf16)
        self._linear(blk, "cq", a, ops.EPI_BF16, cq)
        ops.rmsnorm_rope_(cq, blk.ncq, None, None, self.d, self.eps, x0_scale=self._qs)
        H, kept = self.num_heads, self._text_kept
        self.last_cross_fold = bool(load().wan_cross_fold_plan(B * n, H, self.text_len, kept, int(bf16 or not (blk.f8 and "co" in blk.f8))))
        if self.last_cross_fold:
            probs = att.reshape(-1)[:B * n * H * 64].view(B * n, H * 64)
            ops.cross_probs(cq.view(B, n, C), ctx_kv[0], H, kept, self.text_len - kept, out=probs)
            vfold = self._vfold(bufs, B)
            ops.cross_fold_values(blk.w_co, ctx_kv[1], H, kept, out=vfold)
            for b in range(B):
                ops.gemm(probs[b * n:(b + 1) * n], vfold[b], blk.b_co, ops.EPI_RESID_F32, out=x[b * n:(b + 1) * n])
        else:
            ops.attention_fwd(cq.view(B, n, C), *ctx_kv, self.num_heads, out=att.view(B, n, C), q_prescaled=True, workspace=ws_cross)
            self._linear(blk, "co", self._row_operand(blk, "co", att, bufs, bf16), ops.EPI_RESID_F32, x)
        a = self._ln_operand(blk, "w1", x, em[4], em[3], True, n, bufs, h, bf16)
        self._linear(blk, "w1", a, ops.EPI_GELU_BF16, ff)
        self._linear(blk, "w2", self._row_operand(blk, "w2", ff, bufs, bf16), ops.EPI_RESID_F32, x, gate=em[5], rows_per_batch=n)

    def _vfold(self, bufs, B):
        if getattr(bufs, "vfold", None) is None:
            bufs.vfold = torch.empty(B, self.dim, self.num_heads * 64, device=self._device, dtype=torch.bfloat16)
        return bufs.vfold

    def _run_block(self, blk: _Block, em, xs, bufs, ctx_kv, rp, B, Ll, L, seq_len):
        composite = not blk.f8 and self._attn_events is None and self.use_block_composite
        if composite and not self._usp:
            self._block_composite(blk, em, xs, bufs, ctx_kv, rp, B, Ll, L)
            return
        e = em.unbind(0)
        if self._usp:
            att, spw = self._self_attention_ulysses(blk, e, xs, bufs, rp, B, Ll, L, seq_len)
        else:
            att, spw = self._self_attention(blk, e, xs, bufs, rp, B, Ll, L), None
        self._o_projection(blk, e, xs, att, bufs, Ll, spw)
        if composite:
            self._block_composite(blk, em, xs, bufs, ctx_kv, None, B, Ll, L)
            return
        self._block_tail(blk, e, xs, bufs, ctx_kv, B, Ll, self._ws_cross)

    def _last_block_suffix(self, blk: _Block, em, xs, bufs, ctx_kv, rp, r0, L):
        C, Ll, em = self.dim, xs.shape[0], em.unbind(0)
        qk, att, n = bufs.qk, bufs.att, Ll - r0
        h = self._ln_operand(blk, "qk", xs, em[1], em[0], True, Ll, bufs, bf16=True)
        self._linear(blk, "qk", h, ops.EPI_BF16, qk[:, C:], half=1)
        self._linear(blk, "qk", h[r0:], ops.EPI_BF16, qk[r0:, :C], half=0)
        ops.rmsnorm_rope_(qk[:r0, C:], blk.nk, None, None, self.d, self.eps, self._rope_dev, rp)
        rp2 = RopeParams(rp.F, rp.Hp, rp.Wp, rp.mode, rp.f_src, rp.ground_end, r0, n, rp.max_pos)
        ops.rmsnorm_rope_(qk[r0:, :C], blk.nq, qk[r0:, C:], blk.nk, self.d, self.eps, self._rope_dev, rp2, x0_scale=self._qs)
        self._linear(blk, "v", h[:L], ops.EPI_BF16_T, bufs.vt[0])
        ops.attention_fwd(qk[r0:, :C].unsqueeze(0), qk[:, C:].unsqueeze(0), bufs.vt, self.num_heads, k_len=L, out=att[r0:].unsqueeze(0),
                          q_prescaled=True, workspace=self._ws_self_sfx)
        self._o_projection(blk, em, xs[r0:], att[r0:], bufs, n, bf16=True)
        self._block_tail(blk, em, xs, bufs, ctx_kv, 1, n, self._ws_cross_sfx, r0=r0, bf16=True)

    def _block_cw(self, blk: _Block):
        if getattr(blk, "_cw", None) is None:
            p = lambda t: ctypes.c_void_p(t.data_ptr())
            blk._cw = BlockWeights(self.dim, self.ffn_dim, self.num_heads, self.text_len, float(self.eps),
                                   p(blk.w_qk), p(blk.w_v), p(blk.w_o), p(blk.w_cq), p(blk.w_co), p(blk.w1), p(blk.w2),
                                   p(blk.b_qk), p(blk.b_v), p(blk.b_o), p(blk.b_cq), p(blk.b_co), p(blk.b1), p(blk.b2),
                                   p(blk.nq), p(blk.nk), p(blk.ncq), p(blk.n3w), p(blk.n3b))
        return blk._cw

    def _block_cws(self, bufs, holder, B, Ll, L):
        if getattr(holder, "cws", None) is None:
            lib = load()
            p = lambda t: ctypes.c_void_p(t.data_ptr())
            H = self.num_heads
            bufs.nself = int(lib.wan_attention_workspace_bytes(B, Ll, L, H, 128))
            bufs.ncross = int(lib.wan_attention_workspace_bytes(B, Ll, self.text_len, H, 128))
            vt = getattr(bufs, "vt", None)
            holder.cws = BlockWorkspace(p(bufs.h), p(bufs.qk), p(bufs.att), p(bufs.cq), p(bufs.ff), p(vt) if vt is not None else None,
                                        vt.stride(1) if vt is not None else 0, None, bufs.nself, None, bufs.ncross, None, 0)
        fold = bool(load().wan_cross_fold_plan(B * Ll, self.num_heads, self.text_len, self._text_kept, 1))
        holder.cws.text_kept = self._text_kept
        holder.cws.vfold = self._vfold(bufs, B).data_ptr() if fold else None
        holder.cws.vfold_bytes = bufs.vfold.numel() * 2 if fold else 0
        holder.cws.attn_ws_self = self._ws_self.get(self._device, max(bufs.nself, 16)).data_ptr()
        holder.cws.attn_ws_cross = self._ws_cross.get(self._device, max(bufs.ncross, 16)).data_ptr()
        M = B * Ll
        gws = None
        for (m_, n_, k_) in ((M, 2 * self.dim, self.dim), (M, self.ffn_dim, self.dim), (M, self.dim, self.ffn_dim), (M, self.dim, self.dim),
                             (L, self.dim, self.dim)) + (((Ll, self.dim, self.num_heads * 64),) if fold else ()):
            t = ops.gemm_workspace(self._device, m_, n_, k_)
            if t is not None and (gws is None or t.numel() > gws.numel()):
                gws = t
        holder.cws.gemm_ws = gws.data_ptr() if gws is not None else None
        holder.cws.gemm_ws_bytes = gws.numel() if gws is not None else 0
        return holder.cws

    def _forward_composite(self, x, emod, ehead, kvs, rp, bufs, B, Ll, L, out_dtype, rep=1):
        lib, w, n = load(), self._w, self.num_layers
        p = lambda t: ctypes.c_void_p(t.data_ptr())
        pt, ph, pw = self.patch_size
        _, Cin, F, Hh, Ww = x.shape
        if self._cdw is None:
            arr = (BlockWeights * n)(*[self._block_cw(b) for b in self.blocks])
            self._cdw = (DitWeights(n, self.in_dim, self.out_dim, pt, ph, pw, arr, p(w["pe_w"]), p(w["pe_b"]), p(w["head_w"]), p(w["head_b"])), arr)
        if getattr(bufs, "dws", None) is None:
            M, dev = B * Ll, self._device
            bufs.xs = torch.empty(M, self.dim, device=dev, dtype=torch.float32)
            bufs.tok = torch.empty(L, Cin * pt * ph * pw, device=dev, dtype=torch.bfloat16)
            bufs.yt = torch.empty(M, w["head_w"].shape[0], device=dev, dtype=torch.float32)
            bufs.dws = DitWorkspace()
            bufs.dws.x, bufs.dws.tokens, bufs.dws.head_out = bufs.xs.data_ptr(), bufs.tok.data_ptr(), bufs.yt.data_ptr()
        bufs.dws.block = self._block_cws(bufs, bufs, B, Ll, L)
        ck = (ctypes.c_void_p * n)(*[kv[0].data_ptr() for kv in kvs])
        cvt = (ctypes.c_void_p * n)(*[kv[1].data_ptr() for kv in kvs])
        out = torch.empty(rep * B, self.out_dim, F, Hh, Ww, device=self._device, dtype=out_dtype)
        args = (p(x), 0 if x.dtype == torch.float32 else 1, p(out), 0 if out_dtype == torch.float32 else 1,
                p(emod), p(ehead), ck, cvt, ctypes.byref(self._cdw[0]), ctypes.byref(bufs.dws),
                p(self._rope_dev[0]), p(self._rope_dev[1]), ctypes.byref(rp), B, F, Hh, Ww, Ll,
                min(int(self.mask_source_frames), F // pt) * pt)
        if rep == 1:
            check(lib.wan_dit_forward(*args, ops._stream()), "wan_dit_forward")
        else:
            check(lib.wan_dit_forward_rep(*args, rep, ops._stream()), "wan_dit_forward_rep")
        self.last_cross_fold = bool(load().wan_get_tuning(b"last_cross_fold"))
        return out

    def _block_composite(self, blk: _Block, em, xs, bufs, ctx_kv, rp, B, Ll, L):
        p = ctypes.c_void_p
        self._block_cw(blk)
        self._block_cws(bufs, bufs, B, Ll, L)
        ck, cvt = ctx_kv
        args = (p(xs.data_ptr()), p(em.data_ptr()), p(ck.data_ptr()), p(cvt.data_ptr()), ctypes.byref(blk._cw), ctypes.byref(bufs.cws))
        if rp is None:
            check(load().wan_dit_block_tail_forward(*args, B, Ll, ops._stream()), "wan_dit_block_tail_forward")
        else:
            check(load().wan_dit_block_forward(*args, p(self._rope_dev[0].data_ptr()), p(self._rope_dev[1].data_ptr()), ctypes.byref(rp),
                                               B, Ll, L, ops._stream()), "wan_dit_block_forward")
        self.last_cross_fold = bool(load().wan_get_tuning(b"last_cross_fold"))

    @torch.no_grad()
    def head_forward(self, x: torch.Tensor, e: torch.Tensor) -> torch.Tensor:
        B, Ll, C = x.shape
        w = self._w
        xs = x.to(device=self._device, dtype=torch.float32).reshape(B * Ll, C).contiguous()
        eh = (w["head_mod"][None] + e.to(self._device, torch.float32)[:, None]).permute(1, 0, 2).contiguous()
        h = ops.ln_modulate(xs, eh[1], eh[0], True, Ll, self.eps)
        return ops.gemm(h, w["head_w"], w["head_b"], ops.EPI_F32).view(B, Ll, -1)

    @torch.no_grad()
    def block_forward(self, x: torch.Tensor, e: torch.Tensor, context: torch.Tensor, grid_sizes, block_index: int = 0,
                      frame_split_indices=None, ground_frame_indices=None, text_kept: Optional[int] = None) -> torch.Tensor:
        if self.sp_world_size != 1 or self.force_ulysses:
            raise NotImplementedError("block_forward is the single-device composite")
        self._usp = False
        self._text_kept = self.text_len if text_kept is None else int(text_kept)
        B, Ll, C = x.shape
        grid = tuple(int(v) for v in grid_sizes)
        L = grid[0] * grid[1] * grid[2]
        if L > Ll or C != self.dim or tuple(e.shape) != (B, 6, C) or tuple(context.shape) != (B, self.text_len, C):
            raise ValueError("block_forward: shapes disagree")
        blk = self.blocks[block_index]
        xs = x.to(device=self._device, dtype=torch.float32).reshape(B * Ll, C).clone()
        em = (blk.modulation[None] + e.to(self._device, torch.float32)).permute(1, 0, 2).contiguous()
        ctx = context.to(device=self._device, dtype=torch.bfloat16).reshape(B * self.text_len, C).contiguous()
        rp = self._rope_map(grid, frame_split_indices, ground_frame_indices, 0, Ll)
        bufs = self._workspaces(B, Ll, L, Ll)
        self._run_block(blk, em, xs, bufs, self._context_kv(blk, ctx, B), rp, B, Ll, L, Ll)
        return xs.view(B, Ll, C)

    @torch.no_grad()
    def forward(self, x, t, context, seq_len, clip_fea=None, y=None, y_camera=None, full_ref=None,
                subject_ref=None, cond_flag=True, frame_split_indices=None, ground_frame_indices=None):
        bs = len(x)
        if not self.cfg_skip_now(bs):
            return self._forward(x, t, context, seq_len, clip_fea, y, y_camera, full_ref, subject_ref, cond_flag,
                                 frame_split_indices, ground_frame_indices)
        half = bs // 2
        args = [cfg_skip_half(a, half) for a in (x, t, context, seq_len, clip_fea, y, y_camera, full_ref, subject_ref, cond_flag,
                                                 frame_split_indices, ground_frame_indices)]
        return self._forward(*args, rep=2)

    def _forward(self, x, t, context, seq_len, clip_fea=None, y=None, y_camera=None, full_ref=None,
                 subject_ref=None, cond_flag=True, frame_split_indices=None, ground_frame_indices=None, rep=1):
        if not self.blocks:
            raise RuntimeError("weights are not loaded (call load_state_dict / from_pretrained)")
        if any(v is not None for v in (clip_fea, y, y_camera, full_ref, subject_ref)):
            raise NotImplementedError("i2v / camera / reference conditioning are other model families "
                                      "(SURVEY.md section 2, rows 13-14)")
        if isinstance(x, (list, tuple)):
            if len({tuple(u.shape) for u in x}) != 1:
                raise NotImplementedError("samples of one call must share a latent shape")
            x = torch.stack(list(x))
        if not x.is_cuda:
            raise RuntimeError("input latents are on the CPU; the HIP path has no CPU fallback")
        dtype = x.dtype
        self._dtype = dtype if dtype in (torch.bfloat16, torch.float32) else self._dtype
        B, Cin, F, Hh, Ww = x.shape
        pt, ph, pw = self.patch_size
        if Cin != self.in_dim:
            raise ValueError(f"latent has {Cin} channels, model expects {self.in_dim}")
        grid = (F // pt, Hh // ph, Ww // pw)
        L = grid[0] * grid[1] * grid[2]
        if t.dim() != 1:
            raise NotImplementedError("per-token timesteps (Wan2.2-5B) are never produced by WanPipeline")
        if t.numel() != B or len(context) != B:
            raise ValueError(f"batch mismatch: x has {B} samples, t {t.numel()}, context {len(context)}")
        self._text_kept = max(int(u.shape[0]) for u in context)
        if B > 1 and frame_split_indices is not None and len(frame_split_indices) > 0:
            gfi = ground_frame_indices if (ground_frame_indices is not None and len(ground_frame_indices) > 0) else None
            if len(frame_split_indices) != B or (gfi is not None and len(gfi) != B):
                raise ValueError(f"frame_split_indices / ground_frame_indices must have one entry per sample ({B})")
            keys = [(int(frame_split_indices[b]), tuple(int(v) for v in gfi[b]) if gfi is not None else None) for b in range(B)]
            if len(set(keys)) > 1:
                if self.teacache is not None:
                    raise NotImplementedError("TeaCache keeps one residual per call: samples of a call must share their CoF position map")
                outs = [None] * B
                for key in dict.fromkeys(keys):
                    idx = [b for b in range(B) if keys[b] == key]
                    sel = torch.tensor(idx, device=x.device)
                    y = self._forward(x.index_select(0, sel), t.index_select(0, sel.to(t.device)), [context[b] for b in idx], seq_len,
                                      cond_flag=cond_flag, frame_split_indices=[key[0]] * len(idx),
                                      ground_frame_indices=[key[1]] * len(idx) if key[1] is not None else None)
                    for j, b in enumerate(idx):
                        outs[b] = y[j]
                return torch.stack(outs * rep)
        P, rank = self.sp_world_size, self.sp_world_rank
        usp = self._usp = self._sp is not None and (P > 1 or self.force_ulysses)
        if usp:
            seq_len = int(math.ceil(seq_len / (8 * P))) * 8 * P
        assert L <= seq_len, f"sequence of {L} tokens exceeds seq_len={seq_len}"
        Ll = seq_len // P
        C, H, dev, w = self.dim, self.num_heads, self._device, self._w
        M = B * Ll

        e, e0 = self._time_embed(t)
        emod = (w["mod_all"][:, None] + e0[None]).permute(0, 2, 1, 3).contiguous()
        ehead = (w["head_mod"][None] + e[:, None]).permute(1, 0, 2).contiguous()

        if self.cache_context:
            ctx_kv = self._hoisted_context(context, B)
        else:
            self._ctx_cache = None
            ctx = self._text_embed(context)
            ctx_kv = [None] * self.num_layers

        r0 = 0
        if self.skip_source_frames and B == 1 and not usp:
            r0 = min(int(self.skip_source_frames), grid[0]) * grid[1] * grid[2]
        if (not usp and self.use_block_composite and self.use_forward_composite and not self._fp8 and self.teacache is None
                and self._probe_layer is None and self._attn_events is None and r0 == 0
                and dtype in (torch.float32, torch.bfloat16)):
            kvs = ctx_kv if ctx_kv[0] is not None else [self._context_kv(blk, ctx, B) for blk in self.blocks]
            rp = self._rope_map(grid, frame_split_indices, ground_frame_indices, 0, Ll)
            return self._forward_composite(x.contiguous(), emod, ehead, kvs, rp, self._workspaces(B, Ll, L, seq_len), B, Ll, L, dtype,
                                           rep=rep)

        xs = torch.zeros(M, C, device=dev, dtype=torch.float32)
        lo, hi = rank * Ll, min((rank + 1) * Ll, L)
        for b in range(B):
            tok = ops.patchify(x[b].contiguous() if x.dtype in (torch.float32, torch.bfloat16)
                               else x[b].float().contiguous(), self.patch_size)
            if hi > lo:
                ops.gemm(tok[lo:hi], w["pe_w"], w["pe_b"], ops.EPI_F32, out=xs[b * Ll: b * Ll + (hi - lo)])

        rp = self._rope_map(grid, frame_split_indices, ground_frame_indices, rank * Ll, Ll)

        bufs = self._workspaces(B, Ll, L, seq_len)
        h = bufs.h

        run_blocks, ori_x = True, None
        if self.teacache is not None:
            run_blocks = self.teacache.decide(e0, cond_flag)
            self.should_calc = run_blocks
            if not run_blocks:
                prev = self.teacache.previous_residual_cond if cond_flag else self.teacache.previous_residual_uncond
                xs.add_(prev[-xs.shape[0]:])
            else:
                ori_x = xs.clone()
        for li, blk in enumerate(self.blocks if run_blocks else ()):
            kv = ctx_kv[li] if ctx_kv[li] is not None else self._context_kv(blk, ctx, B)
            if self._probe_layer == li:
                self._probe = xs.clone()
            if r0 and li == self.num_layers - 1:
                self._last_block_suffix(blk, emod[li], xs, bufs, kv, rp, r0, L)
                break
            self._run_block(blk, emod[li], xs, bufs, kv, rp, B, Ll, L, seq_len)
        if ori_x is not None:
            if cond_flag:
                self.teacache.previous_residual_cond = xs - ori_x
            else:
                self.teacache.previous_residual_uncond = xs - ori_x

        if r0:
            yt = torch.zeros(1, Ll, w["head_w"].shape[0], device=dev, dtype=torch.float32)
            ops.ln_modulate(xs[r0:], ehead[1], ehead[0], True, Ll - r0, self.eps, out=h[r0:])
            ops.gemm(h[r0:], w["head_w"], w["head_b"], ops.EPI_F32, out=yt[0, r0:])
        else:
            ops.ln_modulate(xs, ehead[1], ehead[0], True, Ll, self.eps, out=h)
            yt = ops.gemm(h, w["head_w"], w["head_b"], ops.EPI_F32).view(B, Ll, -1)
        if usp:
            cev = self._comm_pair("all_gather")
            yt = self._sp.all_gather_tokens(yt)
            self._comm_done(cev)
        out_dtype = dtype if dtype in (torch.float32, torch.bfloat16) else torch.float32
        out = torch.empty(rep * B, self.out_dim, grid[0] * pt, grid[1] * ph, grid[2] * pw, device=dev, dtype=out_dtype)
        for b in range(B):
            ops.unpatchify(yt[b], grid, self.patch_size, self.out_dim, out_dtype,
                           zero_frames=min(int(self.mask_source_frames), grid[0]) * pt, out=out[b],
                           rep=None if rep == 1 else rep, rep_stride=None if rep == 1 else B * out[0].numel())
        if self.teacache is not None:
            self.teacache.step_done(cond_flag)
        return out.to(dtype)
```

Measured before the change: 18200 tokens/s.

## Fuse cross-attn query RMSNorm into folded cross-probs kernel; trim text K/V rows

Adds a cross_probs_normed kernel that computes per-row RMS statistics of the raw cross-attention query, applies gain and scale in registers, and stages the normalized query and keys through LDS before the MFMA score and softmax. This removes the separate rmsnorm pass over the large query tensor in the folded cross-attention path. The context K/V projection is also limited to the kept+1 text rows when the fold plan applies, skipping padding rows. The fused kernel holds a whole 32-row block per workgroup with fixed occupancy, which may give less parallelism than the old per-head grid.

```diff
diff --git a/include/wan_hip.h b/include/wan_hip.h
--- a/include/wan_hip.h
+++ b/include/wan_hip.h
@@ -140,6 +140,9 @@
 
 wan_status_t wan_cross_probs(const void* q, int64_t ldq, const void* k, int64_t ldk, int64_t k_bstride, void* probs, int64_t ldp,
                              int batch, int64_t rows_per_batch, int num_heads, int kept, int pad_count, void* stream);
+wan_status_t wan_cross_probs_normed(const void* q_raw, int64_t ldq, const float* gain, float eps, float x0_scale, const void* k,
+                                    int64_t ldk, int64_t k_bstride, void* probs, int64_t ldp, int batch, int64_t rows_per_batch,
+                                    int num_heads, int kept, int pad_count, void* stream);
 wan_status_t wan_cross_fold_values(const void* w_co, int64_t ldw, const void* vt, int64_t ldvt, int64_t vt_bstride, void* vfold,
                                    int64_t ldo, int64_t vfold_bstride, int batch, int dim, int num_heads, int kept, void* stream);
 int wan_cross_fold_plan(int64_t rows, int num_heads, int text_len, int kept, int weights_bf16);
diff --git a/videocof_amd/_lib.py b/videocof_amd/_lib.py
--- a/videocof_amd/_lib.py
+++ b/videocof_amd/_lib.py
@@ -161,6 +161,8 @@
     "wan_attention_workspace_bytes": (c_int64, [c_int, c_int, c_int, c_int, c_int]),
     "wan_cross_probs": (c_int, [c_void_p, c_int64, c_void_p, c_int64, c_int64, c_void_p, c_int64, c_int, c_int64, c_int, c_int, c_int,
                                 c_void_p]),
+    "wan_cross_probs_normed": (c_int, [c_void_p, c_int64, c_void_p, c_float, c_float, c_void_p, c_int64, c_int64, c_void_p, c_int64, c_int,
+                                       c_int64, c_int, c_int, c_int, c_void_p]),
     "wan_cross_fold_values": (c_int, [c_void_p, c_int64, c_void_p, c_int64, c_int64, c_void_p, c_int64, c_int64, c_int, c_int, c_int,
                                       c_int, c_void_p]),
     "wan_cross_fold_plan": (c_int, [c_int64, c_int, c_int, c_int, c_int]),
diff --git a/videocof_amd/csrc/common.hpp b/videocof_amd/csrc/common.hpp
--- a/videocof_amd/csrc/common.hpp
+++ b/videocof_amd/csrc/common.hpp
@@ -75,6 +75,25 @@
     return t;
 }
 
+__device__ __forceinline__ float rms_sumsq8(u32x4 v, float ss) {
+#pragma unroll
+    for (int j = 0; j < 4; ++j) {
+        const float a = bf16lo_to_f32(v[j]), b = bf16hi_to_f32(v[j]);
+        ss += a * a + b * b;
+    }
+    return ss;
+}
+
+template <int NW>
+__device__ __forceinline__ float rms_block_total(const float* wave_sums) {
+    float t = 0.f;
+#pragma unroll
+    for (int i = 0; i < NW; ++i) t += wave_sums[i];
+    return t;
+}
+
+__device__ __forceinline__ float rms_rstd(float sumsq, int dim, float eps) { return rsqrtf(sumsq / (float)dim + eps); }
+
 __device__ __forceinline__ float wave_max(float v) {
 #pragma unroll
     for (int o = 32; o > 0; o >>= 1) v = fmaxf(v, __shfl_xor(v, o, 64));
diff --git a/videocof_amd/csrc/cross_fold.hip b/videocof_amd/csrc/cross_fold.hip
--- a/videocof_amd/csrc/cross_fold.hip
+++ b/videocof_amd/csrc/cross_fold.hip
@@ -31,20 +31,64 @@
     return o;
 }
 
+__device__ __forceinline__ void softmax_rows(f32x16 (&acc)[2], int g, int kept, float log2_pad) {
+    float m = -INFINITY;
+#pragma unroll
+    for (int t = 0; t < 2; ++t)
+#pragma unroll
+        for (int i = 0; i < 4; ++i)
+#pragma unroll
+            for (int jj = 0; jj < 4; ++jj) {
+                const int key = 16 * i + 8 * g + 4 * t + jj;
+                float s = acc[t][4 * i + jj];
+                s = key == kept ? s + log2_pad : s;
+                s = key > kept ? -INFINITY : s;
+                acc[t][4 * i + jj] = s;
+                m = fmaxf(m, s);
+            }
+    m = fmaxf(m, __shfl_xor(m, 32, 64));
+    float sum = 0.f;
+#pragma unroll
+    for (int t = 0; t < 2; ++t)
+#pragma unroll
+        for (int i = 0; i < 16; ++i) {
+            const float e = __builtin_amdgcn_exp2f(acc[t][i] - m);
+            acc[t][i] = e;
+            sum += e;
+        }
+    sum += __shfl_xor(sum, 32, 64);
+    const float inv = __builtin_amdgcn_rcpf(sum);
+#pragma unroll
+    for (int t = 0; t < 2; ++t)
+#pragma unroll
+        for (int i = 0; i < 16; ++i) acc[t][i] *= inv;
+}
+
+__device__ __forceinline__ void softmax_store(f32x16 (&acc)[2], int g, int kept, float log2_pad, bf16_t* pr) {
+    softmax_rows(acc, g, kept, log2_pad);
+    if (pr != nullptr) {
+#pragma unroll
+        for (int i = 0; i < 4; ++i) *(u32x4*)(pr + 16 * i) = pack8(acc, i);
+    }
+}
+
+__device__ __forceinline__ void load_keys(bf16x8 (&ka)[2][8], const bf16_t* kh, int64_t ldk, int r, int kept) {
+    const bf16x8 zero8 = {0, 0, 0, 0, 0, 0, 0, 0};
+#pragma unroll
+    for (int t = 0; t < 2; ++t) {
+        const int key = perm_row(t, r);
+#pragma unroll
+        for (int s = 0; s < 8; ++s) ka[t][s] = key <= kept ? *(const bf16x8*)(kh + (int64_t)key * ldk + s * 8) : zero8;
+    }
+}
+
 __global__ __launch_bounds__(256) void cross_probs_kernel(const bf16_t* __restrict__ q, int64_t ldq, const bf16_t* __restrict__ k,
                                                           int64_t ldk, int64_t k_bstride, bf16_t* __restrict__ p, int64_t ldp, int L,
                                                           int kept, float log2_pad) {
     const int lane = threadIdx.x & 63, wave = threadIdx.x >> 6, r = lane & 31, g = lane >> 5;
     const int h = blockIdx.y, b = blockIdx.z;
-    const bf16x8 zero8 = {0, 0, 0, 0, 0, 0, 0, 0};
     bf16x8 ka[2][8];
-    const bf16_t* kh = k + (int64_t)b * k_bstride + (int64_t)h * CF_D + g * 64;
-#pragma unroll
-    for (int t = 0; t < 2; ++t) {
-        const int key = perm_row(t, r);
-#pragma unroll
-        for (int s = 0; s < 8; ++s) ka[t][s] = key <= kept ? *(const bf16x8*)(kh + (int64_t)key * ldk + s * 8) : zero8;
-    }
+    load_keys(ka, k + (int64_t)b * k_bstride + (int64_t)h * CF_D + g * 64, ldk, r, kept);
     const int first = blockIdx.x * (4 * CF_PROB_NB);
     for (int it = 0; it < CF_PROB_NB; ++it) {
         const int row0 = (first + it * 4 + wave) * 32;
@@ -57,41 +101,118 @@
         for (int s = 0; s < 8; ++s) qb[s] = *(const bf16x8*)(qr + s * 8);
         f32x16 acc[2];
         mfma_head(ka, qb, acc);
-        float m = -INFINITY;
+        softmax_store(acc, g, kept, log2_pad, row < L ? p + grow * ldp + (int64_t)h * CF_KEYS + 8 * g : nullptr);
+    }
+}
+
+__device__ __forceinline__ void wave_lds_handover() {
+    __builtin_amdgcn_fence(__ATOMIC_ACQ_REL, "wavefront");
+    __builtin_amdgcn_wave_barrier();
+}
+
+template <int NV>
+__global__ __launch_bounds__(256) __attribute__((amdgpu_waves_per_eu(2, 2))) void cross_probs_normed_kernel(
+    const bf16_t* __restrict__ q, int64_t ldq, const float* __restrict__ gain, float eps, float x0_scale, const bf16_t* __restrict__ k,
+    int64_t ldk, int64_t k_bstride, bf16_t* __restrict__ p, int64_t ldp, int L, int H, int kept, float log2_pad) {
+    constexpr int ROWS = 32;
+    __shared__ __attribute__((aligned(16))) float cf_lds[5 * ROWS + 4 * 32 * CF_VS_LD / 2];
+    const int dim = H * CF_D, nchunk = dim >> 3;
+    float* red = cf_lds;
+    float* rs = red + ROWS * 4;
+    const int lane = threadIdx.x & 63, wave = threadIdx.x >> 6, r = lane & 31, g = lane >> 5;
+    bf16_t* st = (bf16_t*)(rs + ROWS) + wave * (32 * CF_VS_LD);
+    const int b = blockIdx.y;
+    const int row_base = blockIdx.x * ROWS;
+    const int nrows = L - row_base < ROWS ? L - row_base : ROWS;
+    const bf16_t* qblk = q + ((int64_t)b * L + row_base) * ldq;
+    constexpr int R1 = 8;
+    for (int r0 = 0; r0 < nrows; r0 += R1) {
+        u32x4 v[R1][NV];
+#pragma unroll
+        for (int rr = 0; rr < R1; ++rr) {
+            const bool live = r0 + rr < nrows;
+            const u32x4* xr = (const u32x4*)(qblk + (int64_t)(live ? r0 + rr : 0) * ldq);
+#pragma unroll
+            for (int i = 0; i < NV; ++i) {
+                const int idx = threadIdx.x + i * 256;
+                if (live && idx < nchunk) v[rr][i] = xr[idx]; else v[rr][i] = u32x4{0u, 0u, 0u, 0u};
+            }
+        }
+#pragma unroll
+        for (int rr = 0; rr < R1; ++rr) {
+            float ss = 0.f;
+#pragma unroll
+            for (int i = 0; i < NV; ++i)
+                if (threadIdx.x + i * 256 < nchunk) ss = rms_sumsq8(v[rr][i], ss);
+            ss = wave_sum(ss);
+            if (lane == 0) red[(r0 + rr) * 4 + wave] = ss;
+        }
+    }
+    __syncthreads();
+    if (threadIdx.x < ROWS) rs[threadIdx.x] = threadIdx.x < nrows ? rms_rstd(rms_block_total<4>(red + threadIdx.x * 4), dim, eps) * x0_scale : 0.f;
+    __syncthreads();
+    const int sr = lane >> 4, sc = (lane & 15) * 8;
+    const int pr = lane >> 3, pc = (lane & 7) * 8;
+    const u32x4 zero4 = {0u, 0u, 0u, 0u};
+    auto load_q = [&](u32x4 (&dst)[8], int hh) {
+#pragma unroll
+        for (int i = 0; i < 8; ++i) {
+            const int lr = 4 * i + sr;
+            dst[i] = *(const u32x4*)(qblk + (int64_t)(lr < nrows ? lr : nrows - 1) * ldq + hh * CF_D + sc);
+        }
+    };
+    u32x4 nxt[8];
+    if (wave < H) load_q(nxt, wave);
+    for (int h = wave; h < H; h += 4) {
+        const bf16_t* kh = k + (int64_t)b * k_bstride + (int64_t)h * CF_D + sc;
+        u32x4 kv[2][8];
 #pragma unroll
         for (int t = 0; t < 2; ++t)
 #pragma unroll
-            for (int i = 0; i < 4; ++i)
-#pragma unroll
-                for (int jj = 0; jj < 4; ++jj) {
-                    const int key = 16 * i + 8 * g + 4 * t + jj;
-                    float s = acc[t][4 * i + jj];
-                    s = key == kept ? s + log2_pad : s;
-                    s = key > kept ? -INFINITY : s;
-                    acc[t][4 * i + jj] = s;
-                    m = fmaxf(m, s);
-                }
-        m = fmaxf(m, __shfl_xor(m, 32, 64));
-        float sum = 0.f;
-#pragma unroll
-        for (int t = 0; t < 2; ++t)
-#pragma unroll
-            for (int i = 0; i < 16; ++i) {
-                const float e = __builtin_amdgcn_exp2f(acc[t][i] - m);
-                acc[t][i] = e;
-                sum += e;
+            for (int i = 0; i < 8; ++i) {
+                const int key = perm_row(t, 4 * i + sr);
+                kv[t][i] = key <= kept ? *(const u32x4*)(kh + (int64_t)key * ldk) : zero4;
             }
-        sum += __shfl_xor(sum, 32, 64);
-        const float inv = __builtin_amdgcn_rcpf(sum);
-#pragma unroll
-        for (int t = 0; t < 2; ++t)
-#pragma unroll
-            for (int i = 0; i < 16; ++i) acc[t][i] *= inv;
-        if (row < L) {
-            bf16_t* pr = p + grow * ldp + (int64_t)h * CF_KEYS + 8 * g;
-#pragma unroll
-            for (int i = 0; i < 4; ++i) *(u32x4*)(pr + 16 * i) = pack8(acc, i);
-        }
+        const float4 wa = *(const float4*)(gain + h * CF_D + sc), wb = *(const float4*)(gain + h * CF_D + sc + 4);
+        const float wv[8] = {wa.x, wa.y, wa.z, wa.w, wb.x, wb.y, wb.z, wb.w};
+#pragma unroll
+        for (int i = 0; i < 8; ++i) {
+            const float rstd = rs[4 * i + sr];
+            u32x4 o;
+#pragma unroll
+            for (int j = 0; j < 4; ++j)
+                o[j] = pack_bf16x2(bf16lo_to_f32(nxt[i][j]) * rstd * wv[2 * j], bf16hi_to_f32(nxt[i][j]) * rstd * wv[2 * j + 1]);
+            *(u32x4*)(st + (4 * i + sr) * CF_VS_LD + sc) = o;
+        }
+        wave_lds_handover();
+        bf16x8 qb[8];
+#pragma unroll
+        for (int s = 0; s < 8; ++s) qb[s] = *(const bf16x8*)(st + r * CF_VS_LD + g * 64 + s * 8);
+        wave_lds_handover();
+        if (h + 4 < H) load_q(nxt, h + 4);
+        bf16x8 ka[2][8];
+#pragma unroll
+        for (int t = 0; t < 2; ++t) {
+#pragma unroll
+            for (int i = 0; i < 8; ++i) *(u32x4*)(st + (4 * i + sr) * CF_VS_LD + sc) = kv[t][i];
+            wave_lds_handover();
+#pragma unroll
+            for (int s = 0; s < 8; ++s) ka[t][s] = *(const bf16x8*)(st + r * CF_VS_LD + g * 64 + s * 8);
+            wave_lds_handover();
+        }
+        f32x16 acc[2];
+        mfma_head(ka, qb, acc);
+        softmax_rows(acc, g, kept, log2_pad);
+#pragma unroll
+        for (int i = 0; i < 4; ++i) *(u32x4*)(st + r * CF_VS_LD + 8 * g + 16 * i) = pack8(acc, i);
+        wave_lds_handover();
+#pragma unroll
+        for (int i = 0; i < 4; ++i) {
+            const int lr = 8 * i + pr;
+            if (lr < nrows)
+                *(u32x4*)(p + ((int64_t)b * L + row_base + lr) * ldp + (int64_t)h * CF_KEYS + pc) = *(const u32x4*)(st + (8 * i + pr) * CF_VS_LD + pc);
+        }
+        wave_lds_handover();
     }
 }
 
@@ -182,6 +303,40 @@
     return WAN_OK;
 }
 
+extern "C" wan_status_t wan_cross_probs_normed(const void* q_raw, int64_t ldq, const float* gain, float eps, float x0_scale,
+                                               const void* k, int64_t ldk, int64_t k_bstride, void* probs, int64_t ldp, int batch,
+                                               int64_t rows_per_batch, int num_heads, int kept, int pad_count, void* stream) {
+    WAN_REQUIRE(q_raw && gain && k && probs, WAN_ERR_INVALID, "wan_cross_probs_normed: null tensor");
+    WAN_REQUIRE(batch > 0 && rows_per_batch > 0 && num_heads > 0 && (int64_t)batch * rows_per_batch <= 0x7fffffff && batch <= 65535 &&
+                    num_heads <= 65535,
+                WAN_ERR_INVALID, "wan_cross_probs_normed: batch=%d rows_per_batch=%lld heads=%d", batch, (long long)rows_per_batch, num_heads);
+    WAN_REQUIRE(num_heads * CF_D <= 8192, WAN_ERR_UNSUPPORTED, "wan_cross_probs_normed: dim=%d > 8192", num_heads * CF_D);
+    WAN_REQUIRE(kept >= 0 && kept + 1 <= CF_KEYS && pad_count >= 1, WAN_ERR_UNSUPPORTED,
+                "wan_cross_probs_normed: kept=%d (kept + 1 distinct keys must be <= 64) pad_count=%d", kept, pad_count);
+    WAN_REQUIRE(x0_scale == x0_scale && x0_scale != 0.f && eps == eps && eps >= 0.f, WAN_ERR_INVALID,
+                "wan_cross_probs_normed: x0_scale must be a non-zero number (1 = none) and eps a number >= 0");
+    WAN_REQUIRE(ldq >= (int64_t)num_heads * CF_D && ldk >= (int64_t)num_heads * CF_D && ldp >= (int64_t)num_heads * CF_KEYS &&
+                    k_bstride >= (int64_t)(kept + 1) * ldk,
+                WAN_ERR_INVALID, "wan_cross_probs_normed: ldq=%lld ldk=%lld ldp=%lld k_bstride=%lld too small", (long long)ldq,
+                (long long)ldk, (long long)ldp, (long long)k_bstride);
+    WAN_REQUIRE(ldq % 8 == 0 && ldk % 8 == 0 && ldp % 8 == 0 && k_bstride % 8 == 0 && aligned16(q_raw) && aligned16(gain) && aligned16(k) &&
+                    aligned16(probs),
+                WAN_ERR_INVALID, "wan_cross_probs_normed: rows and the gain vector must be 16-byte aligned");
+    const int L = (int)rows_per_batch, dim = num_heads * CF_D;
+    const int nv = (dim / 8 + 255) / 256;
+    dim3 grid((L + 31) / 32, batch);
+#define CPN_CASE(NV)                                                                                                                   \
+    case NV:                                                                                                                           \
+        hipLaunchKernelGGL(cross_probs_normed_kernel<NV>, grid, dim3(256), 0, (hipStream_t)stream, (const bf16_t*)q_raw, ldq, gain, eps, \
+                           x0_scale, (const bf16_t*)k, ldk, k_bstride, (bf16_t*)probs, ldp, L, num_heads, kept,                        \
+                           log2f((float)pad_count));                                                                                   \
+        break;
+    switch (nv) { CPN_CASE(1) CPN_CASE(2) CPN_CASE(3) CPN_CASE(4) }
+#undef CPN_CASE
+    WAN_CHECK_LAUNCH("wan_cross_probs_normed");
+    return WAN_OK;
+}
+
 extern "C" wan_status_t wan_cross_fold_values(const void* w_co, int64_t ldw, const void* vt, int64_t ldvt, int64_t vt_bstride,
                                               void* vfold, int64_t ldo, int64_t vfold_bstride, int batch, int dim, int num_heads,
                                               int kept, void* stream) {
diff --git a/videocof_amd/csrc/dit_block.cpp b/videocof_amd/csrc/dit_block.cpp
--- a/videocof_amd/csrc/dit_block.cpp
+++ b/videocof_amd/csrc/dit_block.cpp
@@ -78,18 +78,19 @@
     const float* shift_mlp = emod + 3 * bC, *scale_mlp = emod + 4 * bC, *gate_mlp = emod + 5 * bC;
     WAN_TRY(wan_ln_modulate(x, w->norm3_w, w->norm3_b, 0, ws->h, M, C, M, eps, stream));
     WAN_TRY(wan_gemm_bf16_ws(ws->h, C, w->w_cq, C, w->b_cq, ws->cq, C, (int)M, C, C, WAN_EPI_BF16, nullptr, 0, GWS, GWSB, stream));
-    WAN_TRY(wan_rmsnorm_rope(ws->cq, w->norm_cq, nullptr, nullptr, C, M, C, 128, eps, nullptr, nullptr, nullptr, qs, stream));
     const int kept = ws->text_kept;
     const bool fold = ws->vfold && ws->vfold_bytes >= wan_cross_fold_workspace_bytes(batch, C) && wan_cross_fold_plan(M, H, T, kept, 1);
     wan_note_cross_fold(fold ? 1 : 0);
     if (fold) {
         const int64_t Kf = (int64_t)H * 64;
-        WAN_TRY(wan_cross_probs(ws->cq, C, ctx_k, C, (int64_t)T * C, ws->att, Kf, batch, Ll, H, kept, T - kept, stream));
+        WAN_TRY(wan_cross_probs_normed(ws->cq, C, w->norm_cq, eps, qs, ctx_k, C, (int64_t)T * C, ws->att, Kf, batch, Ll, H, kept, T - kept,
+                                       stream));
         WAN_TRY(wan_cross_fold_values(w->w_co, C, ctx_vt, T, (int64_t)C * T, ws->vfold, Kf, (int64_t)C * Kf, batch, C, H, kept, stream));
         for (int b = 0; b < batch; ++b)
             WAN_TRY(wan_gemm_bf16_ws(at(ws->att, (int64_t)b * Ll * Kf * 2), Kf, at(ws->vfold, (int64_t)b * C * Kf * 2), Kf, w->b_co,
                                   x + (int64_t)b * Ll * C, C, (int)Ll, C, (int)Kf, WAN_EPI_RESID_F32, nullptr, 0, GWS, GWSB, stream));
     } else {
+        WAN_TRY(wan_rmsnorm_rope(ws->cq, w->norm_cq, nullptr, nullptr, C, M, C, 128, eps, nullptr, nullptr, nullptr, qs, stream));
         WAN_TRY(wan_attention_fwd(ws->cq, C, Ll * C, ctx_k, C, (int64_t)T * C, ctx_vt, T, (int64_t)C * T, ws->att, C, Ll * C, batch, (int)Ll,
                                   T, H, 128, 0.f, WAN_ATTN_Q_PRESCALED, ws->attn_ws_cross, ws->attn_ws_cross_bytes, stream));
         WAN_TRY(wan_gemm_bf16_ws(ws->att, C, w->w_co, C, w->b_co, x, C, (int)M, C, C, WAN_EPI_RESID_F32, nullptr, 0, GWS, GWSB, stream));
diff --git a/videocof_amd/csrc/norm_kernels.hip b/videocof_amd/csrc/norm_kernels.hip
--- a/videocof_amd/csrc/norm_kernels.hip
+++ b/videocof_amd/csrc/norm_kernels.hip
@@ -89,12 +89,7 @@
     }
     __syncthreads();
 #pragma unroll
-    for (int r = 0; r < R; ++r) {
-        float t = 0.f;
-#pragma unroll
-        for (int i = 0; i < NW; ++i) t += red[r][i];
-        v[r] = t;
-    }
+    for (int r = 0; r < R; ++r) v[r] = rms_block_total<NW>(red[r]);
 }
 
 template <int NV, int R>
@@ -220,14 +215,10 @@
         const int idx = threadIdx.x + i * kThreads;
         if (idx < nchunk) {
             v[i] = xr[idx];
-#pragma unroll
-            for (int j = 0; j < 4; ++j) {
-                const float a = bf16lo_to_f32(v[i][j]), b = bf16hi_to_f32(v[i][j]);
-                ss += a * a + b * b;
-            }
-        }
-    }
-    const float rstd = rsqrtf(block_sum<kWaves>(ss, red) / (float)dim + eps)
+            ss = rms_sumsq8(v[i], ss);
+        }
+    }
+    const float rstd = rms_rstd(block_sum<kWaves>(ss, red), dim, eps)
                        * (blockIdx.y == 0 ? x0_scale : x1_scale);
 #pragma unroll
     for (int i = 0; i < NV; ++i) {
@@ -326,13 +317,7 @@
         ss[r] = 0.f;
 #pragma unroll
         for (int i = 0; i < NV; ++i) {
-            if (threadIdx.x + i * kThreads < nchunk) {
-#pragma unroll
-                for (int j = 0; j < 4; ++j) {
-                    const float a = bf16lo_to_f32(v[r][i][j]), b = bf16hi_to_f32(v[r][i][j]);
-                    ss[r] += a * a + b * b;
-                }
-            }
+            if (threadIdx.x + i * kThreads < nchunk) ss[r] = rms_sumsq8(v[r][i], ss[r]);
         }
     }
     block_sum_n<kWaves, R>(ss, red);
@@ -349,7 +334,7 @@
             for (int r = 0; r < R; ++r) {
                 const int64_t row = row0 + r;
                 if (row >= rows) continue;
-                const float rstd = rsqrtf(ss[r] / (float)dim + eps) * post;
+                const float rstd = rms_rstd(ss[r], dim, eps) * post;
                 u32x4 o;
 #pragma unroll
                 for (int j = 0; j < 4; ++j) {
diff --git a/videocof_amd/ops.py b/videocof_amd/ops.py
--- a/videocof_amd/ops.py
+++ b/videocof_amd/ops.py
@@ -494,6 +494,30 @@
 
 
 @_on_tensor_device
+def cross_probs_normed(q_raw: torch.Tensor, gain: torch.Tensor, eps: float, k: torch.Tensor, num_heads: int, kept: int, pad_count: int,
+                       x0_scale: float = 1.0, out: Optional[torch.Tensor] = None) -> torch.Tensor:
+    _need(q_raw, torch.bfloat16, "cross_probs_normed.q_raw")
+    _need(gain, torch.float32, "cross_probs_normed.gain")
+    _need(k, torch.bfloat16, "cross_probs_normed.k")
+    B, L, C = q_raw.shape
+    if k.dim() != 3 or k.shape[0] != B or k.shape[2] != C or C != num_heads * 128 or k.shape[1] < kept + 1:
+        raise ValueError(f"cross_probs_normed: q {tuple(q_raw.shape)} / k {tuple(k.shape)} / heads {num_heads} / kept {kept} disagree")
+    if gain.numel() != C or not gain.is_contiguous():
+        raise ValueError(f"cross_probs_normed: gain must be contiguous with {C} elements")
+    if B > 1 and q_raw.stride(0) != L * q_raw.stride(1):
+        raise ValueError("cross_probs_normed: the samples of q must follow each other without a gap")
+    if out is None:
+        out = torch.empty(B * L, num_heads * 64, device=q_raw.device, dtype=torch.bfloat16)
+    _need(out, torch.bfloat16, "cross_probs_normed.out")
+    if tuple(out.shape) != (B * L, num_heads * 64):
+        raise ValueError(f"cross_probs_normed: out shape {tuple(out.shape)} != ({B * L},{num_heads * 64})")
+    _lib.check(_lib.load().wan_cross_probs_normed(_p(q_raw), q_raw.stride(1), _p(gain), float(eps), float(x0_scale), _p(k), k.stride(1),
+                                                  k.stride(0), _p(out), out.stride(0), B, L, int(num_heads), int(kept), int(pad_count),
+                                                  _stream()), "wan_cross_probs_normed")
+    return out
+
+
+@_on_tensor_device
 def cross_fold_values(w_co: torch.Tensor, vt: torch.Tensor, num_heads: int, kept: int,
                       out: Optional[torch.Tensor] = None) -> torch.Tensor:
     _need(w_co, torch.bfloat16, "cross_fold_values.w_co")
diff --git a/videocof_amd/wan_transformer3d.py b/videocof_amd/wan_transformer3d.py
--- a/videocof_amd/wan_transformer3d.py
+++ b/videocof_amd/wan_transformer3d.py
@@ -136,6 +136,7 @@
         self.cache_context = False
         self._text_kept = text_len
         self.last_cross_fold = False
+        self.last_text_rows = text_len
         self._ctx_cache = None
         self._fp8 = ()
         self.fp8_attn_exponents = (5, 2)
@@ -565,16 +566,36 @@
         hid = ops.gemm(ctx, w["te_w0"], w["te_b0"], ops.EPI_GELU_BF16)
         return ops.gemm(hid, w["te_w2"], w["te_b2"], ops.EPI_BF16)
 
-    def _context_kv(self, blk: _Block, ctx: torch.Tensor, B: int, out=None):
+    def _context_kv(self, blk: _Block, ctx: torch.Tensor, B: int, out=None, rows: Optional[int] = None):
         C, T = self.dim, self.text_len
+        n = T if rows is None else int(rows)
+        self.last_text_rows = n
         ck, cvt = out if out is not None else (None, None)
-        ck = ops.gemm(ctx, blk.w_ck, blk.b_ck, ops.EPI_BF16, out=None if ck is None else ck.view(B * T, C))
-        ops.rmsnorm_rope_(ck, blk.nck, None, None, self.d, self.eps)
+        if n == T:
+            ck = ops.gemm(ctx, blk.w_ck, blk.b_ck, ops.EPI_BF16, out=None if ck is None else ck.view(B * T, C))
+            ops.rmsnorm_rope_(ck, blk.nck, None, None, self.d, self.eps)
+        else:
+            ck = torch.empty(B * T, C, device=self._device, dtype=torch.bfloat16) if ck is None else ck.view(B * T, C)
+            for b in range(B):
+                ops.gemm(ctx[b * T:b * T + n], blk.w_ck, blk.b_ck, ops.EPI_BF16, out=ck[b * T:b * T + n])
+                ops.rmsnorm_rope_(ck[b * T:b * T + n], blk.nck, None, None, self.d, self.eps)
         if cvt is None:
             cvt = torch.empty(B, C, T, device=self._device, dtype=torch.bfloat16)
         for b in range(B):
-            ops.gemm(ctx[b * T:(b + 1) * T], blk.w_cv, blk.b_cv, ops.EPI_BF16_T, out=cvt[b])
+            ops.gemm(ctx[b * T:b * T + n], blk.w_cv, blk.b_cv, ops.EPI_BF16_T, out=cvt[b])
         return ck.view(B, T, C), cvt
+
+    def _text_rows(self, blk: _Block, B: int, rows: int, bf16: bool = False) -> int:
+        lib, T, C, kept = load(), self.text_len, self.dim, self._text_kept
+        if self.cache_context:
+            return T
+        if not lib.wan_cross_fold_plan(rows, self.num_heads, T, kept, int(bf16 or not (blk.f8 and "co" in blk.f8))):
+            return T
+        n = kept + 1
+        same = lambda m: (lib.wan_gemm_ws_plan(m, C, C), lib.wan_gemm_ws_splits(m, C, C))
+        if same(n) != same(B * T) or same(n) != same(T):
+            return T
+        return n
 
     def _hoisted_context(self, context, B, into=None):
         vers = tuple(u._version for u in context)
@@ -883,17 +904,18 @@
             x, h, cq, att, ff = x[r0:], h[r0:], cq[r0:], att[r0:], ff[r0:]
         a = self._ln_operand(blk, "cq", x, blk.n3w, blk.n3b, False, B * n, bufs, h, bf16)
         self._linear(blk, "cq", a, ops.EPI_BF16, cq)
-        ops.rmsnorm_rope_(cq, blk.ncq, None, None, self.d, self.eps, x0_scale=self._qs)
         H, kept = self.num_heads, self._text_kept
         self.last_cross_fold = bool(load().wan_cross_fold_plan(B * n, H, self.text_len, kept, int(bf16 or not (blk.f8 and "co" in blk.f8))))
         if self.last_cross_fold:
             probs = att.reshape(-1)[:B * n * H * 64].view(B * n, H * 64)
-            ops.cross_probs(cq.view(B, n, C), ctx_kv[0], H, kept, self.text_len - kept, out=probs)
+            ops.cross_probs_normed(cq.view(B, n, C), blk.ncq, self.eps, ctx_kv[0], H, kept, self.text_len - kept, x0_scale=self._qs,
+                                   out=probs)
             vfold = self._vfold(bufs, B)
             ops.cross_fold_values(blk.w_co, ctx_kv[1], H, kept, out=vfold)
             for b in range(B):
                 ops.gemm(probs[b * n:(b + 1) * n], vfold[b], blk.b_co, ops.EPI_RESID_F32, out=x[b * n:(b + 1) * n])
         else:
+            ops.rmsnorm_rope_(cq, blk.ncq, None, None, self.d, self.eps, x0_scale=self._qs)
             ops.attention_fwd(cq.view(B, n, C), *ctx_kv, self.num_heads, out=att.view(B, n, C), q_prescaled=True, workspace=ws_cross)
             self._linear(blk, "co", self._row_operand(blk, "co", att, bufs, bf16), ops.EPI_RESID_F32, x)
         a = self._ln_operand(blk, "w1", x, em[4], em[3], True, n, bufs, h, bf16)
@@ -1042,7 +1064,7 @@
         ctx = context.to(device=self._device, dtype=torch.bfloat16).reshape(B * self.text_len, C).contiguous()
         rp = self._rope_map(grid, frame_split_indices, ground_frame_indices, 0, Ll)
         bufs = self._workspaces(B, Ll, L, Ll)
-        self._run_block(blk, em, xs, bufs, self._context_kv(blk, ctx, B), rp, B, Ll, L, Ll)
+        self._run_block(blk, em, xs, bufs, self._context_kv(blk, ctx, B, rows=self._text_rows(blk, B, B * Ll)), rp, B, Ll, L, Ll)
         return xs.view(B, Ll, C)
 
     @torch.no_grad()
@@ -1127,7 +1149,7 @@
         if (not usp and self.use_block_composite and self.use_forward_composite and not self._fp8 and self.teacache is None
                 and self._probe_layer is None and self._attn_events is None and r0 == 0
                 and dtype in (torch.float32, torch.bfloat16)):
-            kvs = ctx_kv if ctx_kv[0] is not None else [self._context_kv(blk, ctx, B) for blk in self.blocks]
+            kvs = ctx_kv if ctx_kv[0] is not None else [self._context_kv(blk, ctx, B, rows=self._text_rows(blk, B, M)) for blk in self.blocks]
             rp = self._rope_map(grid, frame_split_indices, ground_frame_indices, 0, Ll)
             return self._forward_composite(x.contiguous(), emod, ehead, kvs, rp, self._workspaces(B, Ll, L, seq_len), B, Ll, L, dtype,
                                            rep=rep)
@@ -1155,10 +1177,12 @@
             else:
                 ori_x = xs.clone()
         for li, blk in enumerate(self.blocks if run_blocks else ()):
-            kv = ctx_kv[li] if ctx_kv[li] is not None else self._context_kv(blk, ctx, B)
+            suffix = bool(r0) and li == self.num_layers - 1
+            kv = ctx_kv[li] if ctx_kv[li] is not None else self._context_kv(
+                blk, ctx, B, rows=self._text_rows(blk, B, Ll - r0, bf16=True) if suffix else self._text_rows(blk, B, M))
             if self._probe_layer == li:
                 self._probe = xs.clone()
-            if r0 and li == self.num_layers - 1:
+            if suffix:
                 self._last_block_suffix(blk, emod[li], xs, bufs, kv, rp, r0, L)
                 break
             self._run_block(blk, emod[li], xs, bufs, kv, rp, B, Ll, L, seq_len)
```

Result: no change. 18260 tokens/s (median of 6 runs) (+0.3%).
